# AUTOMATIC1111/stable-diffusion-webui

Hardware: AMD Instinct MI355X
Metric: images/sec SD1.5 512x512 20-step Euler-a, batch 8 per GPU (higher is better)
Workload: dtype f16

## Files before the change

### include/sdmi.h

```cpp
#ifndef SDMI_H
#define SDMI_H

#include <stdint.h>

#ifdef __cplusplus
extern "C" {
#endif

#define SDMI_VERSION 100

enum { SDMI_F16 = 0, SDMI_F32 = 1 };

typedef struct sdmi_engine sdmi_engine;

int sdmi_version(void);
const char* sdmi_last_error(void);
int sdmi_device_ok(void);


int64_t sdmi_attention_workspace_bytes(int B, int H, int M, int D);
int sdmi_attention(const void* q, const void* k, const void* v, void* out,
                   int B, int H, int N, int M, int D,
                   int ldq, int ldk, int ldv, int ldo, float scale,
                   void* workspace, int64_t workspace_bytes, void* stream);

int64_t sdmi_attention_wide_workspace_bytes(int B, int N, int M, int D);
int sdmi_attention_wide(const void* q, const void* k, const void* v, void* out,
                        int B, int N, int M, int D,
                        int ldq, int ldk, int ldv, int ldo, float scale,
                        void* workspace, int64_t workspace_bytes, void* stream);

int sdmi_attention_vt(const void* q, const void* k, const void* vt, void* out,
                      int B, int H, int N, int M, int D,
                      int ldq, int ldk, int vt_ld, int ldo, float scale, int force_generic, void* stream);

typedef struct sdmi_conv_desc {
    const void* a0;
    const void* a1;
    const void* w;
    const void* bias;
    const void* rowbias;
    const void* resid;
    void* out;
    int32_t c0, c1, lda0, lda1;
    int32_t B, Hi, Wi, Ho, Wo;
    int32_t taps;
    int32_t stride;
    int32_t pad;
    int32_t up;
    int32_t N;
    int32_t n_real;
    int32_t ldo, ldr;
    int32_t flags;
    float alpha;
    int32_t batch;
    int64_t a_bs, w_bs, o_bs, r_bs;
    int32_t force_generic;
    int32_t reserved;
    void* splitk_workspace;
    int64_t splitk_workspace_bytes;
} sdmi_conv_desc;

enum {
    SDMI_EP_OUT_F32  = 1,
    SDMI_EP_GEGLU    = 2,
    SDMI_EP_NCHW     = 4,
    SDMI_EP_BIAS_ROW = 8,
    SDMI_EP_WRAP = 128,
    SDMI_EP_TRANSPOSE = 64
};
int sdmi_conv_gemm(const sdmi_conv_desc* d, void* stream);
int64_t sdmi_conv_splitk_workspace_bytes(int M, int N, int K, int batch);

int sdmi_pack_conv_weight(const void* w_oihw, int dtype, void* out_f16, int O, int I, int kh, int kw,
                          int O_pad, int I_pad, int geglu, void* stream);

int sdmi_groupnorm(const void* x0, const void* x1, int c0, int c1, const void* gamma_f32, const void* beta_f32,
                   void* out_f16, int B, int HW, int groups, float eps, int silu,
                   void* workspace_f32, int64_t workspace_bytes, void* stream);
int64_t sdmi_groupnorm_workspace_bytes(int B, int HW, int groups);

int sdmi_layernorm(const void* x, const void* gamma_f32, const void* beta_f32, void* out_f16,
                   int64_t rows, int C, float eps, void* stream);

int64_t sdmi_rowchain_ff_pack_bytes(int C, int hidden);
int sdmi_rowchain_ff_pack(const void* w1_f16, const void* b1_f32_or_null, const void* w2_f16, void* packs, int C, int hidden,
                          void* stream);
int sdmi_rowchain_ff(const void* x_f16, void* out_f16, const void* ln_gamma_f32, const void* ln_beta_f32, const void* packs,
                     const void* b2_f32_or_null, int64_t rows, int C, int hidden, float eps, void* stream);

int sdmi_xattn_chain(const void* x_f16, void* out_f16, const void* ln_gamma_f32, const void* ln_beta_f32, const void* wq_f16,
                     const void* wo_f16, const void* bo_f32_or_null, const void* k_f16, const void* vt_f16, int64_t rows,
                     int rows_per_image, int C, int heads, int L, int Lpad, float eps, void* stream);


int sdmi_philox_randn(void* out_f32, int64_t n, uint64_t seed, uint32_t offset, void* stream);

int sdmi_slerp(void* out_f32, const void* low_f32, const void* high_f32, float val, int C, int H, int W, void* scratch_f32,
               void* stream);


int sdmi_cfg_prepare_input(const void* x_f32, const void* c_in_f32, void* x_in, int out_dtype,
                           int B, int reps, int64_t chw, void* stream);

int sdmi_cfg_prepare_concat(const void* x_f32, const void* c_in_f32, const void* c_concat_f32, void* x_in, int out_dtype,
                            int B, int reps, int C, int Cc, int64_t hw, uint32_t zero_reps, void* stream);

int sdmi_cfg_combine(const void* x_f32, const void* eps_f32, const void* c_out_f32, float cond_scale, int mode,
                     const void* mask_f32, const void* nmask_f32, const void* init_latent_f32,
                     void* denoised_f32, int B, int64_t chw, void* stream);

int sdmi_cfg_combine_affine(const void* x_f32, const void* out_f32, const void* c_out_f32, const void* c_skip_f32,
                            float cond_scale, const void* mask_f32, const void* nmask_f32, const void* init_latent_f32,
                            void* denoised_f32, int B, int64_t chw, void* stream);

int sdmi_euler_step(void* x_f32, const void* denoised_f32, const void* noise_f32_or_null,
                    float sigma, float sigma_down, float sigma_up, float s_noise, int64_t n, void* stream);

int sdmi_dpmpp2m_step(void* x_f32, const void* denoised_f32, const void* old_denoised_f32_or_null,
                      float ratio, float em1, float c1, float c2, int64_t n, void* stream);

int sdmi_ddim_step(void* x_f32, const void* e_t_f32, const void* noise_f32_or_null, void* pred_x0_f32_or_null,
                   float a_t, float a_prev, float sigma_t, float sqrt_one_minus_at, int64_t n, void* stream);

int sdmi_axpby(void* y_f32, const void* x_f32, float a, const void* z_f32_or_null, float b, int64_t n, void* stream);

int sdmi_lincomb(void* out_f32, const void* const* terms_f32, const float* coefs, int n_terms, int64_t n, void* stream);

int sdmi_dpm_error_partials(const void* x_low_f32, const void* x_high_f32, const void* x_prev_f32, float atol, float rtol,
                            void* partial256_f32, int64_t n, void* stream);

int sdmi_latent_resize(const void* in_f32, void* out_f32, int planes, int hi, int wi, int ho, int wo, int mode, void* stream);

int sdmi_mask_blend(void* x_f32, const void* init_f32, const void* mask_f32, const void* nmask_f32, int64_t n, void* stream);

int sdmi_image_to_u8(const void* img_f32_nchw, void* out_u8_nhwc, int B, int C, int H, int W, void* stream);

typedef struct sdmi_unet_config {
    int32_t in_channels, out_channels, model_channels;
    int32_t num_levels;
    int32_t channel_mult[8];
    int32_t num_res_blocks;
    int32_t attn_level[8];
    int32_t transformer_depth[8];
    int32_t num_heads;
    int32_t num_head_channels;
    int32_t context_dim;
    int32_t adm_in_channels;
    int32_t reserved[4];
} sdmi_unet_config;

typedef struct sdmi_vae_config {
    int32_t ch, num_levels;
    int32_t ch_mult[8];
    int32_t num_res_blocks, in_channels, out_ch, z_channels;
    float scale_factor;
    int32_t reserved[4];
} sdmi_vae_config;

sdmi_engine* sdmi_engine_create(int device);
void sdmi_engine_destroy(sdmi_engine* e);

int sdmi_unet_configure(sdmi_engine* e, const sdmi_unet_config* cfg);
int sdmi_unet_load_tensor(sdmi_engine* e, const char* key, const void* data, int dtype, int ndim,
                          const int64_t* shape, int on_device);
int sdmi_unet_finalize(sdmi_engine* e);

int sdmi_unet_update_weight(sdmi_engine* e, const char* key, const void* data, int dtype, int ndim,
                            const int64_t* shape, int on_device);

int sdmi_unet_hypernet_clear(sdmi_engine* e);
int sdmi_unet_hypernet_begin(sdmi_engine* e, float multiplier);
int sdmi_unet_hypernet_linear(sdmi_engine* e, int dim, int which, const void* w, const void* b, int dtype, int out_features,
                              int in_features, int on_device);
int sdmi_unet_hypernet_act(sdmi_engine* e, int dim, int which, int act);
int sdmi_unet_hypernet_layernorm(sdmi_engine* e, int dim, int which, const void* gamma, const void* beta, int dtype, int n, int on_device);

int sdmi_unet_update_vector(sdmi_engine* e, const char* key, const void* data, int dtype, int64_t n, int on_device);

int sdmi_lora_merge(void* out_f32, const void* w, int w_dtype, const void* up, int up_dtype, const void* down, int down_dtype,
                    int rows, int cols, int rank, float scale, void* stream);

int sdmi_weight_hadamard(void* out_f32, const void* w_f32, const void* a_f32, const void* b_f32, float scale, int64_t n, void* stream);
int sdmi_weight_kron(void* out_f32, const void* w_f32, const void* w1_f32, const void* w2_f32, int r1, int c1, int r2, int c2, int k,
                     float scale, void* stream);
int sdmi_weight_ia3(void* out_f32, const void* w_f32, const void* v_f32, int rows, int cols, int on_input, float scale, void* stream);
int sdmi_weight_dora(void* out_f32, const void* w_f32, const void* delta_f32, const void* dora_scale_f32, int rows, int cin, int k,
                     float mult, void* stream);

int sdmi_vae_configure(sdmi_engine* e, const sdmi_vae_config* cfg);
int sdmi_vae_load_tensor(sdmi_engine* e, const char* key, const void* data, int dtype, int ndim,
                         const int64_t* shape, int on_device);
int sdmi_vae_finalize(sdmi_engine* e);

int sdmi_unet_set_context(sdmi_engine* e, const void* context, int io_dtype, int Bn, int L, void* stream);
int sdmi_unet_set_context_cached(sdmi_engine* e, const void* context, int io_dtype, int Bn, int L, void* stream);
int sdmi_unet_forward(sdmi_engine* e, const void* x, const void* timesteps, const void* context, const void* y,
                      void* out, int io_dtype, int Bn, int h, int w, int L, void* stream);
enum { SDMI_CALL_UNIFORM_T = 1, SDMI_CALL_CFG_PAIRS = 2, SDMI_CALL_DERIVE = 4 };
int sdmi_unet_set_control(sdmi_engine* e, const void* const* tensors, const int64_t* numel, int n, int only_mid_control);
int sdmi_unet_forward_ex(sdmi_engine* e, const void* x, const void* timesteps, const void* context, const void* y,
                         void* out, int io_dtype, int Bn, int h, int w, int L, int call_flags, void* stream);

int sdmi_vae_decode(sdmi_engine* e, const void* z, int io_dtype, void* out_f32, int B, int h, int w, void* stream);

int sdmi_vae_encode(sdmi_engine* e, const void* x, int io_dtype, void* out_f32, int B, int H, int W, void* stream);

int64_t sdmi_engine_arena_bytes(sdmi_engine* e);
int sdmi_engine_set_option(sdmi_engine* e, const char* name, int value);

int sdmi_engine_tap_count(sdmi_engine* e);
int sdmi_engine_tap_info(sdmi_engine* e, int index, char* name_out, int capacity, int64_t* dims_bhwc);
int sdmi_engine_tap_read(sdmi_engine* e, int index, void* out_f16_nhwc, void* stream);

int sdmi_debug_set(const char* name, int value);
int sdmi_debug_set_str(const char* name, const char* value);

int sdmi_profile_begin(void);
int sdmi_profile_end(char* json_out, int capacity);

int sdmi_bench_conv_gemm(const sdmi_conv_desc* d, int iters, float* ms_out, void* stream);

typedef struct sdmi_clip_config {
    int vocab_size;
    int max_positions;
    int hidden;
    int layers;
    int heads;
    int intermediate;
    int act;
    float eps;
} sdmi_clip_config;

int sdmi_clip_configure(sdmi_engine* e, int slot, const sdmi_clip_config* cfg);
int sdmi_clip_load_tensor(sdmi_engine* e, int slot, const char* key, const void* data, int dtype, int ndim,
                          const int64_t* shape, int on_device);
int sdmi_clip_finalize(sdmi_engine* e, int slot);
int sdmi_clip_forward(sdmi_engine* e, int slot, const void* tokens_i32, const void* inputs_embeds_f32_or_null, int B, int L,
                      int skip, int apply_final_ln, void* out_f32, void* pooled_f32_or_null, void* stream);


enum {
    SDMI_RRDB_EP_NONE = 0,
    SDMI_RRDB_EP_LRELU = 1,
    SDMI_RRDB_EP_RES1 = 2,
    SDMI_RRDB_EP_RES2 = 3
// ... 98 lines not shown
```

### stable-diffusion-webui_amd/_lib.py

```python
from __future__ import annotations

import ctypes as C
import os
import re

_HERE = os.path.dirname(os.path.abspath(__file__))
LIB_PATH = os.environ.get("SDMI_LIB") or os.path.join(_HERE, "lib", "libsdmi.so")
HEADER_PATH = os.path.join(os.path.dirname(_HERE), "include", "sdmi.h")

F16, F32 = 0, 1
EP_OUT_F32, EP_GEGLU, EP_NCHW, EP_BIAS_ROW = 1, 2, 4, 8
EP_TRANSPOSE = 64
EP_WRAP = 128
RRDB_EP_NONE, RRDB_EP_LRELU, RRDB_EP_RES1, RRDB_EP_RES2 = 0, 1, 2, 3
RRDB_ST_F16, RRDB_ST_F32_NCHW, RRDB_ST_U8_HWC = 0, 1, 2
COMPACT_EP_NONE, COMPACT_EP_PRELU, COMPACT_EP_TAIL = 0, 1, 2


class SdmiError(RuntimeError):
    pass


class ConvDesc(C.Structure):
    _fields_ = [
        ("a0", C.c_void_p), ("a1", C.c_void_p), ("w", C.c_void_p), ("bias", C.c_void_p), ("rowbias", C.c_void_p),
        ("resid", C.c_void_p), ("out", C.c_void_p),
        ("c0", C.c_int32), ("c1", C.c_int32), ("lda0", C.c_int32), ("lda1", C.c_int32),
        ("B", C.c_int32), ("Hi", C.c_int32), ("Wi", C.c_int32), ("Ho", C.c_int32), ("Wo", C.c_int32),
        ("taps", C.c_int32), ("stride", C.c_int32), ("pad", C.c_int32), ("up", C.c_int32),
        ("N", C.c_int32), ("n_real", C.c_int32), ("ldo", C.c_int32), ("ldr", C.c_int32),
        ("flags", C.c_int32), ("alpha", C.c_float), ("batch", C.c_int32),
        ("a_bs", C.c_int64), ("w_bs", C.c_int64), ("o_bs", C.c_int64), ("r_bs", C.c_int64),
        ("force_generic", C.c_int32), ("reserved", C.c_int32),
        ("splitk_workspace", C.c_void_p), ("splitk_workspace_bytes", C.c_int64),
    ]


class RrdbDesc(C.Structure):
    _fields_ = [
        ("in_", C.c_void_p), ("w", C.c_void_p), ("bias", C.c_void_p), ("r1", C.c_void_p), ("r2", C.c_void_p), ("out", C.c_void_p),
        ("B", C.c_int32), ("H", C.c_int32), ("W", C.c_int32), ("cin", C.c_int32), ("lda", C.c_int32), ("up", C.c_int32),
        ("nout", C.c_int32), ("n_real", C.c_int32), ("ldo", C.c_int32), ("ldr1", C.c_int32), ("ldr2", C.c_int32),
        ("ep", C.c_int32), ("store", C.c_int32), ("alpha", C.c_float), ("beta", C.c_float),
    ]


class CompactDesc(C.Structure):
    _fields_ = [
        ("in_", C.c_void_p), ("w", C.c_void_p), ("bias", C.c_void_p), ("slope", C.c_void_p), ("base", C.c_void_p), ("out", C.c_void_p),
        ("B", C.c_int32), ("H", C.c_int32), ("W", C.c_int32), ("cin", C.c_int32), ("lda", C.c_int32), ("ldo", C.c_int32),
        ("n_real", C.c_int32), ("ep", C.c_int32), ("r", C.c_int32), ("base_u8", C.c_int32), ("out_u8", C.c_int32), ("grid_cap", C.c_int32),
    ]


class SwinAttnDesc(C.Structure):
    _fields_ = [
        ("qkv", C.c_void_p), ("bias", C.c_void_p), ("out", C.c_void_p),
        ("B", C.c_int32), ("H", C.c_int32), ("W", C.c_int32), ("heads", C.c_int32), ("D", C.c_int32),
        ("ldq", C.c_int32), ("ldo", C.c_int32), ("shift", C.c_int32), ("scale", C.c_float),
    ]


class SwinIRConfigC(C.Structure):
    _fields_ = [("embed_dim", C.c_int32), ("num_layers", C.c_int32), ("depths", C.c_int32 * 16), ("num_heads", C.c_int32),
                ("mlp_hidden", C.c_int32), ("resi_3conv", C.c_int32), ("scale", C.c_int32)]


class UNetConfigC(C.Structure):
    _fields_ = [
        ("in_channels", C.c_int32), ("out_channels", C.c_int32), ("model_channels", C.c_int32),
        ("num_levels", C.c_int32), ("channel_mult", C.c_int32 * 8), ("num_res_blocks", C.c_int32),
        ("attn_level", C.c_int32 * 8), ("transformer_depth", C.c_int32 * 8),
        ("num_heads", C.c_int32), ("num_head_channels", C.c_int32), ("context_dim", C.c_int32),
        ("adm_in_channels", C.c_int32), ("reserved", C.c_int32 * 4),
    ]


class VAEConfigC(C.Structure):
    _fields_ = [
        ("ch", C.c_int32), ("num_levels", C.c_int32), ("ch_mult", C.c_int32 * 8),
        ("num_res_blocks", C.c_int32), ("in_channels", C.c_int32), ("out_ch", C.c_int32), ("z_channels", C.c_int32),
        ("scale_factor", C.c_float), ("reserved", C.c_int32 * 4),
    ]


class ClipConfigC(C.Structure):
    _fields_ = [("vocab_size", C.c_int32), ("max_positions", C.c_int32), ("hidden", C.c_int32), ("layers", C.c_int32),
                ("heads", C.c_int32), ("intermediate", C.c_int32), ("act", C.c_int32), ("eps", C.c_float)]


def declared_symbols() -> list:
    src = open(HEADER_PATH).read()
    src = re.sub(r"/\*.*?\*/", "", src, flags=re.S)
    return sorted(set(re.findall(r"\b(sdmi_[a-z0-9_]+)\s*\(", src)))


if not os.path.exists(LIB_PATH):
    raise ImportError(
        f"{LIB_PATH} is missing: build it with `python -c 'import __graft_entry__ as g; g.build()'` "
        "(hipcc --offload-arch=gfx950). There is no CPU fallback for the MI355X engine.")

lib = C.CDLL(LIB_PATH)

_vp, _i, _i64, _f, _u32 = C.c_void_p, C.c_int, C.c_int64, C.c_float, C.c_uint32
_SIGS = {
    "sdmi_version": (C.c_int, []),
    "sdmi_last_error": (C.c_char_p, []),
    "sdmi_device_ok": (C.c_int, []),
    "sdmi_attention_workspace_bytes": (_i64, [_i, _i, _i, _i]),
    "sdmi_attention": (_i, [_vp, _vp, _vp, _vp, _i, _i, _i, _i, _i, _i, _i, _i, _i, _f, _vp, _i64, _vp]),
    "sdmi_attention_wide_workspace_bytes": (_i64, [_i, _i, _i, _i]),
    "sdmi_attention_wide": (_i, [_vp, _vp, _vp, _vp, _i, _i, _i, _i, _i, _i, _i, _i, _f, _vp, _i64, _vp]),
    "sdmi_attention_vt": (_i, [_vp, _vp, _vp, _vp, _i, _i, _i, _i, _i, _i, _i, _i, _i, _f, _i, _vp]),
    "sdmi_conv_gemm": (_i, [C.POINTER(ConvDesc), _vp]),
    "sdmi_conv_splitk_workspace_bytes": (_i64, [_i, _i, _i, _i]),
    "sdmi_bench_conv_gemm": (_i, [C.POINTER(ConvDesc), _i, C.POINTER(C.c_float), _vp]),
    "sdmi_pack_conv_weight": (_i, [_vp, _i, _vp, _i, _i, _i, _i, _i, _i, _i, _vp]),
    "sdmi_groupnorm": (_i, [_vp, _vp, _i, _i, _vp, _vp, _vp, _i, _i, _i, _f, _i, _vp, _i64, _vp]),
    "sdmi_groupnorm_workspace_bytes": (_i64, [_i, _i, _i]),
    "sdmi_layernorm": (_i, [_vp, _vp, _vp, _vp, _i64, _i, _f, _vp]),
    "sdmi_rowchain_ff_pack_bytes": (_i64, [_i, _i]),
    "sdmi_rowchain_ff_pack": (_i, [_vp, _vp, _vp, _vp, _i, _i, _vp]),
    "sdmi_rowchain_ff": (_i, [_vp, _vp, _vp, _vp, _vp, _vp, _i64, _i, _i, _f, _vp]),
    "sdmi_xattn_chain": (_i, [_vp, _vp, _vp, _vp, _vp, _vp, _vp, _vp, _vp, _i64, _i, _i, _i, _i, _i, _f, _vp]),
    "sdmi_philox_randn": (_i, [_vp, _i64, C.c_uint64, C.c_uint32, _vp]),
    "sdmi_slerp": (_i, [_vp, _vp, _vp, _f, _i, _i, _i, _vp, _vp]),
    "sdmi_cfg_prepare_input": (_i, [_vp, _vp, _vp, _i, _i, _i, _i64, _vp]),
    "sdmi_cfg_prepare_concat": (_i, [_vp, _vp, _vp, _vp, _i, _i, _i, _i, _i, _i64, _u32, _vp]),
    "sdmi_cfg_combine": (_i, [_vp, _vp, _vp, _f, _i, _vp, _vp, _vp, _vp, _i, _i64, _vp]),
    "sdmi_cfg_combine_affine": (_i, [_vp, _vp, _vp, _vp, _f, _vp, _vp, _vp, _vp, _i, _i64, _vp]),
    "sdmi_euler_step": (_i, [_vp, _vp, _vp, _f, _f, _f, _f, _i64, _vp]),
    "sdmi_dpmpp2m_step": (_i, [_vp, _vp, _vp, _f, _f, _f, _f, _i64, _vp]),
    "sdmi_ddim_step": (_i, [_vp, _vp, _vp, _vp, _f, _f, _f, _f, _i64, _vp]),
    "sdmi_axpby": (_i, [_vp, _vp, _f, _vp, _f, _i64, _vp]),
    "sdmi_dpm_error_partials": (_i, [_vp, _vp, _vp, _f, _f, _vp, _i64, _vp]),
    "sdmi_lincomb": (_i, [_vp, C.POINTER(_vp), C.POINTER(_f), _i, _i64, _vp]),
    "sdmi_mask_blend": (_i, [_vp, _vp, _vp, _vp, _i64, _vp]),
    "sdmi_latent_resize": (_i, [_vp, _vp, _i, _i, _i, _i, _i, _i, _vp]),
    "sdmi_image_to_u8": (_i, [_vp, _vp, _i, _i, _i, _i, _vp]),
    "sdmi_engine_create": (_vp, [_i]),
    "sdmi_engine_destroy": (None, [_vp]),
    "sdmi_unet_configure": (_i, [_vp, C.POINTER(UNetConfigC)]),
    "sdmi_unet_load_tensor": (_i, [_vp, C.c_char_p, _vp, _i, _i, C.POINTER(C.c_int64), _i]),
    "sdmi_unet_finalize": (_i, [_vp]),
    "sdmi_clip_configure": (_i, [_vp, _i, C.POINTER(ClipConfigC)]),
    "sdmi_clip_load_tensor": (_i, [_vp, _i, C.c_char_p, _vp, _i, _i, C.POINTER(C.c_int64), _i]),
    "sdmi_clip_finalize": (_i, [_vp, _i]),
    "sdmi_clip_forward": (_i, [_vp, _i, _vp, _vp, _i, _i, _i, _i, _vp, _vp, _vp]),
    "sdmi_unet_update_weight": (_i, [_vp, C.c_char_p, _vp, _i, _i, C.POINTER(C.c_int64), _i]),
    "sdmi_unet_hypernet_clear": (_i, [_vp]),
    "sdmi_unet_hypernet_begin": (_i, [_vp, _f]),
    "sdmi_unet_hypernet_linear": (_i, [_vp, _i, _i, _vp, _vp, _i, _i, _i, _i]),
    "sdmi_unet_hypernet_act": (_i, [_vp, _i, _i, _i]),
    "sdmi_unet_hypernet_layernorm": (_i, [_vp, _i, _i, _vp, _vp, _i, _i, _i]),
    "sdmi_unet_update_vector": (_i, [_vp, C.c_char_p, _vp, _i, _i64, _i]),
    "sdmi_lora_merge": (_i, [_vp, _vp, _i, _vp, _i, _vp, _i, _i, _i, _i, _f, _vp]),
    "sdmi_weight_hadamard": (_i, [_vp, _vp, _vp, _vp, _f, _i64, _vp]),
    "sdmi_weight_kron": (_i, [_vp, _vp, _vp, _vp, _i, _i, _i, _i, _i, _f, _vp]),
    "sdmi_weight_ia3": (_i, [_vp, _vp, _vp, _i, _i, _i, _f, _vp]),
    "sdmi_weight_dora": (_i, [_vp, _vp, _vp, _vp, _i, _i, _i, _f, _vp]),
    "sdmi_vae_configure": (_i, [_vp, C.POINTER(VAEConfigC)]),
    "sdmi_vae_load_tensor": (_i, [_vp, C.c_char_p, _vp, _i, _i, C.POINTER(C.c_int64), _i]),
    "sdmi_vae_finalize": (_i, [_vp]),
    "sdmi_unet_set_context": (_i, [_vp, _vp, _i, _i, _i, _vp]),
    "sdmi_unet_set_context_cached": (_i, [_vp, _vp, _i, _i, _i, _vp]),
    "sdmi_unet_forward": (_i, [_vp, _vp, _vp, _vp, _vp, _vp, _i, _i, _i, _i, _i, _vp]),
    "sdmi_unet_set_control": (_i, [_vp, _vp, _vp, _i, _i]),
    "sdmi_unet_forward_ex": (_i, [_vp, _vp, _vp, _vp, _vp, _vp, _i, _i, _i, _i, _i, _i, _vp]),
    "sdmi_vae_decode": (_i, [_vp, _vp, _i, _vp, _i, _i, _i, _vp]),
    "sdmi_vae_encode": (_i, [_vp, _vp, _i, _vp, _i, _i, _i, _vp]),
    "sdmi_debug_set": (_i, [C.c_char_p, _i]),
    "sdmi_debug_set_str": (_i, [C.c_char_p, C.c_char_p]),
    "sdmi_profile_begin": (_i, []),
    "sdmi_profile_end": (_i, [C.c_char_p, _i]),
    "sdmi_engine_arena_bytes": (_i64, [_vp]),
    "sdmi_engine_set_option": (_i, [_vp, C.c_char_p, _i]),
    "sdmi_engine_tap_count": (_i, [_vp]),
    "sdmi_engine_tap_info": (_i, [_vp, _i, C.c_char_p, _i, C.POINTER(C.c_int64)]),
    "sdmi_engine_tap_read": (_i, [_vp, _i, _vp, _vp]),
    "sdmi_rrdb_conv": (_i, [C.POINTER(RrdbDesc), _vp]),
    "sdmi_esrgan_blob_floats": (_i64, [_i, _i]),
    "sdmi_esrgan_create": (_vp, [_vp, _vp, _i64, _i, _i, _i]),
    "sdmi_esrgan_destroy": (None, [_vp]),
    "sdmi_esrgan_scratch_bytes": (_i64, [_vp, _i, _i, _i]),
    "sdmi_esrgan_run": (_i, [_vp, _vp, _i, _i, _i, _i, _vp, _i, _vp]),
    "sdmi_compact_conv": (_i, [C.POINTER(CompactDesc), _vp]),
    "sdmi_compact_blob_floats": (_i64, [_i, _i]),
    "sdmi_compact_create": (_vp, [_vp, _vp, _i64, _i, _i]),
    "sdmi_compact_destroy": (None, [_vp]),
    "sdmi_compact_scratch_bytes": (_i64, [_vp, _i, _i, _i]),
    "sdmi_compact_run": (_i, [_vp, _vp, _i, _i, _i, _i, _vp, _i, _vp]),
    "sdmi_swin_attention": (_i, [C.POINTER(SwinAttnDesc), _vp]),
    "sdmi_swin_layernorm": (_i, [_vp, _vp, _vp, _vp, _i64, _i, _i, _f, _vp]),
    "sdmi_swinir_blob_floats": (_i64, [C.POINTER(SwinIRConfigC)]),
    "sdmi_swinir_create": (_vp, [_vp, _vp, _i64, C.POINTER(SwinIRConfigC)]),
    "sdmi_swinir_destroy": (None, [_vp]),
    "sdmi_swinir_scratch_bytes": (_i64, [_vp, _i, _i, _i]),
    "sdmi_swinir_run": (_i, [_vp, _vp, _i, _i, _i, _i, _vp, _i, _vp]),
}
for _name, (_res, _args) in _SIGS.items():
    _fn = getattr(lib, _name)
    _fn.restype = _res
    _fn.argtypes = _args


def last_error() -> str:
    return (lib.sdmi_last_error() or b"").decode("utf-8", "replace")


def check(rc: int, what: str = "sdmi call"):
    if rc != 0:
        raise SdmiError(f"{what} failed: {last_error()}")


def device_ok() -> bool:
    return bool(lib.sdmi_device_ok())


def require_device():
    if not device_ok():
        raise SdmiError("no gfx950 (MI355X) device visible to HIP: the engine has no CPU path")


def ptr(t):
    return None if t is None else C.c_void_p(t.data_ptr())


def stream_ptr():
    import torch
    return C.c_void_p(torch.cuda.current_stream().cuda_stream)


def dtype_code(t) -> int:
    import torch
    if t.dtype == torch.float16:
        return F16
    if t.dtype == torch.float32:
        return F32
    raise SdmiError(f"unsupported dtype {t.dtype}: the engine takes fp16 or fp32 tensors")
```

### stable-diffusion-webui_amd/csrc/capi.cpp

```cpp
#include "engine.h"
#include "prof.h"
#include <cstring>

namespace sdmi {
extern int g_vae_attn_rows;
int unet_forward(sdmi_engine* e, const void* x, const void* t, const void* ctx, const void* y, void* out, int io_dtype,
                 int Bn, int h, int w, int L, hipStream_t s);
int vae_decode(sdmi_engine* e, const void* z, int io_dtype, float* out, int B, int h, int w, hipStream_t s);
int vae_encode(sdmi_engine* e, const void* x, int io_dtype, float* out, int B, int H, int W, hipStream_t s);
int engine_load_unet_tensor(sdmi_engine* e, const char* key, const void* data, int dtype, int ndim, const int64_t* shape, int on_device);
int engine_load_vae_tensor(sdmi_engine* e, const char* key, const void* data, int dtype, int ndim, const int64_t* shape, int on_device);
int engine_unet_finalize(sdmi_engine* e);
int engine_clip_configure(sdmi_engine* e, int slot, const sdmi_clip_config* cfg);
int engine_clip_load_tensor(sdmi_engine* e, int slot, const char* key, const void* data, int dtype, int ndim, const int64_t* shape, int on_device);
int engine_clip_finalize(sdmi_engine* e, int slot);
int engine_clip_forward(sdmi_engine* e, int slot, const int* tokens, const float* inputs_embeds, int B, int L, int skip,
                        int apply_final_ln, float* out, float* pooled, hipStream_t s);
int engine_unet_update_weight(sdmi_engine* e, const char* key, const void* data, int dtype, int ndim, const int64_t* shape, int on_device);
int engine_vae_finalize(sdmi_engine* e);
int engine_hypernet_clear(sdmi_engine* e);
int engine_hypernet_begin(sdmi_engine* e, float multiplier);
int engine_hypernet_linear(sdmi_engine* e, int dim, int which, const void* w, const void* b, int dtype, int out_f, int in_f, int on_device);
int engine_hypernet_act(sdmi_engine* e, int dim, int which, int act);
int engine_hypernet_layernorm(sdmi_engine* e, int dim, int which, const void* g, const void* b, int dtype, int n, int on_device);
// ... 82 lines not shown
    SDMI_REQUIRE(ldq % 8 == 0 && ldk % 8 == 0 && ldo % 8 == 0, "sdmi_attention_wide: row strides must be multiples of 8 elements");
    SDMI_REQUIRE(ldq >= D && ldk >= D && ldv >= D && ldo >= D, "sdmi_attention_wide: row strides must be at least D");
    SDMI_REQUIRE(workspace && workspace_bytes >= sdmi_attention_wide_workspace_bytes(B, N, M, D), "attention workspace too small");
    hipStream_t s = (hipStream_t)stream;
    const int mpad = (M + 63) / 64 * 64;
    const int rows_max = N < kWideRows ? N : kWideRows;
    half_t* vt = (half_t*)workspace;
    float* S = (float*)(vt + (size_t)B * D * mpad);
    half_t* P = (half_t*)(S + (size_t)rows_max * mpad);
    if (launch_transpose_v((const half_t*)v, vt, B, 1, M, D, ldv, mpad, s)) return 1;
    for (int b = 0; b < B; ++b)
        for (int r0 = 0; r0 < N; r0 += kWideRows) {
            const int rows = N - r0 < kWideRows ? N - r0 : kWideRows;
            GemmP p{};
            p.a0 = (const half_t*)q + ((size_t)b * N + r0) * ldq; p.c0 = D; p.cin = D; p.lda0 = ldq;
            p.w = (const half_t*)k + (size_t)b * M * ldk; p.ldw = ldk;
            p.out = S;
            p.Hi = rows; p.Wi = 1; p.Ho = rows; p.Wo = 1; p.taps = 1; p.stride = 1;
            p.M = rows; p.N = mpad; p.n_valid = M; p.K = D; p.ldo = mpad; p.rows_per_batch = rows; p.n_real = mpad;
            p.flags = EP_OUT_F32;
            p.alpha = scale;
            if (launch_gemm(p, 1, false, true, s)) return 1;
            if (launch_softmax_rows(S, P, rows, M, mpad, mpad, s)) return 1;
            GemmP g{};
            g.a0 = P; g.c0 = mpad; g.cin = mpad; g.lda0 = mpad;
            g.w = vt + (size_t)b * D * mpad; g.ldw = mpad;
            g.out = (half_t*)out + ((size_t)b * N + r0) * ldo;
            g.Hi = rows; g.Wi = 1; g.Ho = rows; g.Wo = 1; g.taps = 1; g.stride = 1;
            g.M = rows; g.N = D; g.K = mpad; g.ldo = ldo; g.rows_per_batch = rows; g.n_real = D;
            g.alpha = 1.f;
            if (launch_gemm(g, 1, false, true, s)) return 1;
        }
    return 0;
    API_GUARD_END
}

static int desc_to_p(const sdmi_conv_desc* d, GemmP* p) {
    SDMI_REQUIRE(d != nullptr, "null descriptor");
    SDMI_REQUIRE(d->a0 && d->w && d->out, "sdmi_conv_gemm: null a0 / w / out");
    SDMI_REQUIRE(d->B > 0 && d->Hi > 0 && d->Wi > 0 && d->Ho > 0 && d->Wo > 0 && d->N > 0 && d->c0 > 0 && (!d->a1 || d->c1 > 0),
                 "sdmi_conv_gemm: B, Hi, Wi, Ho, Wo, N, c0 (and c1 with a second source) must be positive");
    SDMI_REQUIRE(d->stride >= 0 && d->stride <= 2, "sdmi_conv_gemm: stride must be 1 or 2 (0 = 1)");
    *p = GemmP{};
    p->a0 = (const half_t*)d->a0; p->a1 = (const half_t*)d->a1; p->w = (const half_t*)d->w;
    p->bias = (const float*)d->bias; p->rowbias = (const float*)d->rowbias; p->resid = (const half_t*)d->resid;
    p->out = d->out;
    p->c0 = d->c0; p->c1 = d->a1 ? d->c1 : 0; p->cin = p->c0 + p->c1;
    p->lda0 = d->lda0 ? d->lda0 : d->c0; p->lda1 = d->lda1 ? d->lda1 : d->c1;
    p->Hi = d->Hi; p->Wi = d->Wi; p->Ho = d->Ho; p->Wo = d->Wo;
    p->taps = d->taps; p->stride = d->stride ? d->stride : 1; p->pad = d->pad; p->up = d->up;
    SDMI_REQUIRE(p->taps == 1 || p->taps == 9, "taps must be 1 or 9");
    SDMI_REQUIRE(p->c0 % 8 == 0 && p->c1 % 8 == 0, "sdmi_conv_gemm: c0 and c1 must each be a multiple of 8 (pad channels)");
    SDMI_REQUIRE(p->lda0 >= p->c0 && (!p->a1 || p->lda1 >= p->c1), "sdmi_conv_gemm: lda smaller than the channel count");
    p->M = d->B * d->Ho * d->Wo; p->N = d->N; p->K = p->taps * p->cin;
    p->ldw = p->K; p->ldrb = d->N;
    p->rows_per_batch = d->Ho * d->Wo;
    p->n_real = d->n_real ? d->n_real : d->N;
    p->flags = d->flags;
    SDMI_REQUIRE(!(p->flags & EP_NCHW) || (p->n_real > 0 && p->n_real <= p->N), "sdmi_conv_gemm: n_real must lie in 1 .. N");
    SDMI_REQUIRE(!(p->flags & EP_GEGLU) || p->N % 64 == 0, "sdmi_conv_gemm: SDMI_EP_GEGLU needs N % 64 == 0 (32 values | 32 gates)");
    const int batch = d->batch > 0 ? d->batch : 1;
    const bool tr = (p->flags & EP_TRANSPOSE) != 0, nchw = (p->flags & EP_NCHW) != 0;
    const long cols = tr ? p->rows_per_batch : (p->flags & EP_GEGLU) ? p->N / 2 : p->N;
    const long rows = tr ? (long)d->B * p->N : p->M;
    p->ldo = d->ldo ? d->ldo : (int)cols; p->ldr = d->ldr ? d->ldr : d->N;
    SDMI_REQUIRE(nchw || p->ldo >= cols, "sdmi_conv_gemm: ldo smaller than the stored columns");
    SDMI_REQUIRE(!p->resid || p->ldr >= p->N, "sdmi_conv_gemm: ldr smaller than N");
    p->alpha = d->alpha == 0.f ? 1.f : d->alpha;
    p->a_bs = d->a_bs; p->w_bs = d->w_bs; p->o_bs = d->o_bs; p->r_bs = d->r_bs;
    const long foot = nchw ? (long)d->B * p->n_real * p->rows_per_batch : (rows - 1) * p->ldo + cols;
    SDMI_REQUIRE(batch == 1 || p->o_bs >= foot, "sdmi_conv_gemm: batch > 1 needs o_bs >= the elements one batch element stores");
    SDMI_REQUIRE(batch == 1 || (p->a_bs >= 0 && p->w_bs >= 0 && p->r_bs >= 0), "sdmi_conv_gemm: negative batch stride");
    const size_t need = gemm_splitk_ws_bytes(p->M, p->N, p->K, batch);
    if (d->splitk_workspace && need && (size_t)d->splitk_workspace_bytes >= need) p->splitk_ws = (float*)d->splitk_workspace;
    return 0;
}

int64_t sdmi_conv_splitk_workspace_bytes(int M, int N, int K, int batch) { return (int64_t)gemm_splitk_ws_bytes(M, N, K, batch); }

int sdmi_conv_gemm(const sdmi_conv_desc* d, void* stream) {
    API_GUARD_BEGIN
    GemmP p;
    if (desc_to_p(d, &p)) return 1;
    const char* env = getenv("SDMI_NO_GLDS");
    return launch_gemm(p, d->batch > 0 ? d->batch : 1, d->force_generic == 1, !(env && env[0] == '1') && d->force_generic != 2,
                       (hipStream_t)stream);
    API_GUARD_END
}

int sdmi_bench_conv_gemm(const sdmi_conv_desc* d, int iters, float* ms_out, void* stream) {
    API_GUARD_BEGIN
    GemmP p;
    if (desc_to_p(d, &p)) return 1;
    hipStream_t s = (hipStream_t)stream;
    hipEvent_t e0, e1;
    SDMI_CHECK_HIP(hipEventCreate(&e0));
    SDMI_CHECK_HIP(hipEventCreate(&e1));
    const bool glds = d->force_generic != 2;
    for (int i = 0; i < 2; ++i)
        if (launch_gemm(p, d->batch > 0 ? d->batch : 1, d->force_generic == 1, glds, s)) return 1;
    SDMI_CHECK_HIP(hipEventRecord(e0, s));
    for (int i = 0; i < iters; ++i)
        if (launch_gemm(p, d->batch > 0 ? d->batch : 1, d->force_generic == 1, glds, s)) return 1;
    SDMI_CHECK_HIP(hipEventRecord(e1, s));
    SDMI_CHECK_HIP(hipEventSynchronize(e1));
    float ms = 0.f;
    SDMI_CHECK_HIP(hipEventElapsedTime(&ms, e0, e1));
    *ms_out = ms / (float)iters;
    (void)hipEventDestroy(e0);
    (void)hipEventDestroy(e1);
    return 0;
    API_GUARD_END
}

int sdmi_pack_conv_weight(const void* w, int dtype, void* out, int O, int I, int kh, int kw, int O_pad, int I_pad, int geglu,
                          void* stream) {
    API_GUARD_BEGIN
    return launch_pack_conv_weight(w, dtype, (half_t*)out, O, I, kh, kw, O_pad, I_pad, geglu, (hipStream_t)stream);
    API_GUARD_END
}

int64_t sdmi_groupnorm_workspace_bytes(int B, int HW, int groups) { return groupnorm_ws_bytes(B, HW, groups); }

int sdmi_groupnorm(const void* x0, const void* x1, int c0, int c1, const void* gamma, const void* beta, void* out, int B, int HW,
                   int groups, float eps, int silu, void* ws, int64_t ws_bytes, void* stream) {
    API_GUARD_BEGIN
    SDMI_REQUIRE(ws && ws_bytes >= groupnorm_ws_bytes(B, HW, groups), "groupnorm workspace too small");
    return launch_groupnorm((const half_t*)x0, (const half_t*)x1, c0, x1 ? c1 : 0, (const float*)gamma, (const float*)beta,
                            (half_t*)out, B, HW, groups, eps, silu != 0, (float*)ws, (hipStream_t)stream);
    API_GUARD_END
}

int sdmi_layernorm(const void* x, const void* gamma, const void* beta, void* out, int64_t rows, int C, float eps, void* stream) {
    API_GUARD_BEGIN
    return launch_layernorm((const half_t*)x, (const float*)gamma, (const float*)beta, (half_t*)out, rows, C, eps, (hipStream_t)stream);
    API_GUARD_END
}

int64_t sdmi_rowchain_ff_pack_bytes(int C, int hidden) { return (int64_t)rowchain_ff_pack_bytes(C, hidden); }
int sdmi_rowchain_ff_pack(const void* w1, const void* b1, const void* w2, void* packs, int C, int hidden, void* stream) {
    API_GUARD_BEGIN
    SDMI_REQUIRE(w1 && w2 && packs, "null argument");
    return launch_rowchain_ff_pack((const half_t*)w1, (const float*)b1, (const half_t*)w2, packs, C, hidden, false, (hipStream_t)stream);
    API_GUARD_END
}
int sdmi_rowchain_ff(const void* x, void* out, const void* g, const void* b, const void* packs, const void* b2, int64_t rows, int C,
                     int hidden, float eps, void* stream) {
    API_GUARD_BEGIN
    SDMI_REQUIRE(x && out && g && b && packs, "null argument");
    return launch_rowchain_ff((const half_t*)x, (half_t*)out, (const float*)g, (const float*)b, packs, (const float*)b2, (long)rows, C,
                              hidden, eps, (hipStream_t)stream);
    API_GUARD_END
}
int sdmi_xattn_chain(const void* x, void* out, const void* g, const void* b, const void* wq, const void* wo, const void* bo, const void* k,
                     const void* vt, int64_t rows, int rows_per_image, int C, int heads, int L, int Lpad, float eps, void* stream) {
    API_GUARD_BEGIN
    return launch_xattn_chain((const half_t*)x, (half_t*)out, (const float*)g, (const float*)b, (const half_t*)wq, (const half_t*)wo,
                              (const float*)bo, (const half_t*)k, (const half_t*)vt, (long)rows, rows_per_image, C, heads, L, Lpad, eps,
                              (hipStream_t)stream);
    API_GUARD_END
}


int sdmi_philox_randn(void* out, int64_t n, uint64_t seed, uint32_t offset, void* stream) {
    API_GUARD_BEGIN
    return launch_philox((float*)out, n, seed, offset, (hipStream_t)stream);
    API_GUARD_END
}

int sdmi_slerp(void* out, const void* low, const void* high, float val, int C, int H, int W, void* scratch, void* stream) {
    API_GUARD_BEGIN
    SDMI_REQUIRE(out && low && high && scratch && C > 0 && H > 0 && W > 0, "bad arguments");
    return launch_slerp((float*)out, (const float*)low, (const float*)high, val, C, H, W, (float*)scratch, (hipStream_t)stream);
    API_GUARD_END
}

int sdmi_cfg_prepare_input(const void* x, const void* c_in, void* x_in, int out_dtype, int B, int reps, int64_t chw, void* stream) {
    API_GUARD_BEGIN
    return launch_cfg_prepare((const float*)x, (const float*)c_in, x_in, out_dtype, B, reps, chw, (hipStream_t)stream);
    API_GUARD_END
}

int sdmi_cfg_prepare_concat(const void* x, const void* c_in, const void* c_concat, void* x_in, int out_dtype, int B, int reps,
                            int C, int Cc, int64_t hw, uint32_t zero_reps, void* stream) {
    API_GUARD_BEGIN
    SDMI_REQUIRE(x && c_concat && x_in, "null pointer");
    SDMI_REQUIRE(B > 0 && reps > 0 && reps <= 32 && C > 0 && Cc > 0 && hw > 0, "bad sizes");
    return launch_cfg_prepare_concat((const float*)x, (const float*)c_in, (const float*)c_concat, x_in, out_dtype, B, reps, C, Cc, hw,
                                     zero_reps, (hipStream_t)stream);
    API_GUARD_END
}

int sdmi_cfg_combine(const void* x, const void* eps, const void* c_out, float cond_scale, int mode, const void* mask,
                     const void* nmask, const void* init_latent, void* den, int B, int64_t chw, void* stream) {
    API_GUARD_BEGIN
    SDMI_REQUIRE(mode == 1 || (x && c_out), "sigma-space combine needs x and c_out");
    return launch_cfg_combine((const float*)x, (const float*)eps, (const float*)c_out, cond_scale, mode, (const float*)mask,
                              (const float*)nmask, (const float*)init_latent, (float*)den, B, chw, (hipStream_t)stream);
    API_GUARD_END
}

int sdmi_euler_step(void* x, const void* den, const void* noise, float sigma, float sigma_down, float sigma_up, float s_noise,
                    int64_t n, void* stream) {
    API_GUARD_BEGIN
    SDMI_REQUIRE(x && den && n >= 0, "sdmi_euler_step: null x / denoised or negative n");
    return launch_euler_step((float*)x, (const float*)den, (const float*)noise, sigma, sigma_down, sigma_up, s_noise, n,
                             (hipStream_t)stream);
    API_GUARD_END
}

int sdmi_dpmpp2m_step(void* x, const void* den, const void* old, float ratio, float em1, float c1, float c2, int64_t n,
                      void* stream) {
    API_GUARD_BEGIN
    SDMI_REQUIRE(x && den && n >= 0, "sdmi_dpmpp2m_step: null x / denoised or negative n");
    return launch_dpmpp2m_step((float*)x, (const float*)den, (const float*)old, ratio, em1, c1, c2, n, (hipStream_t)stream);
    API_GUARD_END
}

int sdmi_ddim_step(void* x, const void* e_t, const void* noise, void* pred_x0, float a_t, float a_prev, float sigma_t,
                   float sqrt_one_minus_at, int64_t n, void* stream) {
    API_GUARD_BEGIN
    SDMI_REQUIRE(x && e_t && n >= 0, "sdmi_ddim_step: null x / e_t or negative n");
    return launch_ddim_step((float*)x, (const float*)e_t, (const float*)noise, (float*)pred_x0, a_t, a_prev, sigma_t,
                            sqrt_one_minus_at, n, (hipStream_t)stream);
    API_GUARD_END
}

int sdmi_dpm_error_partials(const void* x_low, const void* x_high, const void* x_prev, float atol, float rtol, void* partial256_f32,
                            int64_t n, void* stream) {
    API_GUARD_BEGIN
    SDMI_REQUIRE(x_low && x_high && x_prev && partial256_f32 && n > 0, "null argument");
    return launch_dpm_error((const float*)x_low, (const float*)x_high, (const float*)x_prev, atol, rtol, (float*)partial256_f32, n,
                            (hipStream_t)stream);
    API_GUARD_END
}
int sdmi_lincomb(void* out, const void* const* terms, const float* coefs, int n_terms, int64_t n, void* stream) {
    API_GUARD_BEGIN
    SDMI_REQUIRE(out && terms && coefs, "null argument");
    return launch_lincomb((float*)out, (const float* const*)terms, coefs, n_terms, n, (hipStream_t)stream);
    API_GUARD_END
}

int sdmi_latent_resize(const void* in, void* out, int planes, int hi, int wi, int ho, int wo, int mode, void* stream) {
    API_GUARD_BEGIN
    SDMI_REQUIRE(in && out, "null argument");
    return launch_latent_resize((const float*)in, (float*)out, planes, hi, wi, ho, wo, mode, (hipStream_t)stream);
    API_GUARD_END
}

int sdmi_cfg_combine_affine(const void* x, const void* out, const void* c_out, const void* c_skip, float cond_scale,
                            const void* mask, const void* nmask, const void* init_latent, void* den, int B, int64_t chw, void* stream) {
    API_GUARD_BEGIN
    SDMI_REQUIRE(x && out && c_out && c_skip && den, "null argument");
    return launch_cfg_combine_affine((const float*)x, (const float*)out, (const float*)c_out, (const float*)c_skip, cond_scale,
                                     (const float*)mask, (const float*)nmask, (const float*)init_latent, (float*)den, B, chw,
                                     (hipStream_t)stream);
    API_GUARD_END
}

int sdmi_mask_blend(void* x, const void* init, const void* mask, const void* nmask, int64_t n, void* stream) {
    API_GUARD_BEGIN
    SDMI_REQUIRE(x && init && mask && nmask, "null argument");
    return launch_mask_blend((float*)x, (const float*)init, (const float*)mask, (const float*)nmask, n, (hipStream_t)stream);
    API_GUARD_END
}

int sdmi_axpby(void* y, const void* x, float a, const void* z, float b, int64_t n, void* stream) {
    API_GUARD_BEGIN
    SDMI_REQUIRE(y && x && n >= 0, "sdmi_axpby: null y / x or negative n");
    return launch_axpby((float*)y, (const float*)x, a, (const float*)z, b, n, (hipStream_t)stream);
    API_GUARD_END
}

int sdmi_image_to_u8(const void* img, void* out, int B, int C, int H, int W, void* stream) {
    API_GUARD_BEGIN
    return launch_image_to_u8((const float*)img, (uint8_t*)out, B, C, H, W, (hipStream_t)stream);
    API_GUARD_END
}

sdmi_engine* sdmi_engine_create(int device) {
    try {
        if (hipSetDevice(device) != hipSuccess) {
            set_error("hipSetDevice failed");
            return nullptr;
        }
        sdmi_engine* e = new sdmi_engine();
        e->device = device;
        const char* g = getenv("SDMI_NO_GLDS");
        if (g && g[0] == '1') e->use_glds = false;
        const char* f = getenv("SDMI_FORCE_GENERIC");
        if (f && f[0] == '1') e->force_generic = true;
        return e;
    } catch (...) {
        set_error("engine allocation failed");
        return nullptr;
    }
}
void sdmi_engine_destroy(sdmi_engine* e) { delete e; }

int sdmi_unet_configure(sdmi_engine* e, const sdmi_unet_config* cfg) {
    API_GUARD_BEGIN
    SDMI_REQUIRE(e && cfg, "null argument");
    SDMI_REQUIRE(cfg->num_levels >= 1 && cfg->num_levels <= 8, "num_levels out of range");
    SDMI_REQUIRE(cfg->model_channels % 64 == 0, "model_channels must be a multiple of 64");
    SDMI_REQUIRE(cfg->context_dim % 64 == 0, "context_dim must be a multiple of 64");
    SDMI_REQUIRE(cfg->in_channels <= 16 && cfg->out_channels <= 64, "in_channels <= 16, out_channels <= 64");
    e->unet.cfg = *cfg;
    e->unet.ready = false;
    return 0;
    API_GUARD_END
}
int sdmi_unet_load_tensor(sdmi_engine* e, const char* key, const void* data, int dtype, int ndim, const int64_t* shape,
// ... 414 lines not shown
```

### stable-diffusion-webui_amd/csrc/common.h

```cpp
#pragma once
#include <hip/hip_runtime.h>
#include <stdint.h>
#include <string>

typedef _Float16 half_t;
typedef _Float16 h8 __attribute__((ext_vector_type(8)));
typedef _Float16 h4 __attribute__((ext_vector_type(4)));
typedef _Float16 h2 __attribute__((ext_vector_type(2)));
typedef float f4 __attribute__((ext_vector_type(4)));
typedef float f16v __attribute__((ext_vector_type(16)));

namespace sdmi {

#ifndef SDMI_GELU_SIG
#define SDMI_GELU_SIG 1
#endif
__device__ __forceinline__ float geglu_gate(float val, float g) {
    const float gc = fminf(fmaxf(g, -10.0f), 10.0f);
    const float g2 = gc * gc;
    float p = fmaf(1.01426306e-3f, g2, -0.106775724f);
    p = fmaf(p, g2, -2.30112135f);
    const float e = __builtin_amdgcn_exp2f(p * gc);
    return (val * g) * __builtin_amdgcn_rcpf(1.0f + e);
}

void set_error(const std::string& msg);
const char* get_error();

#define SDMI_CHECK_HIP(expr)                                                                       \
    do {                                                                                           \
        hipError_t _e = (expr);                                                                    \
        if (_e != hipSuccess) {                                                                    \
            ::sdmi::set_error(std::string(#expr) + ": " + hipGetErrorString(_e));                  \
            return 1;                                                                              \
        }                                                                                          \
    } while (0)

#define SDMI_REQUIRE(cond, msg)                                                                    \
    do {                                                                                           \
        if (!(cond)) {                                                                             \
            ::sdmi::set_error(std::string("requirement failed: ") + #cond + " — " + (msg));        \
            return 1;                                                                              \
        }                                                                                          \
    } while (0)

static inline int cdiv(int64_t a, int64_t b) { return (int)((a + b - 1) / b); }

struct PerDeviceOnce {
    int level[64] = {};
    bool need(int want = 1) {
        int d = 0;
        if (hipGetDevice(&d) != hipSuccess) d = 0;
        d &= 63;
        if (level[d] >= want) return false;
        level[d] = want;
        return true;
    }
};

constexpr int kZeroPageHalfs = 16384;
const half_t* zero_page();

struct GemmP {
    const half_t* a0;
    const half_t* a1;
    const half_t* w;
    const float* bias;
    const float* rowbias;
    const half_t* resid;
    void* out;
    const half_t* zero;
    int c0, c1, cin;
    int lda0, lda1;
    int Hi, Wi, Ho, Wo;
    int taps, stride, pad, up;
    int M, N, K;
    int ldo, ldr;
    int ldw;
    int ldrb;
    int rows_per_batch;
    int n_real;
    int n_valid;
    int flags;
    float alpha;
    long a_bs, w_bs, o_bs, r_bs;
    float* splitk_ws;
    int splitk;
    int splitk_steps;
    long long* dbg;
    float* stats_out;
    int stats_cpg;
    int stats_nchunk;
    int korder;
    int tile_order;
    float bias_scale;
    const int* gate;
    const float* ln_stats;
    const float* ln_s;
    int ln_np;
    float ln_inv_c, ln_eps;
    float* lnp_out;
    int lnp_np;
};

enum { EP_OUT_F32 = 1, EP_GEGLU = 2, EP_NCHW = 4, EP_BIAS_ROW = 8,
       EP_QUICK_GELU = 16, EP_GELU = 32,
       EP_TRANSPOSE = 64,
       EP_WRAP = 128,
       EP_DBG_NO_BAR_A = 0x100, EP_DBG_NO_BAR_B = 0x200, EP_DBG_NO_GLDS = 0x400, EP_DBG_NO_VMWAIT = 0x800,
       EP_DBG_NO_DSREAD = 0x1000,
       EP_LNFOLD = 0x4000,
       EP_HILO = 0x8000,
       EP_NARROW = 0x2000
     };

__host__ __device__ inline half_t* gemm_out_lo(const GemmP& p) {
    return (p.flags & EP_HILO) ? reinterpret_cast<half_t*>(const_cast<float*>(p.ln_stats)) : nullptr;
}
__host__ __device__ inline const half_t* gemm_resid_lo(const GemmP& p) { return (p.flags & EP_HILO) ? reinterpret_cast<const half_t*>(p.ln_s) : nullptr; }

int launch_gemm(const GemmP& p, int batch, bool force_generic, bool use_glds, hipStream_t s, int* stats_nchunk_out = nullptr,
                int* lnp_np_out = nullptr);
extern int g_ep_wide;
extern int g_small_linear_lds;
extern int g_gn_small;
extern int g_gn_fuse;
size_t gemm_splitk_ws_bytes(int M, int N, int K, int batch);
int gemm_set_override(const char* spec);
extern int g_force_gemm_cfg;
extern int g_shortk_gemm_cfg;
extern int g_shortk_max_k;
extern int g_geglu_gemm_cfg;
extern int g_conv_korder;
extern int g_conv_korder_default;
extern int g_tile_order;
extern int g_vt_mode;
extern long g_gn_band_elems;
extern int g_gn_apply_blocks;
extern int g_gemm_lin;
extern int g_gemm_pipe;
extern int g_gemm_pipe_default;
extern int g_force_gemm_split;
extern int g_attn_kvt;
extern int g_attn_occ;
extern int g_attn_lds_pad;
extern int g_attn_fold_min_m;
extern int g_attn_tau;
extern unsigned long long g_attn_dbg;
extern int g_gemm_dbgflags;
extern unsigned long long g_gemm_dbg;

struct AttnP {
    const half_t* q;
    const half_t* k;
    const half_t* vt;
    half_t* out;
    int B, H, N, M, D;
    int ldq, ldk, vt_ld, ldo;
    float scale_log2;
    int causal;
    long long* dbg;
    float tau;
};
int launch_attention(const AttnP& p, bool force_generic, hipStream_t s);
int launch_transpose_v(const half_t* v, half_t* vt, int B, int H, int M, int D, int ldv, int Mpad, hipStream_t s);

bool rowchain_supports(int C);
size_t rowchain_ff_pack_bytes(int C, int hidden);
int launch_rowchain_ff_pack(const half_t* w1, const float* b1, const half_t* w2, void* packs, int C, int hidden, bool permuted,
                            hipStream_t s);
int launch_rowchain_ff(const half_t* x, half_t* out, const float* gamma, const float* beta, const void* packs, const float* bias_out,
                       long rows, int C, int hidden, float eps, hipStream_t s);

int launch_xattn_chain(const half_t* x, half_t* out, const float* gamma, const float* beta, const half_t* wq, const half_t* wo,
                       const float* bo, const half_t* k, const half_t* vt, long rows, int rows_per_image, int C, int heads, int L, int Lpad,
                       float eps, hipStream_t s);

enum { RRDB_EP_NONE = 0, RRDB_EP_LRELU = 1,
       RRDB_EP_RES1 = 2,
       RRDB_EP_RES2 = 3 };
enum { RRDB_ST_F16 = 0, RRDB_ST_F32_NCHW = 1, RRDB_ST_U8_HWC = 2 };
struct RrdbP {
    const half_t* in;
    const half_t* w;
    const float* bias;
    const half_t* r1;
    const half_t* r2;
    void* out;
    const half_t* zero;
    int B, H, W;
    int cin, lda, ldw, up;
    int ldo, n_real, ldr1, ldr2;
    int ep, store;
    float alpha, beta;
    long long M;
};
int launch_rrdb_conv(const RrdbP& p, int nout, hipStream_t s);
int launch_rrdb_input(const void* in, int u8, half_t* out, int B, int C, int H, int W, int f, int cpad, hipStream_t s);

enum { COMPACT_EP_NONE = 0, COMPACT_EP_PRELU = 1,
       COMPACT_EP_TAIL = 2 };
struct CompactP {
    const half_t* in;
    const half_t* w;
    const float* bias;
    const float* slope;
    const void* base;
    void* out;
    const half_t* zero;
    int B, H, W;
    int cin, lda, ldo, n_real;
    int ep, r, base_u8, out_u8;
    int grid_cap;
    int tiles_x, tiles_y;
    int tiles;
};
int launch_compact_conv(const CompactP& p, hipStream_t s);

struct SwinAttnP {
    const half_t* qkv;
    const float* bias;
    half_t* out;
    int B, H, W;
    int heads, D, ldq, ldo;
    int shift;
    float scale;
};
int launch_swin_attention(const SwinAttnP& p, hipStream_t s);
int launch_swin_layernorm(const half_t* x, const float* gamma, const float* beta, half_t* out, int64_t rows, int C, int ld, float eps,
                          hipStream_t s);
int launch_swin_input(const void* in, int u8, half_t* out, int B, int H, int W, int Hp, int Wp, int cpad, hipStream_t s);
int launch_swin_lrelu(half_t* x, int64_t n, float slope, hipStream_t s);
int launch_swin_output(const float* src, void* out, int out_u8, int B, int H, int W, int Hp, int Wp, hipStream_t s);

int launch_groupnorm(const half_t* x0, const half_t* x1, int c0, int c1, const float* gamma, const float* beta,
                     half_t* out, int B, int HW, int groups, float eps, bool silu, float* ws, hipStream_t s, int pre_nchunk = 0,
                     const half_t* x0_lo = nullptr, const half_t* x1_lo = nullptr);
int64_t groupnorm_ws_bytes(int B, int HW, int groups);
int launch_layernorm(const half_t* x, const float* gamma, const float* beta, half_t* out, int64_t rows, int C,
                     float eps, hipStream_t s, const half_t* x_lo = nullptr);
int launch_ln_rowstats(const half_t* x, float* stats, int64_t rows, int C, float eps, hipStream_t s);
int launch_ln_fold_weights(const half_t* w, const float* gamma, const float* beta, const float* bias, half_t* wf, float* s_out,
                           float* c_out, int n_rows, int K, int C, hipStream_t s);

int launch_philox(float* out, int64_t n, uint64_t seed, uint32_t offset, hipStream_t s);
int launch_cfg_prepare(const float* x, const float* c_in, void* xin, int out_dtype, int B, int reps, int64_t chw, hipStream_t s);
int launch_slerp(float* out, const float* low, const float* high, float val, int C, int H, int W, float* scratch, hipStream_t s);
int launch_weight_hadamard(float* out, const float* w, const float* a, const float* b, float scale, int64_t n, hipStream_t s);
int launch_weight_kron(float* out, const float* w, const float* w1, const float* w2, int r1, int c1, int r2, int c2, int k, float scale,
                       hipStream_t s);
int launch_weight_ia3(float* out, const float* w, const float* v, int rows, int cols, int on_input, float scale, hipStream_t s);
int launch_weight_dora(float* out, const float* w, const float* delta, const float* dora_scale, int rows, int cin, int k, float mult,
                       hipStream_t s);
int launch_cfg_prepare_concat(const float* x, const float* c_in, const float* cond, void* xin, int out_dtype, int B, int reps,
                              int C, int Cc, int64_t hw, unsigned zero_reps, hipStream_t s);
int launch_cfg_combine(const float* x, const float* eps, const float* c_out, float cond_scale, int mode,
                       const float* mask, const float* nmask, const float* init_latent, float* den, int B,
                       int64_t chw, hipStream_t s);
int launch_euler_step(float* x, const float* den, const float* noise, float sigma, float sigma_down, float sigma_up,
                      float s_noise, int64_t n, hipStream_t s);
int launch_dpmpp2m_step(float* x, const float* den, const float* old, float ratio, float em1, float c1, float c2,
                        int64_t n, hipStream_t s);
int launch_ddim_step(float* x, const float* e, const float* noise, float* pred_x0, float a_t, float a_prev,
                     float sigma_t, float somat, int64_t n, hipStream_t s);
int launch_axpby(float* y, const float* x, float a, const float* z, float b, int64_t n, hipStream_t s);
int launch_dpm_error(const float* lo, const float* hi, const float* prev, float atol, float rtol, float* partial256, int64_t n,
                     hipStream_t s);
int launch_lincomb(float* out, const float* const* terms, const float* coefs, int n_terms, int64_t n, hipStream_t s);
int launch_lora_merge(float* out, const void* w, int w_dtype, const void* up, int up_dtype, const void* down, int down_dtype,
                      int rows, int cols, int rank, float scale, hipStream_t s);
int launch_clip_embed(const int* tokens, const void* tok_emb, int tok_dtype, const float* pos_emb, const float* inputs_embeds,
                      half_t* out, int B, int L, int C, int vocab, hipStream_t s);
int launch_clip_pool(const int* tokens, const half_t* hidden, float* pooled, int B, int L, int C, hipStream_t s);
int launch_latent_resize(const float* in, float* out, int planes, int hi, int wi, int ho, int wo, int mode, hipStream_t s);
int launch_cfg_combine_affine(const float* x, const float* out, const float* c_out, const float* c_skip, float cond_scale,
                              const float* mask, const float* nmask, const float* init_latent, float* den, int B, int64_t chw,
                              hipStream_t s);
int launch_act_f16(half_t* x, int64_t n, int kind, hipStream_t s);
int launch_axpy_f16(half_t* y, const half_t* x, const half_t* h, float a, int64_t n, hipStream_t s);
int launch_silu_f32(const float* x, float* y, int64_t n, hipStream_t s);
int launch_mask_blend(float* x, const float* init, const float* mask, const float* nmask, int64_t n, hipStream_t s);
int launch_image_to_u8(const float* img, uint8_t* out, int B, int C, int H, int W, hipStream_t s);

int launch_nchw_to_nhwc(const void* x, int dtype, half_t* out, int B, int C, int HW, int cpad, float scale,
                        const float* mix_w, const float* mix_b, hipStream_t s, bool lo_ch = false);
int launch_add_nchw_residual(const half_t* src, const half_t* src_lo, const void* ctrl, int dtype, half_t* dst, half_t* dst_lo, int B, int C,
                             int HW, hipStream_t s);
int launch_copy_out(const float* src, void* dst, int dtype, int64_t n, hipStream_t s);
int launch_convert_to_f16(const void* src, int dtype, half_t* dst, int64_t n, hipStream_t s);
int launch_convert_to_f32(const void* src, int dtype, float* dst, int64_t n, hipStream_t s);
int launch_ctx_compare(const void* src, int dtype, const half_t* cached, int B, int L, int Lpad, int C, int* gate, hipStream_t s);
int launch_ctx_update_gated(const void* src, int dtype, half_t* cached, int B, int L, int Lpad, int C, const int* gate, hipStream_t s);
int launch_timestep_embedding(const void* t, int dtype, float* out, int B, int dim, hipStream_t s);
int launch_small_linear(const float* a, const half_t* w, const float* bias, const float* add, float* out, int B,
                        int N, int K, int lda, int ldo, bool silu_in, bool silu_out, hipStream_t s);
int launch_softmax_rows(const float* in, half_t* out, int64_t rows, int cols, int ldi, int ldo, hipStream_t s);
int launch_pack_conv_weight(const void* w, int dtype, half_t* out, int O, int I, int kh, int kw, int O_pad,
                            int I_pad, int geglu, hipStream_t s);
int launch_pack_bias(const void* b, int dtype, float* out, int O, int O_pad, int geglu, hipStream_t s);

}
```

### stable-diffusion-webui_amd/csrc/engine.cpp

```cpp
#include "engine.h"

#include <algorithm>
#include <cmath>
#include <cstring>
#include <functional>

namespace sdmi {

static thread_local std::string g_err;
void set_error(const std::string& m) { g_err = m; }
const char* get_error() { return g_err.c_str(); }

const half_t* zero_page() {
    static thread_local int cached_dev = -1;
    static thread_local half_t* cached = nullptr;
    static std::map<int, half_t*> pages;
    int dev = 0;
    if (hipGetDevice(&dev) != hipSuccess) return nullptr;
    if (dev == cached_dev) return cached;
    auto it = pages.find(dev);
    if (it == pages.end()) {
        void* p = nullptr;
        if (hipMalloc(&p, kZeroPageHalfs * sizeof(half_t)) != hipSuccess) return nullptr;
        if (hipMemset(p, 0, kZeroPageHalfs * sizeof(half_t)) != hipSuccess) return nullptr;
// ... 481 lines not shown
    {
        ConvArgs c;
        c.a0 = t1; c.c0 = w.cin; c.B = B; c.Hi = H; c.Wi = Wd; c.Ho = H; c.Wo = Wd; c.pad = 1;
        if (embs) { c.rowbias = embs + w.emb_off; c.ldrb = emb_ld; }
        c.out = h1; c.ldo = w.cout;
        c.out_lo = acc ? r.lo(h1, M * w.cout) : nullptr;
        c.stats_C = w.cout;
        TRY(run_conv(r, w.c1, c));
    }
    half_t* t2 = r.H(M * w.cout);
    TRY(run_gn(r, w.n2, h1, nullptr, w.cout, 0, B, HW, eps, true, t2, acc ? r.lo(h1, M * w.cout) : nullptr));
    const half_t* resid = x0;
    const half_t* resid_lo = x0_lo;
    if (w.has_skip) {
        half_t* sk = acc ? r.S(M * w.cout) : r.H(M * w.cout);
        ConvArgs c;
        c.a0 = x0; c.a1 = x1; c.c0 = c0; c.c1 = c1; c.B = B; c.Hi = H; c.Wi = Wd; c.Ho = H; c.Wo = Wd;
        c.out = sk; c.ldo = w.cout;
        c.resid_lo = nullptr;
        c.out_lo = acc ? r.lo(sk, M * w.cout) : nullptr;
        c.bias_scale = ss;
        TRY(run_conv(r, w.skip, c));
        resid = sk;
        resid_lo = c.out_lo;
    } else {
        SDMI_REQUIRE(x1 == nullptr, "identity skip with a concatenated input");
    }
    half_t* o = out_buf ? out_buf : (reuse ? o_pre : (acc ? r.S(M * w.cout) : r.H(M * w.cout)));
    {
        ConvArgs c;
        c.a0 = t2; c.c0 = w.cout; c.B = B; c.Hi = H; c.Wi = Wd; c.Ho = H; c.Wo = Wd; c.pad = 1;
        c.resid = resid; c.ldr = w.cout; c.out = o; c.ldo = w.cout;
        c.resid_lo = resid_lo; c.out_lo = acc ? r.lo(o, (out_buf ? LR : M) * w.cout) : nullptr;
        c.alpha = ss; c.bias_scale = ss;
        c.stats_C = ss == 1.f ? w.cout : 0;
        c.stats_ws_pre = st_pre;
        TRY(run_conv(r, w.c2, c));
    }
    if (reuse) r.ar->rewind(mk);
    *out = o;
    return 0;
}

static int run_attn(Run& r, const half_t* q, const half_t* k, const half_t* vt, half_t* out, int B, int H, int N, int M,
                    int D, int ldq, int ldk, int vt_ld, int ldo) {
    if (r.dry) return 0;
    AttnP p{};
    p.q = q; p.k = k; p.vt = vt; p.out = out;
    p.B = B; p.H = H; p.N = N; p.M = M; p.D = D;
    p.ldq = ldq; p.ldk = ldk; p.vt_ld = vt_ld; p.ldo = ldo;
    p.scale_log2 = (1.0f / sqrtf((float)D)) * 1.4426950408889634f;
    return launch_attention(p, r.e->force_generic, r.s);
}

static int run_vt(Run& r, const ConvW& Wv, const half_t* x, int ldx, int B, int tokens, int tokens_pad, half_t* vt,
                  bool bias_row, const int* gate = nullptr) {
    if (r.dry) return 0;
    GemmP p{};
    const int C = Wv.n_pad, K = Wv.cin_pad;
    if (g_vt_mode == 1 && tokens == tokens_pad && tokens % 4 == 0 && ldx == K && gate == nullptr) {
        p.a0 = x; p.c0 = K; p.cin = K; p.lda0 = ldx;
        p.w = Wv.w; p.ldw = K;
        p.bias = bias_row ? Wv.b : nullptr;
        p.out = vt;
        p.Hi = tokens; p.Wi = 1; p.Ho = tokens; p.Wo = 1;
        p.taps = 1; p.stride = 1; p.pad = 0; p.up = 0;
        p.M = B * tokens; p.N = C; p.K = K; p.n_valid = C;
        p.ldo = tokens_pad; p.rows_per_batch = tokens; p.n_real = C;
        p.flags = EP_TRANSPOSE;
        p.alpha = 1.f;
        return launch_gemm(p, 1, r.e->force_generic, r.e->use_glds, r.s);
    }
    p.a0 = Wv.w; p.c0 = K; p.cin = K; p.lda0 = K;
    p.w = x; p.ldw = ldx;
    p.bias = bias_row ? Wv.b : nullptr;
    p.out = vt;
    p.Hi = C; p.Wi = 1; p.Ho = C; p.Wo = 1;
    p.taps = 1; p.stride = 1; p.pad = 0; p.up = 0;
    p.M = C; p.N = tokens_pad; p.K = K; p.n_valid = tokens;
    p.ldo = tokens_pad; p.rows_per_batch = C; p.n_real = tokens_pad;
    p.flags = bias_row ? EP_BIAS_ROW : 0;
    p.alpha = 1.f;
    p.a_bs = 0; p.w_bs = (long)tokens * ldx;
    p.o_bs = (long)C * tokens_pad;
    p.gate = gate;
    return launch_gemm(p, B, r.e->force_generic, r.e->use_glds, r.s);
}

static bool hn_has_dim(const sdmi_engine* e, int dim) {
    for (const auto& n : e->hypernets)
        if (n.by_dim.count(dim)) return true;
    return false;
}

template <typename Alloc>
static int run_hn(Run& r, int dim, int which, const half_t* x, size_t rows, Alloc alloc, bool no_split, const half_t** out) {
    const half_t* cur = x;
    for (const HnNet& net : r.e->hypernets) {
        auto it = net.by_dim.find(dim);
        if (it == net.by_dim.end()) continue;
        const HnModule& mod = which ? it->second.second : it->second.first;
        const half_t* h = cur;
        int width = dim;
        half_t* y = nullptr;
        for (size_t i = 0; i < mod.ops.size(); ++i) {
            const HnOp& op = mod.ops[i];
            const bool last = i + 1 == mod.ops.size();
            if (op.kind == 0) {
                SDMI_REQUIRE(op.lin.cin_pad == width || r.dry, "hypernetwork layer widths do not chain");
                half_t* t = alloc(rows * (size_t)op.lin.n_pad);
                if (last) {
                    SDMI_REQUIRE(op.lin.n_pad == dim, "hypernetwork output width must equal its input width");
                    TRY(run_linear(r, op.lin, h, (int)rows, cur, t, op.lin.n_pad, net.multiplier, no_split));
                    y = t;
                } else {
                    TRY(run_linear(r, op.lin, h, (int)rows, nullptr, t, op.lin.n_pad, 1.f, no_split));
                }
                h = t;
                width = op.lin.n_pad;
            } else if (op.kind == 1) {
                if (!r.dry) TRY(launch_act_f16(const_cast<half_t*>(h), (int64_t)rows * width, op.act, r.s));
            } else {
                half_t* t = alloc(rows * (size_t)width);
                if (!r.dry) TRY(launch_layernorm(h, op.ln.g, op.ln.b, t, (int64_t)rows, width, 1e-5f, r.s));
                h = t;
            }
        }
        if (y == nullptr) {
            SDMI_REQUIRE(width == dim, "hypernetwork output width must equal its input width");
            y = alloc(rows * (size_t)dim);
            if (!r.dry) TRY(launch_axpy_f16(y, cur, h, net.multiplier, (int64_t)rows * dim, r.s));
        }
        cur = y;
    }
    *out = cur;
    return 0;
}

static int run_st(Run& r, const STW& st, const half_t* x, int B, int H, int Wd, int L, half_t** out,
                  const std::string& name = std::string(), int Bh = 0) {
    sdmi_engine* e = r.e;
    const int C = st.ch, HW = H * Wd;
    const size_t M = (size_t)B * HW;
    int B1 = Bh > 0 ? Bh : B;
    size_t M1 = (size_t)B1 * HW;
    const int Npad = rup(HW, 64);
    const bool reuse = r.reuse();
    half_t* o_pre = reuse ? r.H(M * C) : nullptr;
    half_t* cur_pre = reuse ? r.H(M * C) : nullptr;
    half_t* pp[2] = {reuse ? r.H(M * C) : nullptr, (reuse && st.blocks.size() > 1) ? r.H(M * C) : nullptr};
    const size_t mk = r.ar->mark();
    const bool acc = r.acc();
    const size_t MC = M * C;
    half_t* n0 = r.H(M * C);
    TRY(run_gn(r, st.norm, x, nullptr, C, 0, B1, HW, 1e-6f, false, n0, r.lo(x, MC)));
    half_t* cur = reuse ? cur_pre : r.S(M * C);
    const bool fold_any = e->ln_fold && !acc && !hn_has_dim(e, C) && !e->force_generic && e->use_glds && g_vt_mode == 1 && HW == Npad && HW % 4 == 0;
    r.lnp_want = fold_any && e->ln_fold >= 2;
    TRY(run_linear(r, st.proj_in, n0, (int)M1, nullptr, cur, C, 1.f, false, nullptr, r.lo(cur, MC)));
    if (reuse) r.ar->rewind(mk);
    int bi = 0, blk = 0;
    for (const TBlockW& b : st.blocks) {
        const std::string bname = name + ".transformer_blocks." + std::to_string(bi++);
        const bool fold = fold_any;
        half_t* a1 = nullptr;
        if (fold) {
            LnStats st1;
            TRY(run_ln_stats(r, b.ln1, cur, M, &st1));
            half_t* qk = r.H(M * 2 * C);
            TRY(run_linear_ln(r, b.qk1, b.ln1, cur, st1, (int)M, qk, 2 * C));
            half_t* vt = r.H((size_t)B * C * Npad);
            TRY(run_vt_ln(r, b.v1, b.ln1, cur, st1, B, HW, Npad, vt));
            a1 = r.H(M * C);
            TRY(run_attn(r, qk, qk + C, vt, a1, B, st.heads, HW, HW, st.dhead, 2 * C, 2 * C, Npad, C));
        }
        half_t* n1 = fold ? nullptr : r.H(M * C);
        if (!fold) TRY(run_ln(r, b.ln1, cur, M1, n1, r.lo(cur, MC)));
        if (fold) {
        } else if (!hn_has_dim(e, C)) {
            half_t* qk = r.H(M * 2 * C);
            TRY(run_linear(r, b.qk1, n1, (int)M1, nullptr, qk, 2 * C));
            half_t* vt = r.H((size_t)B * C * Npad);
            TRY(run_vt(r, b.v1, n1, C, B1, HW, Npad, vt, false));
            a1 = r.H(M * C);
            TRY(run_attn(r, qk, qk + C, vt, a1, B1, st.heads, HW, HW, st.dhead, 2 * C, 2 * C, Npad, C));
        } else {
            auto alloc = [&](size_t n) { return r.H(n); };
            const half_t *xk = nullptr, *xv = nullptr;
            TRY(run_hn(r, C, 0, n1, M, alloc, false, &xk));
            TRY(run_hn(r, C, 1, n1, M, alloc, false, &xv));
            ConvW wq = b.qk1, wk = b.qk1;
            wq.n_pad = wk.n_pad = C; wq.cout = wk.cout = C;
            wk.w = b.qk1.w + (size_t)C * b.qk1.cin_pad;
            if (b.qk1.b) wk.b = b.qk1.b + C;
            half_t* q = r.H(M * C);
            half_t* k = r.H(M * C);
            TRY(run_linear(r, wq, n1, (int)M, nullptr, q, C));
            TRY(run_linear(r, wk, xk, (int)M, nullptr, k, C));
            half_t* vt = r.H((size_t)B * C * Npad);
            TRY(run_vt(r, b.v1, xv, C, B, HW, Npad, vt, false));
            a1 = r.H(M * C);
            TRY(run_attn(r, q, k, vt, a1, B, st.heads, HW, HW, st.dhead, C, C, Npad, C));
        }
        half_t* x1 = r.S(M * C);
        r.lnp_want = fold && e->ln_fold >= 2;
        TRY(run_linear(r, b.o1, a1, (int)M1, cur, x1, C, 1.f, false, r.lo(cur, MC), r.lo(x1, MC)));
        if (B1 != B) {
            if (!r.dry) SDMI_CHECK_HIP(hipMemcpyAsync(x1 + M1 * C, x1, M1 * C * sizeof(half_t), hipMemcpyDeviceToDevice, r.s));
            if (!r.dry && acc) SDMI_CHECK_HIP(hipMemcpyAsync(x1 + MC + M1 * C, x1 + MC, M1 * C * sizeof(half_t), hipMemcpyDeviceToDevice, r.s));
            B1 = B; M1 = M;
        }
        r.tap(bname + ".attn1+x", x1, B, H, Wd, C);
        const bool chain_ok = !fold && !acc && !e->force_generic && e->use_glds && rowchain_supports(C) && HW % 128 == 0 && e->n_streams <= 1;
        const bool xchain = chain_ok && (e->fuse_rows & 1) && !hn_has_dim(e, C) && st.heads == 8 && st.dhead == 40 && !b.q2.b &&
                            b.q2.cin_pad == C && b.q2.n_pad == C && b.o2.cin_pad == C && b.o2.n_pad == C;
        half_t* x2 = nullptr;
        if (xchain) {
            x2 = r.S(M * C);
            if (!r.dry) {
                SDMI_REQUIRE(e->ctx_valid && e->ctx_B == (r.Btot ? r.Btot : B), "context not set for this batch size");
                TRY(launch_xattn_chain(x1, x2, b.ln2.g, b.ln2.b, b.q2.w, b.o2.w, b.o2.b, e->ctx_k[b.ctx_slot] + (size_t)r.b0 * e->ctx_L * C,
                                       e->ctx_vt[b.ctx_slot] + (size_t)r.b0 * C * e->ctx_Lpad, (long)M, HW, C, st.heads, e->ctx_L,
                                       e->ctx_Lpad, 1e-5f, r.s));
            }
        } else {
        half_t* q2 = nullptr;
        if (fold) {
            LnStats st2;
            TRY(run_ln_stats(r, b.ln2, x1, M, &st2));
            q2 = r.H(M * C);
            TRY(run_linear_ln(r, b.q2, b.ln2, x1, st2, (int)M, q2, C));
        } else {
            half_t* n2 = r.H(M * C);
            TRY(run_ln(r, b.ln2, x1, M, n2, r.lo(x1, MC)));
            q2 = r.H(M * C);
            TRY(run_linear(r, b.q2, n2, (int)M, nullptr, q2, C));
        }
        half_t* a2 = r.H(M * C);
        if (!r.dry) {
            SDMI_REQUIRE(e->ctx_valid && e->ctx_B == (r.Btot ? r.Btot : B), "context not set for this batch size");
            AttnP p{};
            p.q = q2; p.out = a2;
            p.k = e->ctx_k[b.ctx_slot] + (size_t)r.b0 * e->ctx_L * C;
            p.vt = e->ctx_vt[b.ctx_slot] + (size_t)r.b0 * C * e->ctx_Lpad;
            p.B = B; p.H = st.heads; p.N = HW; p.M = e->ctx_L; p.D = st.dhead;
            p.ldq = C; p.ldk = C; p.vt_ld = e->ctx_Lpad; p.ldo = C;
            p.scale_log2 = (1.0f / sqrtf((float)st.dhead)) * 1.4426950408889634f;
            TRY(launch_attention(p, e->force_generic, r.s));
        }
        x2 = r.S(M * C);
        r.lnp_want = fold && e->ln_fold >= 2;
        TRY(run_linear(r, b.o2, a2, (int)M, x1, x2, C, 1.f, false, r.lo(x1, MC), r.lo(x2, MC)));
        }
        r.tap(bname + ".attn2+x", x2, B, H, Wd, C);
        half_t* x3 = reuse ? pp[blk & 1] : r.S(M * C);
        if (chain_ok && (e->fuse_rows & 2) && b.ff1.geglu && b.ff1.n_pad % 64 == 0 && b.ff2.cin_pad * 2 == b.ff1.n_pad && b.ff1.cin_pad == C &&
            b.ff2.n_pad == C) {
            if (!r.dry) {
                const int hidden = b.ff2.cin_pad;
                if (!b.ff_packs) {
                    void* pk = nullptr;
                    SDMI_CHECK_HIP(hipMalloc(&pk, rowchain_ff_pack_bytes(C, hidden)));
                    e->owned.push_back(pk);
                    b.ff_packs = (char*)pk;
                }
                if (b.ff_epoch != e->weights_epoch) {
                    TRY(launch_rowchain_ff_pack(b.ff1.w, b.ff1.b, b.ff2.w, b.ff_packs, C, hidden, true, r.s));
                    b.ff_epoch = e->weights_epoch;
                }
                TRY(launch_rowchain_ff(x2, x3, b.ln3.g, b.ln3.b, b.ff_packs, b.ff2.b, (long)M, C, hidden, 1e-5f, r.s));
            }
        } else {
        half_t* g = nullptr;
        if (fold) {
            LnStats st3;
            TRY(run_ln_stats(r, b.ln3, x2, M, &st3));
            g = r.H(M * 4 * C);
            TRY(run_linear_ln(r, b.ff1, b.ln3, x2, st3, (int)M, g, 4 * C));
        } else {
            half_t* n3 = r.H(M * C);
            TRY(run_ln(r, b.ln3, x2, M, n3, r.lo(x2, MC)));
            g = r.H(M * 4 * C);
            TRY(run_linear(r, b.ff1, n3, (int)M, nullptr, g, 4 * C));
        }
        r.lnp_want = fold && e->ln_fold >= 2;
        TRY(run_linear(r, b.ff2, g, (int)M, x2, x3, C, 1.f, false, r.lo(x2, MC), r.lo(x3, MC)));
        }
        r.tap(bname, x3, B, H, Wd, C);
        cur = x3;
        ++blk;
        if (reuse) r.ar->rewind(mk);
    }
    half_t* o = reuse ? o_pre : r.S(M * C);
    TRY(run_linear(r, st.proj_out, cur, (int)M, x, o, C, 1.f, false, r.lo(x, MC), r.lo(o, MC)));
    *out = o;
    (void)L;
    return 0;
}

static void ctx_free(sdmi_engine* e) {
    for (void* p : e->ctx_owned) (void)hipFree(p);
    e->ctx_owned.clear(); e->ctx_k.clear(); e->ctx_vt.clear();
    e->ctx_f16 = nullptr; e->ctx_valid = false;
}

static void collect_st(const UNetW& u, std::vector<const STW*>* out) {
    for (auto& blk : u.input) for (auto& L : blk) if (L.kind == UNetLayer::ST) out->push_back(&L.st);
    for (auto& L : u.middle) if (L.kind == UNetLayer::ST) out->push_back(&L.st);
    for (auto& blk : u.output) for (auto& L : blk) if (L.kind == UNetLayer::ST) out->push_back(&L.st);
}

static int unet_set_context(sdmi_engine* e, const void* ctx, int dtype, int Bn, int L, hipStream_t s, bool conditional = false) {
    UNetW& u = e->unet;
    SDMI_REQUIRE(u.ready, "unet not finalized");
    const int cd = u.cfg.context_dim;
    const int Lpad = rup(L, 64);
    const int* gate = nullptr;
    if (conditional && e->ctx_valid && e->ctx_B == Bn && e->ctx_L == L && !e->ctx_k.empty() && !hn_has_dim(e, cd)) {
        if (!e->ctx_gate) {
            SDMI_CHECK_HIP(hipMalloc((void**)&e->ctx_gate, 256));
            e->owned.push_back(e->ctx_gate);
        }
        SDMI_CHECK_HIP(hipMemsetAsync(e->ctx_gate, 0, sizeof(int), s));
        TRY(launch_ctx_compare(ctx, dtype, e->ctx_f16, Bn, L, Lpad, cd, e->ctx_gate, s));
        gate = e->ctx_gate;
    }
    if (e->ctx_B != Bn || e->ctx_L != L || e->ctx_k.empty()) {
        SDMI_CHECK_HIP(hipStreamSynchronize(s));
        ctx_free(e);
        void* p = nullptr;
        SDMI_CHECK_HIP(hipMalloc(&p, (size_t)Bn * Lpad * cd * sizeof(half_t)));
// ... 1331 lines not shown
        c.a0 = a; c.c0 = w.cin_pad; c.B = B; c.Hi = c.Ho = Hp; c.Wi = c.Wo = Wp; c.pad = w.taps == 9 ? 1 : 0;
        c.resid = resid; c.ldr = w.n_pad; c.out = o; c.ldo = w.n_pad; c.flags = flags;
        const size_t mark = r.ar->mark();
        const int rc = run_conv(r, w, c);
        r.ar->rewind(mark);
        return rc;
    };
    auto lnorm = [&](const NormW& w, const half_t* a, half_t* o) -> int {
        return r.dry ? 0 : launch_swin_layernorm(a, w.g, w.b, o, (int64_t)M, n.C, Cp, 1e-5f, r.s);
    };
    auto lrelu = [&](half_t* a, size_t cnt, float slope) -> int { return r.dry ? 0 : launch_swin_lrelu(a, (int64_t)cnt, slope, r.s); };
    auto resi = [&](const ConvW* w, const half_t* a, const half_t* resid, half_t* o) -> int {
        if (!n.cfg.resi_3conv) return conv(w[0], a, resid, o);
        TRY(conv(w[0], a, nullptr, c1));
        TRY(lrelu(c1, M * 64, 0.2f));
        TRY(conv(w[1], c1, nullptr, c2));
        TRY(lrelu(c2, M * 64, 0.2f));
        return conv(w[2], c2, resid, o);
    };

    if (!r.dry) {
        TRY(launch_swin_input(in, in_u8, x0, B, H, W, Hp, Wp, 64, r.s));
        if (n.lda > 32 * n.cfg.num_heads)
            SDMI_CHECK_HIP(hipMemsetAsync(att, 0, M * n.lda * sizeof(half_t), r.s));
    }
    TRY(conv(n.first, x0, nullptr, feat));
    half_t* x = pool[0];
    std::vector<half_t*> free_ = {pool[1], pool[2], pool[3]};
    TRY(lnorm(n.pe_norm, feat, x));
    for (const sdmi_swinir::Layer& L : n.layers) {
        half_t* cur = x;
        for (size_t j = 0; j < L.blocks.size(); ++j) {
            const sdmi_swinir::Block& bk = L.blocks[j];
            half_t* mid = free_.back(); free_.pop_back();
            half_t* nxt = free_.back(); free_.pop_back();
            TRY(lnorm(bk.n1, cur, ln));
            TRY(conv(bk.qkv, ln, nullptr, qkv));
            if (!r.dry) {
                SwinAttnP a{};
                a.qkv = qkv; a.bias = bk.bias; a.out = att; a.B = B; a.H = Hp; a.W = Wp; a.heads = n.cfg.num_heads; a.D = n.D;
                a.ldq = n.ldq; a.ldo = n.lda; a.shift = (j & 1) ? 4 : 0; a.scale = 1.0f / sqrtf((float)n.D);
                TRY(launch_swin_attention(a, r.s));
            }
            TRY(conv(bk.proj, att, cur, mid));
            TRY(lnorm(bk.n2, mid, ln));
            TRY(conv(bk.fc1, ln, nullptr, hid, EP_GELU));
            TRY(conv(bk.fc2, hid, mid, nxt));
            free_.push_back(mid);
            if (cur != x) free_.push_back(cur);
            cur = nxt;
        }
        half_t* y = free_.back(); free_.pop_back();
        TRY(resi(L.conv, cur, x, y));
        free_.push_back(x);
        if (cur != x) free_.push_back(cur);
        x = y;
    }
    TRY(lnorm(n.norm, x, ln));
    half_t* trunk = free_.back();
    TRY(resi(n.after, ln, feat, trunk));
    TRY(conv(n.before, trunk, nullptr, c1));
    TRY(lrelu(c1, M * 64, 0.01f));
    if (r.dry) return 0;

    auto tail = [&](const ConvW& w, const half_t* src, int hh, int ww, int upf, void* dst, int store) -> int {
        RrdbP p{};
        p.in = src; p.w = w.w; p.bias = w.b; p.out = dst;
        p.B = B; p.H = hh; p.W = ww; p.cin = 64; p.lda = 64; p.up = upf;
        p.ldo = store == RRDB_ST_F16 ? 64 : 0; p.n_real = w.cout; p.ep = store == RRDB_ST_F16 ? RRDB_EP_LRELU : RRDB_EP_NONE; p.store = store;
        p.alpha = 1.f; p.beta = 1.f;
        return launch_rrdb_conv(p, w.n_pad, r.s);
    };
    TRY(tail(n.up1, c1, 2 * Hp, 2 * Wp, 1, up[0], RRDB_ST_F16));
    const half_t* t = up[0];
    if (sc == 4) { TRY(tail(n.up2, t, 4 * Hp, 4 * Wp, 1, up[1], RRDB_ST_F16)); t = up[1]; }
    TRY(tail(n.hr, t, sc * Hp, sc * Wp, 0, up[2], RRDB_ST_F16));
    TRY(tail(n.last, up[2], sc * Hp, sc * Wp, 0, full, RRDB_ST_F32_NCHW));
    return launch_swin_output(full, out, out_u8, B, H * sc, W * sc, Hp * sc, Wp * sc, r.s);
}

static bool swinir_size_ok(const sdmi_swinir& n, int B, int H, int W) {
    if (B <= 0 || H < 8 || W < 8) return false;
    const long long M = (long long)B * rup(H, 8) * rup(W, 8);
    const long long widest = std::max<long long>({(long long)n.ldq, (long long)n.hid_pad, (long long)n.Cp, 64ll * n.cfg.scale * n.cfg.scale});
    return M * widest < (1ll << 31) - 256;
}

int64_t swinir_scratch_bytes(const sdmi_swinir* n, int B, int H, int W) {
    if (!n || !swinir_size_ok(*n, B, H, W)) return 0;
    Arena ar;
    ar.dry = true;
    Run dry(n->e, nullptr, true, &ar);
    if (swinir_pass(dry, *n, nullptr, 0, B, H, W, nullptr, 0) != 0) return 0;
    return (int64_t)ar.high;
}

int swinir_run(sdmi_swinir* n, const void* in, int in_u8, int B, int H, int W, void* out, int out_u8, hipStream_t s) {
    SDMI_REQUIRE(n && in && out, "null argument");
    sdmi_engine* e = n->e;
    SDMI_REQUIRE(B > 0 && H >= 8 && W >= 8, "image sides must be at least 8 (a smaller side cannot be reflect-padded to a window)");
    SDMI_REQUIRE(swinir_size_ok(*n, B, H, W), "image too large: every intermediate tensor must stay below 2^31 elements");
    SDMI_CHECK_HIP(hipSetDevice(e->device));
    const bool tiling = e->tiling;
    e->tiling = false;
    struct Restore { sdmi_engine* e; bool v; ~Restore() { e->tiling = v; } } restore{e, tiling};
    Run dry{e, s, true};
    e->arena.dry = true; e->arena.high = 0;
    const int rc = swinir_pass(dry, *n, in, in_u8, B, H, W, out, out_u8);
    e->arena.dry = false;
    TRY(rc);
    TRY(ensure_arena(e, e->arena.high, s));
    Run run{e, s, false};
    return swinir_pass(run, *n, in, in_u8, B, H, W, out, out_u8);
}

}

sdmi_swinir::~sdmi_swinir() {
    for (void* p : owned) (void)hipFree(p);
}

sdmi_compact::~sdmi_compact() {
    for (void* p : owned) (void)hipFree(p);
}

sdmi_esrgan::~sdmi_esrgan() {
    for (void* p : owned) (void)hipFree(p);
}

sdmi_engine::~sdmi_engine() {
    (void)hipSetDevice(device);
    (void)hipDeviceSynchronize();
    sdmi::free_raw(raw_unet);
    sdmi::free_raw(raw_vae);
    sdmi::free_raw(raw_clip[0]);
    sdmi::free_raw(raw_clip[1]);
    sdmi::ctx_free(this);
    for (void* p : owned) (void)hipFree(p);
    for (void* p : owned_vae) (void)hipFree(p);
    for (void* p : owned_hn) (void)hipFree(p);
    if (hn_ctx_scratch) (void)hipFree(hn_ctx_scratch);
    if (arena.base) (void)hipFree(arena.base);
    for (auto& a : aux_arenas) if (a.base) (void)hipFree(a.base);
    for (hipStream_t st : aux_streams) (void)hipStreamDestroy(st);
    for (hipEvent_t ev : ev_join) (void)hipEventDestroy(ev);
    if (ev_fork) (void)hipEventDestroy(ev_fork);
}

#ifndef __HIP__
#include "rrdb.hip"
#include "compact.hip"
#include "swinir.hip"
#include "xattn_chain.hip"
#endif
```

### stable-diffusion-webui_amd/csrc/engine.h

```cpp
#pragma once
#include "common.h"
#include "../../include/sdmi.h"

#include <cstdlib>
#include <map>
#include <memory>
#include <string>
#include <vector>

namespace sdmi {

struct RawTensor {
    void* ptr = nullptr;
    int dtype = 0;
    std::vector<int64_t> shape;
    size_t bytes = 0;
};

struct ConvW {
    half_t* w = nullptr;
    float* b = nullptr;
    int cin = 0, cin_pad = 0, cout = 0, n_pad = 0, taps = 1;
    bool geglu = false;
    mutable half_t* w_ln = nullptr;
// ... 6 lines not shown
    float* b = nullptr;
    int c = 0;
};

struct ResW {
    NormW n1, n2;
    ConvW c1, c2, skip;
    bool has_skip = false;
    int cin = 0, cout = 0;
    int emb_off = -1;
};
struct TBlockW {
    NormW ln1, ln2, ln3;
    ConvW qk1;
    ConvW v1;
    ConvW o1, q2, k2, v2, o2, ff1, ff2;
    int ctx_slot = -1;
    mutable char* ff_packs = nullptr;
    mutable long ff_epoch = -1;
};
struct STW {
    NormW norm;
    ConvW proj_in, proj_out;
    std::vector<TBlockW> blocks;
    int ch = 0, heads = 0, dhead = 0;
};
struct UNetLayer {
    enum Kind { CONV_IN, RES, ST, DOWN, UP } kind;
    ResW res;
    STW st;
    ConvW conv;
    int c0 = 0, c1 = 0;
};
struct UNetW {
    sdmi_unet_config cfg{};
    ConvW te0, te2, le0, le2;
    ConvW emb_all;
    int emb_cols = 0;
    std::vector<std::vector<UNetLayer>> input, output;
    std::vector<UNetLayer> middle;
    NormW out_norm;
    ConvW out_conv;
    int n_ctx_slots = 0;
    bool ready = false;
};

struct VAEAttnW {
    NormW norm;
    ConvW qk, v, proj;
    int c = 0;
};
struct VAELevel {
    std::vector<ResW> blocks;
    ConvW resample;
    bool has_resample = false;
};
struct ClipLayerW {
    NormW ln1, ln2;
    ConvW qk, v, o, fc1, fc2;
};
struct ClipW {
    sdmi_clip_config cfg{};
    void* tok_emb = nullptr;
    int tok_dtype = 0;
    float* pos_emb = nullptr;
    std::vector<ClipLayerW> layers;
    NormW final_ln;
    half_t* text_proj = nullptr;
    int proj_dim = 0;
    bool configured = false, ready = false;
};

struct VAEW {
    sdmi_vae_config cfg{};
    float* pqc_w = nullptr;
    float* pqc_b = nullptr;
    ConvW d_conv_in, d_conv_out;
    ResW d_mid1, d_mid2;
    VAEAttnW d_attn;
    std::vector<VAELevel> d_up;
    NormW d_norm_out;
    ConvW e_conv_in, e_conv_out;
    ResW e_mid1, e_mid2;
    VAEAttnW e_attn;
    std::vector<VAELevel> e_down;
    NormW e_norm_out;
    bool has_encoder = false;
    bool ready = false;
};

struct HnOp {
    int kind = 0;
    ConvW lin;
    int act = 0;
    NormW ln;
};
struct HnModule {
    std::vector<HnOp> ops;
};
struct HnNet {
    float multiplier = 1.f;
    std::map<int, std::pair<HnModule, HnModule>> by_dim;
};

class Arena {
public:
    char* base = nullptr;
    size_t cap = 0, off = 0, high = 0;
    bool dry = false;
    void reset() { off = 0; }
    size_t mark() const { return off; }
    void rewind(size_t m) { off = m; }
    void* take(size_t bytes) {
        const size_t a = (off + 255) & ~size_t(255);
        off = a + bytes;
        if (off > high) high = off;
        if (dry) return (void*)(uintptr_t)(0x1000 + a);
        return base + a;
    }
};

}

struct sdmi_engine {
    int device = 0;
    std::map<std::string, sdmi::RawTensor> raw_unet, raw_vae;
    struct PackSite { half_t* dst; int O, cin, kh, Opad, cin_pad, geglu; };
    std::map<std::string, std::vector<PackSite>> unet_sites;
    struct VecSite { float* dst; int n, n_pad, geglu; };
    std::map<std::string, std::vector<VecSite>> unet_vec_sites;
    bool recording_unet_sites = false;
    std::vector<void*> owned;
    std::vector<void*> owned_vae;
    std::vector<void*>* alloc_sink = nullptr;
    std::vector<sdmi::HnNet> hypernets;
    std::vector<void*> owned_hn;
    char* hn_ctx_scratch = nullptr;
    size_t hn_ctx_scratch_bytes = 0;
    sdmi::UNetW unet;
    sdmi::VAEW vae;
    sdmi::ClipW clip[2];
    std::map<std::string, sdmi::RawTensor> raw_clip[2];
    sdmi::Arena arena;
    int n_streams = 1;
    int arena_reuse = 0;
    std::vector<hipStream_t> aux_streams;
    std::vector<sdmi::Arena> aux_arenas;
    std::vector<hipEvent_t> ev_join;
    hipEvent_t ev_fork = nullptr;
    bool force_generic = false;
    bool use_glds = true;
    float vae_stream_scale = 1.f;
    int ln_fold = 0;
    int fuse_rows = [] { const char* e = getenv("SDMI_FUSE_ROWS"); return e ? atoi(e) : 3; }();
    bool residual_fp32 = false;
    long weights_epoch = 0;
    bool cfg_pairs = false;
    bool uniform_t = false;
    bool auto_promises = false;
    bool tiling = false;
    bool trace = false;
    struct Tap { std::string name; const half_t* ptr; int B, H, W, C; };
    std::vector<Tap> taps;
    std::vector<const void*> control;
    std::vector<int64_t> control_numel;
    bool only_mid_control = false;
    half_t* ctx_f16 = nullptr;
    std::vector<half_t*> ctx_k;
    std::vector<half_t*> ctx_vt;
    std::vector<void*> ctx_owned;
    int ctx_B = 0, ctx_L = 0, ctx_Lpad = 0;
    bool ctx_valid = false;
    int* ctx_gate = nullptr;

    ~sdmi_engine();
};

struct sdmi_esrgan {
    struct Conv { half_t* w = nullptr; float* b = nullptr; int cin = 0, nout = 0, n_real = 0; };
    sdmi_engine* e = nullptr;
    int num_block = 0, in_ch = 0, scale = 0;
    int unshuffle = 1;
    int cin0 = 0;
    Conv first, body, up1, up2, hr, last;
    std::vector<Conv> rdb;
    std::vector<void*> owned;
    ~sdmi_esrgan();
};

struct sdmi_compact {
    struct Conv { half_t* w = nullptr; float* b = nullptr; float* slope = nullptr; };
    sdmi_engine* e = nullptr;
    int num_conv = 0, scale = 0;
    std::vector<Conv> convs;
    std::vector<void*> owned;
    ~sdmi_compact();
};

struct sdmi_swinir {
    struct Block {
        sdmi::NormW n1, n2;
        sdmi::ConvW qkv, proj, fc1, fc2;
        float* bias = nullptr;
    };
    struct Layer {
        std::vector<Block> blocks;
        sdmi::ConvW conv[3];
    };
    sdmi_engine* e = nullptr;
    sdmi_swinir_config cfg{};
    int C = 0, Cp = 0, D = 0, ldq = 0, lda = 0, hid_pad = 0;
    sdmi::ConvW first, after[3], before, up1, up2, hr, last;
    sdmi::NormW pe_norm, norm;
    std::vector<Layer> layers;
    std::vector<void*> owned;
    ~sdmi_swinir();
};
```

### stable-diffusion-webui_amd/csrc/norm.hip

```cpp
#include "common.h"
#include "prof.h"
#include <algorithm>
#include <cstdio>
#include <cstdlib>

namespace sdmi {

static constexpr int GN_MAX_C = 4096;

template <bool HILO = false>
__global__ __launch_bounds__(256) void gn_stats_kernel(const half_t* x0, const half_t* x1, int c0, int c1, int HW,
                                                       int groups, int rows_per_chunk, float* partial, const half_t* l0 = nullptr,
                                                       const half_t* l1 = nullptr) {
    __shared__ float s_sum[GN_MAX_C];
    __shared__ float s_sq[GN_MAX_C];
    const int C = c0 + c1, VP = C / 8;
    const int chunk = blockIdx.x, b = blockIdx.y, nchunk = gridDim.x;
    const int tid = threadIdx.x;
    const int TP = VP < 256 ? VP : 256;
    const int R = 256 / TP;
    const int p_begin = chunk * rows_per_chunk;
    const int p_end = min(HW, p_begin + rows_per_chunk);
    if (tid < TP * R) {
        const int tr = tid / TP, tc = tid - tr * TP;
        for (int cv = tc; cv < VP; cv += TP) {
            const int c = cv * 8;
            const half_t* src;
            int cc, ld;
            if (c < c0) { src = x0; cc = c; ld = c0; } else { src = x1; cc = c - c0; ld = c1; }
            const half_t* base = src + (long)b * HW * ld + cc;
            [[maybe_unused]] const half_t* lbase = HILO ? (c < c0 ? l0 : l1) + (long)b * HW * ld + cc : nullptr;
            float a[8], q[8], k[8];
#pragma unroll
            for (int e = 0; e < 8; ++e) { a[e] = 0.f; q[e] = 0.f; k[e] = 0.f; }
            int pix = p_begin + tr;
            const int n_t = pix < p_end ? (p_end - pix + R - 1) / R : 0;
            if (pix < p_end) {
                const h8 v = *reinterpret_cast<const h8*>(base + (long)pix * ld);
                h8 lv = {0, 0, 0, 0, 0, 0, 0, 0};
                if constexpr (HILO) lv = *reinterpret_cast<const h8*>(lbase + (long)pix * ld);
#pragma unroll
                for (int e = 0; e < 8; ++e) k[e] = HILO ? (float)v[e] + (float)lv[e] : (float)v[e];
                pix += R;
            }
            for (; pix + 3 * R < p_end; pix += 4 * R) {
                h8 v[4];
#pragma unroll
                for (int u = 0; u < 4; ++u) v[u] = *reinterpret_cast<const h8*>(base + (long)(pix + u * R) * ld);
#pragma unroll
                for (int u = 0; u < 4; ++u) {
                    h8 lv = {0, 0, 0, 0, 0, 0, 0, 0};
                    if constexpr (HILO) lv = *reinterpret_cast<const h8*>(lbase + (long)(pix + u * R) * ld);
#pragma unroll
                    for (int e = 0; e < 8; ++e) { const float f = (HILO ? (float)v[u][e] + (float)lv[e] : (float)v[u][e]) - k[e]; a[e] += f; q[e] = fmaf(f, f, q[e]); }
                }
            }
            for (; pix < p_end; pix += R) {
                const h8 v = *reinterpret_cast<const h8*>(base + (long)pix * ld);
                h8 lv = {0, 0, 0, 0, 0, 0, 0, 0};
                if constexpr (HILO) lv = *reinterpret_cast<const h8*>(lbase + (long)pix * ld);
#pragma unroll
                for (int e = 0; e < 8; ++e) { const float f = (HILO ? (float)v[e] + (float)lv[e] : (float)v[e]) - k[e]; a[e] += f; q[e] = fmaf(f, f, q[e]); }
            }
            const float inv = n_t > 0 ? 1.0f / (float)n_t : 0.f;
#pragma unroll
            for (int e = 0; e < 8; ++e) { s_sum[tr * C + c + e] = fmaf(a[e], inv, k[e]); s_sq[tr * C + c + e] = fmaxf(q[e] - a[e] * a[e] * inv, 0.f); }
        }
    }
    __syncthreads();
    {
        const int g = tid >> 3, l8 = tid & 7;
        const int cpg = C / groups, n = R * cpg;
        const int np = max(p_end - p_begin, 0);
        const float pv = g < groups ? s_sum[g * cpg] : 0.f;
        float a = 0.f;
        if (g < groups)
            for (int i = l8; i < n; i += 8) {
                const int r = i / cpg, c = g * cpg + (i - r * cpg);
                a = fmaf((float)max((np - r + R - 1) / R, 0), s_sum[r * C + c] - pv, a);
            }
        for (int off = 4; off > 0; off >>= 1) a += __shfl_xor(a, off);
        const float mean = np > 0 ? pv + a / ((float)np * (float)cpg) : 0.f;
        float q = 0.f;
        if (g < groups)
            for (int i = l8; i < n; i += 8) {
                const int r = i / cpg, c = g * cpg + (i - r * cpg);
                const float d = s_sum[r * C + c] - mean;
                q += fmaf((float)max((np - r + R - 1) / R, 0) * d, d, s_sq[r * C + c]);
            }
        for (int off = 4; off > 0; off >>= 1) q += __shfl_xor(q, off);
        if (g < groups && l8 == 0) {
            float* dst = partial + (((long)b * nchunk + chunk) * groups + g) * 2;
            dst[0] = mean; dst[1] = np > 0 ? q : 0.f;
        }
    }
}

__device__ __forceinline__ void gn_merge(float& n, float& mean, float& m2, float nb, float mb, float qb) {
    if (nb > 0.f) {
        const float r = nb / (n + nb), d = mb - mean;
        mean = fmaf(d, r, mean);
        m2 = (m2 + qb) + d * d * n * r;
        n += nb;
    }
}

template <bool HILO = false, int U = 8>
__global__ __launch_bounds__(256) void gn_apply_kernel(const half_t* x0, const half_t* x1, int c0, int c1, int HW,
                                                       int groups, int nchunk, int chunk_rows, int chunk_period, const float* partial,
                                                       const float* gamma, const float* beta, half_t* out, float eps,
                                                       int silu, const half_t* l0 = nullptr, const half_t* l1 = nullptr) {
    extern __shared__ __attribute__((aligned(16))) char smem[];
    __shared__ float s_mean[64], s_rstd[64];
    const int C = c0 + c1, VP = C / 8, cpg = C / groups;
    float* s_scale = reinterpret_cast<float*>(smem);
    float* s_shift = s_scale + C;
    const int b = blockIdx.y, tid = threadIdx.x;
    const int stride = (int)gridDim.x * 256;
    const int sp = stride / VP, sr = stride - sp * VP;
    const int spU = (U * stride) / VP, srU = U * stride - spU * VP;
    const int i_init = (int)blockIdx.x * 256 + tid;
    int pix_u[U], cv_u[U];
    unsigned iv[U];
    pix_u[0] = i_init / VP; cv_u[0] = i_init - pix_u[0] * VP; iv[0] = (unsigned)i_init;
#pragma unroll
    for (int u = 1; u < U; ++u) {
        iv[u] = iv[u - 1] + (unsigned)stride;
        pix_u[u] = pix_u[u - 1] + sp; cv_u[u] = cv_u[u - 1] + sr;
        if (cv_u[u] >= VP) { cv_u[u] -= VP; ++pix_u[u]; }
    }
    const half_t* x0b = x0 + (long)b * HW * c0;
    const half_t* x1b = x1 ? x1 + (long)b * HW * c1 : nullptr;
    [[maybe_unused]] const half_t* l0b = HILO ? l0 + (long)b * HW * c0 : nullptr;
    [[maybe_unused]] const half_t* l1b = (HILO && l1) ? l1 + (long)b * HW * c1 : nullptr;
    half_t* outb = out + (long)b * HW * C;
    h8 v[U];
    [[maybe_unused]] h8 lv[HILO ? U : 1];
    int cs[U];
    bool ok[U];
    auto request = [&]() {
#pragma unroll
        for (int u = 0; u < U; ++u) {
            ok[u] = pix_u[u] < HW;
            const unsigned pix = ok[u] ? (unsigned)pix_u[u] : 0u;
            const int c = (ok[u] ? cv_u[u] : 0) * 8;
            cs[u] = c;
            const half_t* src;
            unsigned cc, ld;
            if (c < c0) { src = x0b; cc = (unsigned)c; ld = (unsigned)c0; } else { src = x1b; cc = (unsigned)(c - c0); ld = (unsigned)c1; }
            v[u] = *reinterpret_cast<const h8*>(src + (__umul24(pix, ld) + cc));
            if constexpr (HILO) lv[u] = *reinterpret_cast<const h8*>((c < c0 ? l0b : l1b) + (__umul24(pix, ld) + cc));
        }
    };
    request();
    {
        const int g = tid >> 3, l8 = tid & 7;
        float n = 0.f, mean = 0.f, m2 = 0.f;
        if (g < groups)
            for (int ch = l8; ch < nchunk; ch += 8) {
                const float* src = partial + (((long)b * nchunk + ch) * groups + g) * 2;
                const int j = ch % chunk_period;
                gn_merge(n, mean, m2, (float)(max(min(chunk_rows, HW - j * chunk_rows), 0) * cpg), src[0], src[1]);
            }
        for (int off = 4; off > 0; off >>= 1) {
            const float nb = __shfl_xor(n, off), mb = __shfl_xor(mean, off), qb = __shfl_xor(m2, off);
            gn_merge(n, mean, m2, nb, mb, qb);
        }
        if (g < groups && l8 == 0) {
            s_mean[g] = mean;
            s_rstd[g] = rsqrtf(m2 / n + eps);
        }
    }
    __syncthreads();
    for (int c = tid; c < C; c += 256) {
        const int g = c / cpg;
        const float sc = s_rstd[g] * gamma[c];
        s_scale[c] = sc;
        s_shift[c] = beta[c] - s_mean[g] * sc;
    }
    __syncthreads();
    while (true) {
#pragma unroll
        for (int u = 0; u < U; ++u) {
            if (!ok[u]) continue;
            const f4 sa = *reinterpret_cast<const f4*>(&s_scale[cs[u]]), sb = *reinterpret_cast<const f4*>(&s_scale[cs[u] + 4]);
            const f4 ha = *reinterpret_cast<const f4*>(&s_shift[cs[u]]), hb = *reinterpret_cast<const f4*>(&s_shift[cs[u] + 4]);
            h8 o;
#pragma unroll
            for (int e = 0; e < 8; ++e) {
                const float sc = e < 4 ? sa[e] : sb[e - 4], sh = e < 4 ? ha[e] : hb[e - 4];
                float y = fmaf(HILO ? (float)v[u][e] + (float)lv[HILO ? u : 0][e] : (float)v[u][e], sc, sh);
                if (silu) y = y * __builtin_amdgcn_rcpf(1.0f + __expf(-y));
                o[e] = (half_t)y;
            }
            *reinterpret_cast<h8*>(outb + iv[u] * 8u) = o;
        }
#pragma unroll
        for (int u = 0; u < U; ++u) {
            iv[u] += (unsigned)(U * stride);
            pix_u[u] += spU; cv_u[u] += srU;
            if (cv_u[u] >= VP) { cv_u[u] -= VP; ++pix_u[u]; }
        }
        if (pix_u[0] >= HW) break;
        request();
    }
}

template <int NVT, bool HILO = false>
__global__ __launch_bounds__(256) void gn_fused_small_kernel(const half_t* x0, const half_t* x1, int c0, int c1, int HW, int groups,
                                                             const float* gamma, const float* beta, half_t* out, float eps, int silu,
                                                             const half_t* l0 = nullptr, const half_t* l1 = nullptr) {
    __shared__ float red[2][4];
    const int C = c0 + c1, cpg = C / groups, VW = cpg / 8;
    const int g = blockIdx.x, b = blockIdx.y, tid = threadIdx.x;
    const int cbase = g * cpg;
    const half_t* x0b = x0 + (long)b * HW * c0;
    const half_t* x1b = x1 ? x1 + (long)b * HW * c1 : nullptr;
    h8 v[NVT];
    [[maybe_unused]] h8 vl[HILO ? NVT : 1];
    [[maybe_unused]] const half_t* l0b = HILO ? l0 + (long)b * HW * c0 : nullptr;
    [[maybe_unused]] const half_t* l1b = (HILO && l1) ? l1 + (long)b * HW * c1 : nullptr;
    int off[NVT], cch[NVT];
    float s = 0.f;
    const int sp = 256 / VW, sr = 256 - sp * VW;
    int pix = tid / VW, vc = tid - pix * VW;
#pragma unroll
    for (int k = 0; k < NVT; ++k) {
        const bool ok = pix < HW;
        const int pp = ok ? pix : 0;
        const int c = cbase + vc * 8;
        off[k] = ok ? pp * C + c : -1;
        cch[k] = c;
        const half_t* src = c < c0 ? x0b + (long)pp * c0 + c : x1b + (long)pp * c1 + (c - c0);
        h8 z = {0, 0, 0, 0, 0, 0, 0, 0};
        v[k] = ok ? *reinterpret_cast<const h8*>(src) : z;
        if constexpr (HILO) {
            const half_t* srcl = c < c0 ? l0b + (long)pp * c0 + c : l1b + (long)pp * c1 + (c - c0);
            vl[k] = ok ? *reinterpret_cast<const h8*>(srcl) : z;
        }
        pix += sp; vc += sr;
        if (vc >= VW) { vc -= VW; ++pix; }
    }
#pragma unroll
    for (int k = 0; k < NVT; ++k)
#pragma unroll
        for (int e = 0; e < 8; ++e) s += HILO ? (float)v[k][e] + (float)vl[HILO ? k : 0][e] : (float)v[k][e];
    for (int o = 32; o > 0; o >>= 1) s += __shfl_xor(s, o);
    if ((tid & 63) == 0) red[0][tid >> 6] = s;
    __syncthreads();
    const float n = (float)cpg * (float)HW;
    const float mean = ((red[0][0] + red[0][1]) + (red[0][2] + red[0][3])) / n;
    float q = 0.f;
#pragma unroll
    for (int k = 0; k < NVT; ++k)
        if (off[k] >= 0) {
#pragma unroll
            for (int e = 0; e < 8; ++e) { const float d = (HILO ? (float)v[k][e] + (float)vl[HILO ? k : 0][e] : (float)v[k][e]) - mean; q = fmaf(d, d, q); }
        }
    for (int o = 32; o > 0; o >>= 1) q += __shfl_xor(q, o);
    if ((tid & 63) == 0) red[1][tid >> 6] = q;
    __syncthreads();
    const float rstd = rsqrtf(((red[1][0] + red[1][1]) + (red[1][2] + red[1][3])) / n + eps);
    half_t* outb = out + (long)b * HW * C;
#pragma unroll
    for (int k = 0; k < NVT; ++k) {
        if (off[k] < 0) continue;
        const int c = cch[k];
        const f4 g0 = *reinterpret_cast<const f4*>(gamma + c), g1 = *reinterpret_cast<const f4*>(gamma + c + 4);
        const f4 b0 = *reinterpret_cast<const f4*>(beta + c), b1 = *reinterpret_cast<const f4*>(beta + c + 4);
        h8 o;
#pragma unroll
        for (int e = 0; e < 8; ++e) {
            const float gm = e < 4 ? g0[e] : g1[e - 4], bt = e < 4 ? b0[e] : b1[e - 4];
            float y = fmaf(((HILO ? (float)v[k][e] + (float)vl[HILO ? k : 0][e] : (float)v[k][e]) - mean) * rstd, gm, bt);
            if (silu) y = y * __builtin_amdgcn_rcpf(1.0f + __expf(-y));
            o[e] = (half_t)y;
        }
        *reinterpret_cast<h8*>(outb + off[k]) = o;
    }
}

int g_gn_apply_blocks = 0;
int g_gn_small = [] { const char* e = getenv("SDMI_GN_SMALL"); return e ? atoi(e) : 1; }();

static inline int gn_chunks(int B, int HW) {
    int n = (1024 + B - 1) / B;
    if (n > HW / 32) n = HW / 32;
    if (n > 64) n = 64;
    if (n < 1) n = 1;
    return n;
}

long g_gn_band_elems = 0;
static inline long gn_band_limit() { return g_gn_band_elems > 0 ? g_gn_band_elems : (1L << 31); }
static inline int gn_row_limit() { return g_gn_band_elems > 0 ? (1 << 30) : (1 << 24); }
static int gn_bands(int HW, int C) {
    if ((long)HW * C < gn_band_limit() && HW < gn_row_limit()) return 1;
    for (int nb = 2; nb <= 8192; nb *= 2)
        if (HW % nb == 0 && (long)(HW / nb) * C < gn_band_limit() && HW / nb < gn_row_limit()) return nb;
    return 0;
}

int64_t groupnorm_ws_bytes(int B, int HW, int groups) {
    int64_t chunks = gn_chunks(B, HW);
    if ((long)HW * GN_MAX_C >= gn_band_limit() || HW >= gn_row_limit()) {
        int nb = 2;
        while (nb < 8192 && !((long)(HW / nb) * GN_MAX_C < gn_band_limit() && HW / nb < gn_row_limit())) nb *= 2;
        chunks = std::max<int64_t>(chunks, (int64_t)nb * 64);
    }
    return (int64_t)B * chunks * groups * 2 * sizeof(float);
}

static int groupnorm_banded(const half_t* x0, const half_t* x1, int c0, int c1, const float* gamma, const float* beta, half_t* out, int B,
                            int HW, int groups, float eps, bool silu, float* ws, hipStream_t s, int nb) {
    const int C = c0 + c1, HWb = HW / nb;
    const int nchunk_b = gn_chunks(1, HWb), rows = cdiv(HWb, nchunk_b), nchunk = nb * nchunk_b;
    SDMI_REQUIRE((int64_t)B * nchunk * groups * 2 * (int64_t)sizeof(float) <= groupnorm_ws_bytes(B, HW, groups),
                 "banded GroupNorm: partial sums exceed the workspace groupnorm_ws_bytes provisions");
    char pname[64];
    snprintf(pname, sizeof pname, "groupnorm_silu_banded B%d HW%d C%d x%d", B, HW, C, nb);
    ProfScope ps(pname, 0.0, 3.0 * B * (double)HW * C * 2.0, s);
    const long per_image = (long)nchunk * groups * 2;
    for (int b = 0; b < B; ++b)
        for (int k = 0; k < nb; ++k) {
            const long row0 = (long)b * HW + (long)k * HWb;
            hipLaunchKernelGGL(gn_stats_kernel<false>, dim3(nchunk_b, 1), dim3(256), 0, s, x0 + row0 * c0, x1 ? x1 + row0 * c1 : nullptr, c0, c1, HWb,
                               groups, rows, ws + b * per_image + (long)k * nchunk_b * groups * 2, nullptr, nullptr);
            SDMI_CHECK_HIP(hipGetLastError());
        }
    const long nvec = (long)HWb * (C / 8);
    const long trips = std::max<long>(1, cdiv(nvec, 2048L * 2048));
    int blocks = (int)std::max<long>(1, cdiv(nvec, 2048 * trips));
    if (g_gn_apply_blocks > 0) blocks = g_gn_apply_blocks;
    const size_t smem = (size_t)2 * C * sizeof(float);
    for (int b = 0; b < B; ++b)
        for (int k = 0; k < nb; ++k) {
            const long row0 = (long)b * HW + (long)k * HWb;
            hipLaunchKernelGGL((gn_apply_kernel<false, 8>), dim3(blocks, 1), dim3(256), smem, s, x0 + row0 * c0, x1 ? x1 + row0 * c1 : nullptr, c0, c1,
                               HWb, groups, nchunk, rows, nchunk_b, ws + b * per_image, gamma, beta, out + row0 * C, eps, silu ? 1 : 0, nullptr, nullptr);
            SDMI_CHECK_HIP(hipGetLastError());
        }
    return 0;
}


int launch_groupnorm(const half_t* x0, const half_t* x1, int c0, int c1, const float* gamma, const float* beta,
                     half_t* out, int B, int HW, int groups, float eps, bool silu, float* ws, hipStream_t s, int pre_nchunk,
                     const half_t* x0_lo, const half_t* x1_lo) {
    const int C = c0 + c1;
    const bool hilo = x0_lo != nullptr;
    SDMI_REQUIRE(!hilo || (x1 == nullptr) == (x1_lo == nullptr), "GroupNorm (hi, lo) input: both sources as pairs");
    SDMI_REQUIRE(C % 8 == 0 && c0 % 8 == 0, "GroupNorm channels must be multiples of 8");
    SDMI_REQUIRE(C <= GN_MAX_C && groups <= 32 && C % groups == 0, "GroupNorm: C <= 4096, groups <= 32, C % groups == 0");
    if (const int nb = gn_bands(HW, C); nb != 1) {
        SDMI_REQUIRE(nb > 1, "GroupNorm: an image of 2^31 elements or more must split into equal power-of-two bands of rows below that limit");
        SDMI_REQUIRE(!hilo && pre_nchunk <= 0, "GroupNorm beyond 2^31 elements per image: fp16 input with its own statistics pass only");
        return groupnorm_banded(x0, x1, c0, c1, gamma, beta, out, B, HW, groups, eps, silu, ws, s, nb);
    }
    char pname[64];
    {
        const int cpg = C / groups;
        const long nv = (long)HW * (cpg / 8);
        if (pre_nchunk <= 0 && g_gn_small && cpg % 8 == 0 && nv <= (hilo ? 6 : 12) * 256) {
            snprintf(pname, sizeof pname, "groupnorm_silu_fused B%d HW%d C%d", B, HW, C);
            ProfScope ps(pname, 0.0, (hilo ? 3.0 : 2.0) * B * (double)HW * C * 2.0, s);
            const dim3 grid(groups, B);
#define SDMI_GNS(NVT, HL) hipLaunchKernelGGL((gn_fused_small_kernel<NVT, HL>), grid, dim3(256), 0, s, x0, x1, c0, c1, HW, groups, gamma, beta, out, eps, silu ? 1 : 0, x0_lo, x1_lo)
            if (hilo) { if (nv <= 2 * 256) SDMI_GNS(2, true); else SDMI_GNS(6, true); }
            else if (nv <= 4 * 256) SDMI_GNS(4, false);
            else SDMI_GNS(12, false);
#undef SDMI_GNS
            SDMI_CHECK_HIP(hipGetLastError());
            return 0;
        }
    }
    const int nchunk = pre_nchunk > 0 ? pre_nchunk : gn_chunks(B, HW);
    const int rows = cdiv(HW, nchunk);
    snprintf(pname, sizeof pname, pre_nchunk > 0 ? "groupnorm_silu_apply B%d HW%d C%d" : "groupnorm_silu B%d HW%d C%d", B, HW, C);
    ProfScope ps(pname, 0.0, (pre_nchunk > 0 ? 2.0 : 3.0) * B * (double)HW * C * 2.0, s);
    if (pre_nchunk <= 0) {
        if (hilo) hipLaunchKernelGGL(gn_stats_kernel<true>, dim3(nchunk, B), dim3(256), 0, s, x0, x1, c0, c1, HW, groups, rows, ws, x0_lo, x1_lo);
        else hipLaunchKernelGGL(gn_stats_kernel<false>, dim3(nchunk, B), dim3(256), 0, s, x0, x1, c0, c1, HW, groups, rows, ws, nullptr, nullptr);
        SDMI_CHECK_HIP(hipGetLastError());
    }
    const long nvec = (long)HW * (C / 8);
    const long cap = std::max(1, 2048 / B);
    const long trips = std::max<long>(1, cdiv(nvec, 2048 * cap));
    int blocks = (int)std::max<long>(1, cdiv(nvec, 2048 * trips));
    if (g_gn_apply_blocks > 0) blocks = g_gn_apply_blocks;
    const size_t smem = (size_t)2 * C * sizeof(float);
    if (hilo)
        hipLaunchKernelGGL((gn_apply_kernel<true, 4>), dim3(blocks, B), dim3(256), smem, s, x0, x1, c0, c1, HW, groups, nchunk, rows, nchunk, ws, gamma,
                           beta, out, eps, silu ? 1 : 0, x0_lo, x1_lo);
    else
        hipLaunchKernelGGL((gn_apply_kernel<false, 8>), dim3(blocks, B), dim3(256), smem, s, x0, x1, c0, c1, HW, groups, nchunk, rows, nchunk, ws, gamma,
                           beta, out, eps, silu ? 1 : 0, nullptr, nullptr);
    SDMI_CHECK_HIP(hipGetLastError());
    return 0;
}

#define LN_VAL(r, k, e) (HILO ? (float)v[r][k][e] + (float)vl[HILO ? (r) : 0][HILO ? (k) : 0][e] : (float)v[r][k][e])
template <int K, int RPW, bool HILO = false>
__global__ __launch_bounds__(256) void layernorm_kernel(const half_t* x, const float* gamma, const float* beta,
                                                        half_t* out, long rows, int C, float eps, const half_t* xlo = nullptr) {
    const int lane = threadIdx.x & 63, wave = threadIdx.x >> 6;
    const long row0 = ((long)blockIdx.x * 4 + wave) * RPW;
    if (row0 >= rows) return;
    const int VP = C / 8;
    const float inv_c = 1.0f / (float)C;
    h8 v[RPW][K];
    [[maybe_unused]] h8 vl[HILO ? RPW : 1][HILO ? K : 1];
    float sum[RPW];
#pragma unroll
    for (int r = 0; r < RPW; ++r) {
        const long row = min(row0 + r, rows - 1);
        const half_t* src = x + row * C;
#pragma unroll
        for (int k = 0; k < K; ++k) {
            const int cv = lane + k * 64;
            h8 z = {0, 0, 0, 0, 0, 0, 0, 0};
            v[r][k] = cv < VP ? *reinterpret_cast<const h8*>(src + cv * 8) : z;
            if constexpr (HILO) vl[r][k] = cv < VP ? *reinterpret_cast<const h8*>(xlo + row * C + cv * 8) : z;
        }
    }
#pragma unroll
    for (int r = 0; r < RPW; ++r) {
        float a = 0.f;
#pragma unroll
        for (int k = 0; k < K; ++k)
#pragma unroll
            for (int e = 0; e < 8; ++e) a += LN_VAL(r, k, e);
        sum[r] = a;
    }
    for (int off = 32; off > 0; off >>= 1)
#pragma unroll
        for (int r = 0; r < RPW; ++r) sum[r] += __shfl_xor(sum[r], off);
    float mean[RPW], sq[RPW];
#pragma unroll
    for (int r = 0; r < RPW; ++r) {
        mean[r] = sum[r] * inv_c;
        float q = 0.f;
#pragma unroll
        for (int k = 0; k < K; ++k) {
            const int cv = lane + k * 64;
            if (cv < VP) {
#pragma unroll
                for (int e = 0; e < 8; ++e) { const float d = LN_VAL(r, k, e) - mean[r]; q = fmaf(d, d, q); }
            }
        }
        sq[r] = q;
    }
    for (int off = 32; off > 0; off >>= 1)
#pragma unroll
        for (int r = 0; r < RPW; ++r) sq[r] += __shfl_xor(sq[r], off);
#pragma unroll
    for (int k = 0; k < K; ++k) {
        const int cv = lane + k * 64;
        if (cv < VP) {
            const f4 g0 = *reinterpret_cast<const f4*>(gamma + cv * 8), g1 = *reinterpret_cast<const f4*>(gamma + cv * 8 + 4);
            const f4 b0 = *reinterpret_cast<const f4*>(beta + cv * 8), b1 = *reinterpret_cast<const f4*>(beta + cv * 8 + 4);
#pragma unroll
            for (int r = 0; r < RPW; ++r) {
                if (row0 + r >= rows) continue;
                const float rstd = rsqrtf(fmaf(sq[r], inv_c, eps));
                h8 o;
#pragma unroll
                for (int e = 0; e < 8; ++e) {
                    const float g = e < 4 ? g0[e] : g1[e - 4], bb = e < 4 ? b0[e] : b1[e - 4];
                    o[e] = (half_t)((LN_VAL(r, k, e) - mean[r]) * rstd * g + bb);
                }
                *reinterpret_cast<h8*>(out + (row0 + r) * C + cv * 8) = o;
            }
        }
    }
}

#undef LN_VAL

template <int K, int RPW>
__global__ __launch_bounds__(256) void ln_rowstats_kernel(const half_t* x, float* stats, long rows, int C, float eps) {
    const int lane = threadIdx.x & 63, wave = threadIdx.x >> 6;
    const long row0 = ((long)blockIdx.x * 4 + wave) * RPW;
    if (row0 >= rows) return;
    const int VP = C / 8;
    const float inv_c = 1.0f / (float)C;
    h8 v[RPW][K];
    float sum[RPW];
#pragma unroll
    for (int r = 0; r < RPW; ++r) {
        const long row = min(row0 + r, rows - 1);
        const half_t* src = x + row * C;
#pragma unroll
        for (int k = 0; k < K; ++k) {
            const int cv = lane + k * 64;
            h8 z = {0, 0, 0, 0, 0, 0, 0, 0};
            v[r][k] = cv < VP ? *reinterpret_cast<const h8*>(src + cv * 8) : z;
        }
    }
#pragma unroll
    for (int r = 0; r < RPW; ++r) {
        float a = 0.f;
#pragma unroll
        for (int k = 0; k < K; ++k)
#pragma unroll
            for (int e = 0; e < 8; ++e) a += (float)v[r][k][e];
        sum[r] = a;
    }
    for (int off = 32; off > 0; off >>= 1)
#pragma unroll
        for (int r = 0; r < RPW; ++r) sum[r] += __shfl_xor(sum[r], off);
    float mean[RPW], sq[RPW];
#pragma unroll
    for (int r = 0; r < RPW; ++r) {
        mean[r] = sum[r] * inv_c;
        float q = 0.f;
#pragma unroll
        for (int k = 0; k < K; ++k) {
            const int cv = lane + k * 64;
            if (cv < VP) {
#pragma unroll
                for (int e = 0; e < 8; ++e) { const float d = (float)v[r][k][e] - mean[r]; q = fmaf(d, d, q); }
            }
        }
        sq[r] = q;
    }
    for (int off = 32; off > 0; off >>= 1)
#pragma unroll
        for (int r = 0; r < RPW; ++r) sq[r] += __shfl_xor(sq[r], off);
    if (lane == 0) {
#pragma unroll
        for (int r = 0; r < RPW; ++r)
            if (row0 + r < rows) {
                stats[(row0 + r) * 2 + 0] = mean[r];
                stats[(row0 + r) * 2 + 1] = rsqrtf(fmaf(sq[r], inv_c, eps));
            }
    }
}
// ... 78 lines not shown
```

### stable-diffusion-webui_amd/csrc/xattn_chain.hip

```cpp
#include "common.h"
#include "prof.h"

#include <algorithm>
#include <cmath>

namespace sdmi {

#ifdef __HIP__
typedef const __attribute__((address_space(1))) void* xgptr_t;
typedef __attribute__((address_space(3))) void* xlptr_t;
#define XC_WAIT_VM3() asm volatile("s_waitcnt vmcnt(3) lgkmcnt(0)" ::: "memory")
#define XC_WAIT_VM0() asm volatile("s_waitcnt vmcnt(0) lgkmcnt(0)" ::: "memory")
#define XC_FENCE() asm volatile("" ::: "memory")
#define XC_REAL_BRANCH() asm volatile("")
#define XC_OPAQUE(x) asm volatile("" : "+v"(x))
#else
typedef const void* xgptr_t;
typedef void* xlptr_t;
#define XC_WAIT_VM3() ((void)0)
#define XC_WAIT_VM0() ((void)0)
#define XC_FENCE() ((void)0)
#define XC_REAL_BRANCH() ((void)0)
#define XC_OPAQUE(x) ((void)0)
#endif

constexpr int kXcC = 320, kXcD = 40, kXcRows = 128;
constexpr int kXcRowBytes = kXcC * 2;
constexpr int kXcImage = kXcRows * kXcRowBytes;
constexpr int kXcStage = 24 * 1024;
constexpr int kXcLds = kXcImage + 3 * kXcStage;

struct XattnP {
    const half_t* x;
    half_t* out;
    const float* gamma;
    const float* beta;
    const half_t* wq;
    const half_t* wo;
    const float* bo;
    const half_t* k;
    const half_t* vt;
    int rows_per_image;
    int L, Lpad;
    float eps, scale_log2, tau;
};

__device__ __forceinline__ int xc_img(int row, int col) { return row * kXcRowBytes + ((((col >> 3) ^ ((row >> 1) & 7))) << 4) + (col & 7) * 2; }

__global__ __launch_bounds__(512) void rowchain_xattn_kernel(const XattnP p) {
#ifdef __HIP__
    extern __shared__ __attribute__((aligned(16))) char smem[];
#else
    __shared__ __attribute__((aligned(16))) char smem[kXcLds];
#endif
    char* const img = smem;
    char* const ring = smem + kXcImage;
    const int tid = threadIdx.x, lane = tid & 63;
    const int wave = __builtin_amdgcn_readfirstlane(tid >> 6);
    const int wr = wave >> 2, wc = wave & 3;
    const int l16 = lane & 15, q4 = lane >> 4;
    const int lq = lane & 31, half = lane >> 5;
    const long row0 = (long)blockIdx.x * kXcRows;
    const int image = (int)(row0 / p.rows_per_image);
    const half_t* const kimg = p.k + (long)image * p.L * kXcC;
    const half_t* const vimg = p.vt + (long)image * kXcC * p.Lpad;
    const int nblk = (p.L + 31) >> 5;
    const int nsteps = 20 + 2 * nblk;

    auto stage_cols = [&](const half_t* w, int ld, int k0, char* buf) {
        int ln = lane;
        XC_OPAQUE(ln);
#pragma unroll
        for (int u = 0; u < 3; ++u) {
            const int pb = u * 8 + wave;
            const int n = pb * 16 + (ln >> 2);
            const int seg = (ln & 3) ^ (3 * ((n >> 3) & 1));
            const half_t* src = w + (long)min(n, kXcC - 1) * ld + k0 + seg * 8;
            __builtin_amdgcn_global_load_lds((xgptr_t)src, (xlptr_t)(buf + pb * 1024), 16, 0, 0);
        }
    };
    auto stage_keys = [&](int key0, char* buf) {
        int ln = lane;
        XC_OPAQUE(ln);
#pragma unroll
        for (int u = 0; u < 3; ++u) {
            const int pb = u * 8 + wave;
            const int pc = pb * 64 + ln;
            const int r = pc / 40, ps = pc - r * 40;
            const int rr = min(r, 31);
            const int key = min(key0 + rr, p.L - 1);
            const half_t* src = kimg + (long)key * kXcC + ((ps ^ ((rr >> 1) & 7)) << 3);
            __builtin_amdgcn_global_load_lds((xgptr_t)src, (xlptr_t)(buf + pb * 1024), 16, 0, 0);
        }
    };
    auto issue = [&](int seq) {
        if (seq >= nsteps) return;
        char* buf = ring + (seq % 3) * kXcStage;
        if (seq < 10) stage_cols(p.wq, kXcC, seq * 32, buf);
        else if (seq < 10 + 2 * nblk) {
            const int blk = (seq - 10) >> 1;
            if ((seq - 10) & 1) stage_cols(vimg, p.Lpad, blk * 32, buf);
            else stage_keys(blk * 32, buf);
        } else stage_cols(p.wo, kXcC, (seq - 10 - 2 * nblk) * 32, buf);
    };
    auto open_step = [&](int s) -> const char* {
        if (s + 1 < nsteps) XC_WAIT_VM3(); else XC_WAIT_VM0();
        __builtin_amdgcn_s_barrier();
        XC_FENCE();
        issue(s + 2);
        return ring + (s % 3) * kXcStage;
    };

    issue(0);
    issue(1);

    {
        const int sub = tid & 7;
        const float inv_c = 1.0f / (float)kXcC;
        h8 v[2][5];
#pragma unroll
        for (int ps = 0; ps < 2; ++ps) {
            const half_t* src = p.x + (row0 + ps * 64 + (tid >> 3)) * kXcC + sub * 8;
#pragma unroll
            for (int i = 0; i < 5; ++i) v[ps][i] = *reinterpret_cast<const h8*>(src + i * 64);
        }
#pragma unroll
        for (int ps = 0; ps < 2; ++ps) {
            const int row = ps * 64 + (tid >> 3);
            float a = 0.f;
#pragma unroll
            for (int i = 0; i < 5; ++i)
#pragma unroll
                for (int e = 0; e < 8; ++e) a += (float)v[ps][i][e];
            for (int off = 4; off > 0; off >>= 1) a += __shfl_xor(a, off);
            const float mean = a * inv_c;
            float sq = 0.f;
#pragma unroll
            for (int i = 0; i < 5; ++i)
#pragma unroll
                for (int e = 0; e < 8; ++e) { const float d = (float)v[ps][i][e] - mean; sq = fmaf(d, d, sq); }
            for (int off = 4; off > 0; off >>= 1) sq += __shfl_xor(sq, off);
            const float rstd = rsqrtf(fmaf(sq, inv_c, p.eps));
#pragma unroll
            for (int i = 0; i < 5; ++i) {
                const int c0 = (i * 8 + sub) * 8;
                const f4 g0 = *reinterpret_cast<const f4*>(p.gamma + c0), g1 = *reinterpret_cast<const f4*>(p.gamma + c0 + 4);
                const f4 b0 = *reinterpret_cast<const f4*>(p.beta + c0), b1 = *reinterpret_cast<const f4*>(p.beta + c0 + 4);
                h8 o;
#pragma unroll
                for (int e = 0; e < 8; ++e) {
                    const float g = e < 4 ? g0[e] : g1[e - 4], bb = e < 4 ? b0[e] : b1[e - 4];
                    o[e] = (half_t)(((float)v[ps][i][e] - mean) * rstd * g + bb);
                }
                *reinterpret_cast<h8*>(img + xc_img(row, c0)) = o;
            }
        }
    }

    const int a_off = (64 * wr + l16) * kXcRowBytes, a_sw = (l16 >> 1) & 7;
    const int w_off = (80 * wc + l16) * 64 + ((q4 ^ (3 * (l16 >> 3))) << 4);
    f4 acc[4][5];
    auto zero_acc = [&]() {
#pragma unroll
        for (int mi = 0; mi < 4; ++mi)
#pragma unroll
            for (int j = 0; j < 5; ++j) acc[mi][j] = f4{0.f, 0.f, 0.f, 0.f};
    };
    auto gemm_step = [&](const char* buf, int kc) {
        h8 af[4], wf[5];
#pragma unroll
        for (int j = 0; j < 5; ++j) wf[j] = *reinterpret_cast<const h8*>(buf + w_off + j * 1024);
#pragma unroll
        for (int mi = 0; mi < 4; ++mi) af[mi] = *reinterpret_cast<const h8*>(img + a_off + mi * 16 * kXcRowBytes + (((kc * 4 + q4) ^ a_sw) << 4));
#pragma unroll
        for (int mi = 0; mi < 4; ++mi)
#pragma unroll
            for (int j = 0; j < 5; ++j) acc[mi][j] = __builtin_amdgcn_mfma_f32_16x16x32_f16(wf[j], af[mi], acc[mi][j], 0, 0, 0);
    };

    zero_acc();
    int s = 0;
#pragma unroll 1
    for (; s < 10; ++s) {
        const char* buf = open_step(s);
        gemm_step(buf, s);
    }

    const char* kb = open_step(s++);
#pragma unroll
    for (int mi = 0; mi < 4; ++mi)
#pragma unroll
        for (int j = 0; j < 5; ++j) {
            const h4 hv = {(half_t)acc[mi][j][0], (half_t)acc[mi][j][1], (half_t)acc[mi][j][2], (half_t)acc[mi][j][3]};
            *reinterpret_cast<h4*>(img + xc_img(64 * wr + 16 * mi + l16, 80 * wc + 16 * j + 4 * q4)) = hv;
        }
    XC_FENCE();
    __builtin_amdgcn_wave_barrier();
    f16v o[4][2];
    float m_run[4];
    h8 pb[4][2];
// ... 183 lines not shown
```

### stable-diffusion-webui_amd/ops.py

```python
from __future__ import annotations

import ctypes as C
from typing import Optional

import torch

from . import _lib
from ._lib import lib, check, ptr, stream_ptr, ConvDesc, F16, F32, EP_OUT_F32, EP_GEGLU, EP_NCHW, EP_BIAS_ROW


def _rup(x, m):
    return (x + m - 1) // m * m


def attention(q: torch.Tensor, k: torch.Tensor, v: torch.Tensor, heads: int, scale: Optional[float] = None) -> torch.Tensor:
    _lib.require_device()
    assert q.dtype == torch.float16 and k.dtype == torch.float16 and v.dtype == torch.float16
    b, n, c = q.shape
    m = k.shape[1]
    d = c // heads
    q, k, v = [t if t.stride(-1) == 1 and t.stride(0) == t.shape[1] * t.stride(1) else t.contiguous() for t in (q, k, v)]
    out = torch.empty((b, n, c), dtype=torch.float16, device=q.device)
    scale = d ** -0.5 if scale is None else scale
    if heads == 1 and d > 160 and d % 64 == 0:
# ... 19 lines not shown
    return out


def pack_conv_weight(w: torch.Tensor, geglu: bool = False, pad: int = 64) -> torch.Tensor:
    _lib.require_device()
    w = w.contiguous()
    if w.dim() == 2:
        w = w[:, :, None, None]
    o, i, kh, kw = w.shape
    o_pad, i_pad = _rup(o, pad), _rup(i, pad)
    out = torch.empty((o_pad, kh * kw, i_pad), dtype=torch.float16, device=w.device)
    check(lib.sdmi_pack_conv_weight(ptr(w), _lib.dtype_code(w), ptr(out), o, i, kh, kw, o_pad, i_pad, 1 if geglu else 0,
                                    stream_ptr()), "pack_conv_weight")
    return out


def pack_bias(b: Optional[torch.Tensor], n_pad: int, geglu: bool = False) -> Optional[torch.Tensor]:
    if b is None:
        return None
    bf = b.float()
    if geglu:
        o = bf.shape[0]
        half = o // 2
        idx = torch.arange(o, device=bf.device)
        g, r = idx // 64, idx % 64
        src = torch.where(r < 32, g * 32 + r, half + g * 32 + (r - 32))
        bf = bf[src]
    out = torch.zeros(n_pad, dtype=torch.float32, device=b.device)
    out[: bf.shape[0]] = bf
    return out


def conv_gemm(a0: torch.Tensor, w_packed: torch.Tensor, *, a1: Optional[torch.Tensor] = None, bias=None, rowbias=None,
              resid=None, taps: int = 9, stride: int = 1, pad: int = 1, up: bool = False, Ho=None, Wo=None,
              geglu: bool = False, out_f32: bool = False, nchw_real: int = 0, bias_row: bool = False, alpha: float = 1.0,
              impl: str = "mfma", transpose: bool = False, wrap: bool = False) -> torch.Tensor:
    _lib.require_device()
    assert a0.dtype == torch.float16 and a0.is_contiguous()
    b, hi, wi, c0 = a0.shape
    c1 = a1.shape[3] if a1 is not None else 0
    n = w_packed.shape[0]
    if Ho is None:
        if up:
            Ho, Wo = 2 * hi, 2 * wi
        elif taps == 9:
            p2 = 2 if pad else 1
            Ho, Wo = (hi + p2 - 3) // stride + 1, (wi + p2 - 3) // stride + 1
        else:
            Ho, Wo = hi, wi
    d = ConvDesc()
    d.a0, d.a1, d.w = a0.data_ptr(), (a1.data_ptr() if a1 is not None else None), w_packed.data_ptr()
    d.bias = bias.data_ptr() if bias is not None else None
    d.rowbias = rowbias.data_ptr() if rowbias is not None else None
    d.resid = resid.data_ptr() if resid is not None else None
    d.c0, d.c1, d.lda0, d.lda1 = c0, c1, c0, c1
    d.B, d.Hi, d.Wi, d.Ho, d.Wo = b, hi, wi, Ho, Wo
    d.taps, d.stride, d.pad, d.up = taps, stride, pad if taps == 9 else 0, 1 if up else 0
    d.N = n
    flags = 0
    n_out = n
    if geglu:
        flags |= EP_GEGLU
        n_out = n // 2
    if bias_row:
        flags |= EP_BIAS_ROW
    if wrap:
        flags |= _lib.EP_WRAP
    if nchw_real:
        flags |= EP_NCHW
        out = torch.empty((b, nchw_real, Ho, Wo), dtype=torch.float32, device=a0.device)
        d.n_real = nchw_real
    elif out_f32:
        flags |= EP_OUT_F32
        out = torch.empty((b, Ho, Wo, n_out), dtype=torch.float32, device=a0.device)
    elif transpose:
        flags |= _lib.EP_TRANSPOSE
        out = torch.empty((b, n_out, Ho * Wo), dtype=torch.float16, device=a0.device)
    else:
        out = torch.empty((b, Ho, Wo, n_out), dtype=torch.float16, device=a0.device)
    d.out = out.data_ptr()
    d.ldo = Ho * Wo if transpose else n_out
    d.ldr = resid.shape[-1] if resid is not None else 0
    d.flags = flags
    d.alpha = alpha
    d.batch = 1
    d.force_generic = {"mfma": 0, "generic": 1, "mfma_reg": 2}[impl]
    wsb = lib.sdmi_conv_splitk_workspace_bytes(b * Ho * Wo, n, taps * (c0 + c1), 1)
    if wsb and not geglu and not nchw_real:
        ws = torch.empty(wsb, dtype=torch.uint8, device=a0.device)
        d.splitk_workspace, d.splitk_workspace_bytes = ws.data_ptr(), wsb
    check(lib.sdmi_conv_gemm(C.byref(d), stream_ptr()), "sdmi_conv_gemm")
    return out


def groupnorm(x0: torch.Tensor, gamma: torch.Tensor, beta: torch.Tensor, *, x1: Optional[torch.Tensor] = None,
              groups: int = 32, eps: float = 1e-5, silu: bool = True) -> torch.Tensor:
    _lib.require_device()
    b, h, w, c0 = x0.shape
    c1 = x1.shape[3] if x1 is not None else 0
    out = torch.empty((b, h, w, c0 + c1), dtype=torch.float16, device=x0.device)
    wsb = lib.sdmi_groupnorm_workspace_bytes(b, h * w, groups)
    ws = torch.empty(max(wsb, 16), dtype=torch.uint8, device=x0.device)
    check(lib.sdmi_groupnorm(ptr(x0), ptr(x1), c0, c1, ptr(gamma.float().contiguous()), ptr(beta.float().contiguous()),
                             ptr(out), b, h * w, groups, float(eps), 1 if silu else 0, ptr(ws), wsb, stream_ptr()), "sdmi_groupnorm")
    return out


def layernorm(x: torch.Tensor, gamma: torch.Tensor, beta: torch.Tensor, eps: float = 1e-5) -> torch.Tensor:
    _lib.require_device()
    c = x.shape[-1]
    x = x.contiguous()
    out = torch.empty_like(x)
    check(lib.sdmi_layernorm(ptr(x), ptr(gamma.float().contiguous()), ptr(beta.float().contiguous()), ptr(out),
                             x.numel() // c, c, float(eps), stream_ptr()), "sdmi_layernorm")
    return out


def rowchain_ff_pack(w1: torch.Tensor, b1, w2: torch.Tensor) -> torch.Tensor:
    _lib.require_device()
    hidden, c = w2.shape[1], w2.shape[0]
    w1, w2 = w1.half().contiguous(), w2.half().contiguous()
    b1 = b1.float().contiguous() if b1 is not None else None
    packs = torch.empty(int(lib.sdmi_rowchain_ff_pack_bytes(c, hidden)), dtype=torch.uint8, device=w1.device)
    check(lib.sdmi_rowchain_ff_pack(ptr(w1), ptr(b1) if b1 is not None else None, ptr(w2), ptr(packs), c, hidden, stream_ptr()),
          "sdmi_rowchain_ff_pack")
    return packs


def rowchain_ff(x: torch.Tensor, gamma, beta, packs: torch.Tensor, b2, hidden: int, eps: float = 1e-5) -> torch.Tensor:
    _lib.require_device()
    c = x.shape[-1]
    x = x.contiguous()
    out = torch.empty_like(x)
    b2 = b2.float().contiguous() if b2 is not None else None
    check(lib.sdmi_rowchain_ff(ptr(x), ptr(out), ptr(gamma.float().contiguous()), ptr(beta.float().contiguous()), ptr(packs),
                               ptr(b2) if b2 is not None else None, x.numel() // c, c, hidden, float(eps), stream_ptr()), "sdmi_rowchain_ff")
    return out


def xattn_chain(x: torch.Tensor, gamma, beta, wq: torch.Tensor, wo: torch.Tensor, bo, k: torch.Tensor, vt: torch.Tensor, L: int,
                heads: int = 8, eps: float = 1e-5) -> torch.Tensor:
    _lib.require_device()
    images, rpi, c = x.shape
    x = x.contiguous()
    out = torch.empty_like(x)
    wq, wo, k, vt = wq.half().contiguous(), wo.half().contiguous(), k.half().contiguous(), vt.half().contiguous()
    bo = bo.float().contiguous() if bo is not None else None
    check(lib.sdmi_xattn_chain(ptr(x), ptr(out), ptr(gamma.float().contiguous()), ptr(beta.float().contiguous()), ptr(wq), ptr(wo),
                               ptr(bo) if bo is not None else None, ptr(k), ptr(vt), images * rpi, rpi, c, heads, int(L), vt.shape[-1],
                               float(eps), stream_ptr()), "sdmi_xattn_chain")
    return out


def philox_randn(shape, seed: int, offset: int, device) -> torch.Tensor:
    _lib.require_device()
    out = torch.empty(tuple(shape), dtype=torch.float32, device=device)
    check(lib.sdmi_philox_randn(ptr(out), out.numel(), C.c_uint64(seed & 0xFFFFFFFFFFFFFFFF), C.c_uint32(offset), stream_ptr()),
          "sdmi_philox_randn")
    return out


def lincomb(out: torch.Tensor, terms, coefs) -> torch.Tensor:
    _lib.require_device()
    n = len(terms)
    assert 1 <= n <= 6 and len(coefs) == n
    for t in terms:
        assert t.dtype == torch.float32 and t.is_contiguous() and t.numel() == out.numel()
    assert out.dtype == torch.float32 and out.is_contiguous()
    tarr = (C.c_void_p * n)(*[t.data_ptr() for t in terms])
    carr = (C.c_float * n)(*[float(c) for c in coefs])
    check(lib.sdmi_lincomb(ptr(out), tarr, carr, n, out.numel(), stream_ptr()), "sdmi_lincomb")
    return out


def mask_blend(x: torch.Tensor, init: torch.Tensor, mask: torch.Tensor, nmask: torch.Tensor) -> torch.Tensor:
    _lib.require_device()
    m = mask.to(x.device, torch.float32).expand_as(x).contiguous()
    nm = nmask.to(x.device, torch.float32).expand_as(x).contiguous()
    init = init.to(x.device, torch.float32).expand_as(x).contiguous()
    check(lib.sdmi_mask_blend(ptr(x), ptr(init), ptr(m), ptr(nm), x.numel(), stream_ptr()), "sdmi_mask_blend")
    return x


def latent_resize(x: torch.Tensor, size, mode: str = "bilinear", antialias: bool = False) -> torch.Tensor:
    _lib.require_device()
    x = x.float().contiguous()
    b, c, hi, wi = x.shape
    ho, wo = int(size[0]), int(size[1])
    out = torch.empty((b, c, ho, wo), dtype=torch.float32, device=x.device)
    code = {"nearest": 0, "nearest-exact": 1, "bilinear": 2, "bicubic": 3}[mode]
    if antialias:
        if mode not in ("bilinear", "bicubic"):
            raise ValueError("antialias is defined for the bilinear and bicubic modes")
        code += 2
    check(lib.sdmi_latent_resize(ptr(x), ptr(out), b * c, hi, wi, ho, wo, code, stream_ptr()), "sdmi_latent_resize")
    return out


def image_to_u8(img: torch.Tensor) -> torch.Tensor:
    _lib.require_device()
    img = img.float().contiguous()
    b, c, h, w = img.shape
    out = torch.empty((b, h, w, c), dtype=torch.uint8, device=img.device)
    check(lib.sdmi_image_to_u8(ptr(img), ptr(out), b, c, h, w, stream_ptr()), "sdmi_image_to_u8")
    return out


def pack_rrdb_weight(w: torch.Tensor, nout: Optional[int] = None) -> torch.Tensor:
    _lib.require_device()
    w = w.contiguous()
    o, i, kh, kw = w.shape
    assert (kh, kw) == (3, 3)
    nout = nout or (32 if o <= 32 else 64)
    cin = _rup(i, 32)
    out = torch.empty((nout, 9, cin), dtype=torch.float16, device=w.device)
    check(lib.sdmi_pack_conv_weight(ptr(w), _lib.dtype_code(w), ptr(out), o, i, 3, 3, nout, cin, 0, stream_ptr()), "pack_rrdb_weight")
    return out


def rrdb_conv(x: torch.Tensor, w_packed: torch.Tensor, bias: Optional[torch.Tensor] = None, *, cin: Optional[int] = None,
              out: Optional[torch.Tensor] = None, out_offset: int = 0, n_real: Optional[int] = None, ep: str = "lrelu",
              alpha: float = 1.0, r1: Optional[torch.Tensor] = None, beta: float = 1.0, r2: Optional[torch.Tensor] = None,
              up: bool = False, store: str = "f16") -> torch.Tensor:
    _lib.require_device()
    assert x.dtype == torch.float16 and x.is_contiguous() and w_packed.dtype == torch.float16 and w_packed.is_contiguous()
    b, hi, wi, lda = x.shape
    nout, cin_w = w_packed.shape[0], w_packed.shape[2]
    cin = cin_w if cin is None else cin
    assert cin == cin_w, "the packed weights fix the number of input channels"
    ho, wo = (2 * hi, 2 * wi) if up else (hi, wi)
    n_real = nout if n_real is None else n_real
    d = _lib.RrdbDesc()
    d.in_, d.w = x.data_ptr(), w_packed.data_ptr()
    d.bias = bias.data_ptr() if bias is not None else None
    if bias is not None:
        assert bias.dtype == torch.float32 and bias.numel() == nout
    for name, r in (("r1", r1), ("r2", r2)):
        if r is not None:
            assert r.dtype == torch.float16 and r.is_contiguous() and tuple(r.shape[:3]) == (b, ho, wo)
            setattr(d, name, r.data_ptr())
            setattr(d, "ld" + name, r.shape[3])
    d.B, d.H, d.W, d.cin, d.lda, d.up = b, ho, wo, cin, lda, 1 if up else 0
    d.nout, d.n_real = nout, n_real
    d.ep = {"none": _lib.RRDB_EP_NONE, "lrelu": _lib.RRDB_EP_LRELU, "res1": _lib.RRDB_EP_RES1, "res2": _lib.RRDB_EP_RES2}[ep]
    d.store = {"f16": _lib.RRDB_ST_F16, "f32_nchw": _lib.RRDB_ST_F32_NCHW, "u8_hwc": _lib.RRDB_ST_U8_HWC}[store]
    d.alpha, d.beta = alpha, beta
    if store == "f16":
        if out is None:
            out = torch.empty((b, ho, wo, out_offset + n_real), dtype=torch.float16, device=x.device)
        assert out.dtype == torch.float16 and out.is_contiguous() and tuple(out.shape[:3]) == (b, ho, wo)
        assert out_offset + n_real <= out.shape[3]
        d.out, d.ldo = out.data_ptr() + 2 * out_offset, out.shape[3]
    elif store == "f32_nchw":
        out = torch.empty((b, n_real, ho, wo), dtype=torch.float32, device=x.device)
        d.out = out.data_ptr()
    else:
        out = torch.empty((b, ho, wo, n_real), dtype=torch.uint8, device=x.device)
        d.out = out.data_ptr()
    check(lib.sdmi_rrdb_conv(C.byref(d), stream_ptr()), "sdmi_rrdb_conv")
    return out


def pack_compact_weight(w: torch.Tensor) -> torch.Tensor:
    _lib.require_device()
    w = w.contiguous()
    o, i, kh, kw = w.shape
    assert (kh, kw) == (3, 3) and o <= 64 and i <= 64
    cin = _rup(i, 32)
    out = torch.empty((64, 9, cin), dtype=torch.float16, device=w.device)
    check(lib.sdmi_pack_conv_weight(ptr(w), _lib.dtype_code(w), ptr(out), o, i, 3, 3, 64, cin, 0, stream_ptr()), "pack_compact_weight")
    return out


def compact_conv(x: torch.Tensor, w_packed: torch.Tensor, bias: Optional[torch.Tensor] = None, *, slope: Optional[torch.Tensor] = None,
                 out: Optional[torch.Tensor] = None, n_real: Optional[int] = None, ep: str = "prelu", r: int = 0,
                 base: Optional[torch.Tensor] = None, store: str = "f32_nchw", grid_cap: int = 0) -> torch.Tensor:
    _lib.require_device()
    assert x.dtype == torch.float16 and x.is_contiguous() and w_packed.dtype == torch.float16 and w_packed.is_contiguous()
    b, h, w, lda = x.shape
    d = _lib.CompactDesc()
    d.in_, d.w = x.data_ptr(), w_packed.data_ptr()
    if bias is not None:
        assert bias.dtype == torch.float32 and bias.numel() == 64
        d.bias = bias.data_ptr()
    if slope is not None:
        assert slope.dtype == torch.float32 and slope.numel() == 64
        d.slope = slope.data_ptr()
    d.B, d.H, d.W, d.cin, d.lda = b, h, w, w_packed.shape[2], lda
    d.ep = {"none": _lib.COMPACT_EP_NONE, "prelu": _lib.COMPACT_EP_PRELU, "tail": _lib.COMPACT_EP_TAIL}[ep]
    d.grid_cap = grid_cap
    if ep == "tail":
        d.r, d.n_real = r, (3 * r * r if n_real is None else n_real)
        if base is not None:
            assert base.is_contiguous() and base.dtype in (torch.uint8, torch.float32)
            assert tuple(base.shape) == ((b, h, w, 3) if base.dtype == torch.uint8 else (b, 3, h, w))
            d.base, d.base_u8 = base.data_ptr(), 1 if base.dtype == torch.uint8 else 0
        rs = max(r, 0)
        out = (torch.empty((b, h * rs, w * rs, 3), dtype=torch.uint8, device=x.device) if store == "u8_hwc"
               else torch.empty((b, 3, h * rs, w * rs), dtype=torch.float32, device=x.device))
        d.out, d.out_u8 = out.data_ptr(), 1 if store == "u8_hwc" else 0
    else:
        d.n_real = 64 if n_real is None else n_real
        if out is None:
            out = torch.empty((b, h, w, d.n_real), dtype=torch.float16, device=x.device)
        assert out.dtype == torch.float16 and out.is_contiguous() and tuple(out.shape[:3]) == (b, h, w)
        d.out, d.ldo = out.data_ptr(), out.shape[3]
# ... 34 lines not shown
```

Baseline: 20.92.

## Fuse GroupNorm apply, proj_in, LayerNorm and QK/V projections into one kernel

Adds a row-chain kernel for C=320 transformer blocks that applies GroupNorm from precomputed chunk statistics, runs proj_in, LayerNorm1 and the QK and V projections. It writes x0, QK and transposed V directly, and reuses GroupNorm stats from a prior kernel when available. The default fuse_rows mask now includes bit 4, so the path runs by default for the first transformer block at the highest-resolution level. This removes several intermediate HBM round trips and kernel launches. In exchange it adds complex hand-scheduled LDS code and can only be used under narrow shape conditions.

```diff
diff --git a/include/sdmi.h b/include/sdmi.h
--- a/include/sdmi.h
+++ b/include/sdmi.h
@@ -79,6 +79,8 @@
                    void* out_f16, int B, int HW, int groups, float eps, int silu,
                    void* workspace_f32, int64_t workspace_bytes, void* stream);
 int64_t sdmi_groupnorm_workspace_bytes(int B, int HW, int groups);
+int sdmi_groupnorm_stats(const void* x_f16, int C, int B, int HW, int groups, void* workspace_f32, int64_t workspace_bytes,
+                         int* nchunk_out, void* stream);
 
 int sdmi_layernorm(const void* x, const void* gamma_f32, const void* beta_f32, void* out_f16,
                    int64_t rows, int C, float eps, void* stream);
@@ -92,6 +94,11 @@
 int sdmi_xattn_chain(const void* x_f16, void* out_f16, const void* ln_gamma_f32, const void* ln_beta_f32, const void* wq_f16,
                      const void* wo_f16, const void* bo_f32_or_null, const void* k_f16, const void* vt_f16, int64_t rows,
                      int rows_per_image, int C, int heads, int L, int Lpad, float eps, void* stream);
+
+int sdmi_qkv_chain(const void* h_f16, const void* gn_partial_f32, int nchunk, const void* gn_gamma_f32, const void* gn_beta_f32, float gn_eps,
+                   const void* w_in_f16, const void* b_in_f32_or_null, const void* ln_gamma_f32, const void* ln_beta_f32, float ln_eps,
+                   const void* wqk_f16, const void* bqk_f32_or_null, const void* wv_f16, void* x0_f16, void* qk_f16, void* vt_f16,
+                   int64_t rows, int rows_per_image, int C, int vt_ld, void* stream);
 
 
 int sdmi_philox_randn(void* out_f32, int64_t n, uint64_t seed, uint32_t offset, void* stream);
diff --git a/stable-diffusion-webui_amd/_lib.py b/stable-diffusion-webui_amd/_lib.py
--- a/stable-diffusion-webui_amd/_lib.py
+++ b/stable-diffusion-webui_amd/_lib.py
@@ -118,11 +118,13 @@
     "sdmi_pack_conv_weight": (_i, [_vp, _i, _vp, _i, _i, _i, _i, _i, _i, _i, _vp]),
     "sdmi_groupnorm": (_i, [_vp, _vp, _i, _i, _vp, _vp, _vp, _i, _i, _i, _f, _i, _vp, _i64, _vp]),
     "sdmi_groupnorm_workspace_bytes": (_i64, [_i, _i, _i]),
+    "sdmi_groupnorm_stats": (_i, [_vp, _i, _i, _i, _i, _vp, _i64, _vp, _vp]),
     "sdmi_layernorm": (_i, [_vp, _vp, _vp, _vp, _i64, _i, _f, _vp]),
     "sdmi_rowchain_ff_pack_bytes": (_i64, [_i, _i]),
     "sdmi_rowchain_ff_pack": (_i, [_vp, _vp, _vp, _vp, _i, _i, _vp]),
     "sdmi_rowchain_ff": (_i, [_vp, _vp, _vp, _vp, _vp, _vp, _i64, _i, _i, _f, _vp]),
     "sdmi_xattn_chain": (_i, [_vp, _vp, _vp, _vp, _vp, _vp, _vp, _vp, _vp, _i64, _i, _i, _i, _i, _i, _f, _vp]),
+    "sdmi_qkv_chain": (_i, [_vp, _vp, _i, _vp, _vp, _f, _vp, _vp, _vp, _vp, _f, _vp, _vp, _vp, _vp, _vp, _vp, _i64, _i, _i, _i, _vp]),
     "sdmi_philox_randn": (_i, [_vp, _i64, C.c_uint64, C.c_uint32, _vp]),
     "sdmi_slerp": (_i, [_vp, _vp, _vp, _f, _i, _i, _i, _vp, _vp]),
     "sdmi_cfg_prepare_input": (_i, [_vp, _vp, _vp, _i, _i, _i, _i64, _vp]),
diff --git a/stable-diffusion-webui_amd/csrc/capi.cpp b/stable-diffusion-webui_amd/csrc/capi.cpp
--- a/stable-diffusion-webui_amd/csrc/capi.cpp
+++ b/stable-diffusion-webui_amd/csrc/capi.cpp
@@ -258,12 +258,29 @@
                               hidden, eps, (hipStream_t)stream);
     API_GUARD_END
 }
+int sdmi_groupnorm_stats(const void* x, int C, int B, int HW, int groups, void* ws, int64_t ws_bytes, int* nchunk_out, void* stream) {
+    API_GUARD_BEGIN
+    SDMI_REQUIRE(x && nchunk_out, "null argument");
+    SDMI_REQUIRE(ws && ws_bytes >= groupnorm_ws_bytes(B, HW, groups), "groupnorm workspace too small");
+    return launch_groupnorm_stats((const half_t*)x, C, B, HW, groups, (float*)ws, (hipStream_t)stream, nchunk_out);
+    API_GUARD_END
+}
 int sdmi_xattn_chain(const void* x, void* out, const void* g, const void* b, const void* wq, const void* wo, const void* bo, const void* k,
                      const void* vt, int64_t rows, int rows_per_image, int C, int heads, int L, int Lpad, float eps, void* stream) {
     API_GUARD_BEGIN
     return launch_xattn_chain((const half_t*)x, (half_t*)out, (const float*)g, (const float*)b, (const half_t*)wq, (const half_t*)wo,
                               (const float*)bo, (const half_t*)k, (const half_t*)vt, (long)rows, rows_per_image, C, heads, L, Lpad, eps,
                               (hipStream_t)stream);
+    API_GUARD_END
+}
+int sdmi_qkv_chain(const void* h, const void* gn_partial, int nchunk, const void* gn_g, const void* gn_b, float gn_eps, const void* w_in,
+                   const void* b_in, const void* ln_g, const void* ln_b, float ln_eps, const void* wqk, const void* bqk, const void* wv, void* x0,
+                   void* qk, void* vt, int64_t rows, int rows_per_image, int C, int vt_ld, void* stream) {
+    API_GUARD_BEGIN
+    return launch_qkv_chain((const half_t*)h, (const float*)gn_partial, nchunk, (const float*)gn_g, (const float*)gn_b, gn_eps,
+                            (const half_t*)w_in, (const float*)b_in, (const float*)ln_g, (const float*)ln_b, ln_eps, (const half_t*)wqk,
+                            (const float*)bqk, (const half_t*)wv, (half_t*)x0, (half_t*)qk, (half_t*)vt, (long)rows, rows_per_image, C, vt_ld,
+                            (hipStream_t)stream);
     API_GUARD_END
 }
 
diff --git a/stable-diffusion-webui_amd/csrc/chain_tile.h b/stable-diffusion-webui_amd/csrc/chain_tile.h
--- /dev/null
+++ b/stable-diffusion-webui_amd/csrc/chain_tile.h
@@ -0,0 +1,58 @@
+#pragma once
+#include "common.h"
+
+namespace sdmi {
+
+#ifdef __HIP__
+typedef const __attribute__((address_space(1))) void* xgptr_t;
+typedef __attribute__((address_space(3))) void* xlptr_t;
+#define XC_WAIT_VM3() asm volatile("s_waitcnt vmcnt(3) lgkmcnt(0)" ::: "memory")
+#define XC_WAIT_VM0() asm volatile("s_waitcnt vmcnt(0) lgkmcnt(0)" ::: "memory")
+#define XC_WAIT_LGKM() asm volatile("s_waitcnt lgkmcnt(0)" ::: "memory")
+#define XC_FENCE() asm volatile("" ::: "memory")
+#define XC_REAL_BRANCH() asm volatile("")
+#define XC_OPAQUE(x) asm volatile("" : "+v"(x))
+#else
+typedef const void* xgptr_t;
+typedef void* xlptr_t;
+#define XC_WAIT_VM3() ((void)0)
+#define XC_WAIT_VM0() ((void)0)
+#define XC_WAIT_LGKM() ((void)0)
+#define XC_FENCE() ((void)0)
+#define XC_REAL_BRANCH() ((void)0)
+#define XC_OPAQUE(x) ((void)0)
+#endif
+
+constexpr int kXcC = 320, kXcD = 40, kXcRows = 128;
+constexpr int kXcRowBytes = kXcC * 2;
+constexpr int kXcImage = kXcRows * kXcRowBytes;
+constexpr int kXcStage = 24 * 1024;
+constexpr int kXcLds = kXcImage + 3 * kXcStage;
+
+__device__ __forceinline__ int xc_img(int row, int col) { return row * kXcRowBytes + ((((col >> 3) ^ ((row >> 1) & 7))) << 4) + (col & 7) * 2; }
+
+__device__ __forceinline__ void gn_merge(float& n, float& mean, float& m2, float nb, float mb, float qb) {
+    if (nb > 0.f) {
+        const float r = nb / (n + nb), d = mb - mean;
+        mean = fmaf(d, r, mean);
+        m2 = (m2 + qb) + d * d * n * r;
+        n += nb;
+    }
+}
+
+__device__ __forceinline__ void gn_merge_chunks(const float* partial_b, int nchunk, int chunk_period, int chunk_rows, int HW, int cpg, int groups,
+                                                int g, int l8, float& n, float& mean, float& m2) {
+    n = 0.f; mean = 0.f; m2 = 0.f;
+    if (g < groups)
+        for (int ch = l8; ch < nchunk; ch += 8) {
+            const float* src = partial_b + ((long)ch * groups + g) * 2;
+            const int j = ch % chunk_period;
+            gn_merge(n, mean, m2, (float)(max(min(chunk_rows, HW - j * chunk_rows), 0) * cpg), src[0], src[1]);
+        }
+    for (int off = 4; off > 0; off >>= 1) {
+        const float nb = __shfl_xor(n, off), mb = __shfl_xor(mean, off), qb = __shfl_xor(m2, off);
+        gn_merge(n, mean, m2, nb, mb, qb);
+    }
+}
+
+}
diff --git a/stable-diffusion-webui_amd/csrc/common.h b/stable-diffusion-webui_amd/csrc/common.h
--- a/stable-diffusion-webui_amd/csrc/common.h
+++ b/stable-diffusion-webui_amd/csrc/common.h
@@ -176,6 +176,11 @@
                        const float* bo, const half_t* k, const half_t* vt, long rows, int rows_per_image, int C, int heads, int L, int Lpad,
                        float eps, hipStream_t s);
 
+int launch_qkv_chain(const half_t* h, const float* gn_partial, int nchunk, const float* gn_gamma, const float* gn_beta, float gn_eps,
+                     const half_t* w_in, const float* b_in, const float* ln_gamma, const float* ln_beta, float ln_eps, const half_t* wqk,
+                     const float* bqk, const half_t* wv, half_t* x0, half_t* qk, half_t* vt, long rows, int rows_per_image, int C, int vt_ld,
+                     hipStream_t s);
+
 enum { RRDB_EP_NONE = 0, RRDB_EP_LRELU = 1,
        RRDB_EP_RES1 = 2,
        RRDB_EP_RES2 = 3 };
@@ -237,6 +242,7 @@
                      half_t* out, int B, int HW, int groups, float eps, bool silu, float* ws, hipStream_t s, int pre_nchunk = 0,
                      const half_t* x0_lo = nullptr, const half_t* x1_lo = nullptr);
 int64_t groupnorm_ws_bytes(int B, int HW, int groups);
+int launch_groupnorm_stats(const half_t* x, int C, int B, int HW, int groups, float* ws, hipStream_t s, int* nchunk_out);
 int launch_layernorm(const half_t* x, const float* gamma, const float* beta, half_t* out, int64_t rows, int C,
                      float eps, hipStream_t s, const half_t* x_lo = nullptr);
 int launch_ln_rowstats(const half_t* x, float* stats, int64_t rows, int C, float eps, hipStream_t s);
diff --git a/stable-diffusion-webui_amd/csrc/engine.cpp b/stable-diffusion-webui_amd/csrc/engine.cpp
--- a/stable-diffusion-webui_amd/csrc/engine.cpp
+++ b/stable-diffusion-webui_amd/csrc/engine.cpp
@@ -657,13 +657,39 @@
     const size_t mk = r.ar->mark();
     const bool acc = r.acc();
     const size_t MC = M * C;
+    const bool fold_any = e->ln_fold && !acc && !hn_has_dim(e, C) && !e->force_generic && e->use_glds && g_vt_mode == 1 && HW == Npad && HW % 4 == 0;
+    const bool qchain = (e->fuse_rows & 4) && !e->ln_fold && !acc && !e->force_generic && e->use_glds && rowchain_supports(C) && HW % 128 == 0 &&
+                        e->n_streams <= 1 && !hn_has_dim(e, C) && st.heads == 8 && st.dhead == 40 && HW == Npad && !st.blocks.empty() &&
+                        st.proj_in.taps == 1 && st.proj_in.cin_pad == C && st.proj_in.n_pad == C && st.blocks[0].qk1.cin_pad == C &&
+                        st.blocks[0].qk1.n_pad == 2 * C && st.blocks[0].v1.cin_pad == C && st.blocks[0].v1.n_pad == C;
+    half_t* cur = nullptr;
+    half_t *qk_front = nullptr, *vt_front = nullptr;
+    if (qchain) {
+        const TBlockW& b0 = st.blocks[0];
+        float* ws = r.F(groupnorm_ws_bytes(B1, HW, 32) / sizeof(float));
+        cur = reuse ? cur_pre : r.S(M * C);
+        qk_front = r.H(M * 2 * C);
+        vt_front = r.H((size_t)B * C * Npad);
+        if (!r.dry) {
+            SDMI_REQUIRE(st.norm.c == C, "GroupNorm channel mismatch");
+            const float* partial = r.st_ws;
+            int nchunk = r.st_nchunk;
+            if (!(nchunk > 0 && r.st_tensor == x)) {
+                TRY(launch_groupnorm_stats(x, C, B1, HW, 32, ws, r.s, &nchunk));
+                partial = ws;
+            }
+            TRY(launch_qkv_chain(x, partial, nchunk, st.norm.g, st.norm.b, 1e-6f, st.proj_in.w, st.proj_in.b, b0.ln1.g, b0.ln1.b, 1e-5f, b0.qk1.w,
+                                 b0.qk1.b, b0.v1.w, cur, qk_front, vt_front, (long)M1, HW, C, Npad, r.s));
+        }
+        r.st_tensor = nullptr; r.st_nchunk = 0;
+    } else {
     half_t* n0 = r.H(M * C);
     TRY(run_gn(r, st.norm, x, nullptr, C, 0, B1, HW, 1e-6f, false, n0, r.lo(x, MC)));
-    half_t* cur = reuse ? cur_pre : r.S(M * C);
-    const bool fold_any = e->ln_fold && !acc && !hn_has_dim(e, C) && !e->force_generic && e->use_glds && g_vt_mode == 1 && HW == Npad && HW % 4 == 0;
+    cur = reuse ? cur_pre : r.S(M * C);
     r.lnp_want = fold_any && e->ln_fold >= 2;
     TRY(run_linear(r, st.proj_in, n0, (int)M1, nullptr, cur, C, 1.f, false, nullptr, r.lo(cur, MC)));
     if (reuse) r.ar->rewind(mk);
+    }
     int bi = 0, blk = 0;
     for (const TBlockW& b : st.blocks) {
         const std::string bname = name + ".transformer_blocks." + std::to_string(bi++);
@@ -679,9 +705,13 @@
             a1 = r.H(M * C);
             TRY(run_attn(r, qk, qk + C, vt, a1, B, st.heads, HW, HW, st.dhead, 2 * C, 2 * C, Npad, C));
         }
-        half_t* n1 = fold ? nullptr : r.H(M * C);
-        if (!fold) TRY(run_ln(r, b.ln1, cur, M1, n1, r.lo(cur, MC)));
+        const bool front = qchain && blk == 0;
+        half_t* n1 = (fold || front) ? nullptr : r.H(M * C);
+        if (!fold && !front) TRY(run_ln(r, b.ln1, cur, M1, n1, r.lo(cur, MC)));
         if (fold) {
+        } else if (front) {
+            a1 = r.H(M * C);
+            TRY(run_attn(r, qk_front, qk_front + C, vt_front, a1, B1, st.heads, HW, HW, st.dhead, 2 * C, 2 * C, Npad, C));
         } else if (!hn_has_dim(e, C)) {
             half_t* qk = r.H(M * 2 * C);
             TRY(run_linear(r, b.qk1, n1, (int)M1, nullptr, qk, 2 * C));
@@ -2319,4 +2349,5 @@
 #include "compact.hip"
 #include "swinir.hip"
 #include "xattn_chain.hip"
+#include "qkv_chain.hip"
 #endif
diff --git a/stable-diffusion-webui_amd/csrc/engine.h b/stable-diffusion-webui_amd/csrc/engine.h
--- a/stable-diffusion-webui_amd/csrc/engine.h
+++ b/stable-diffusion-webui_amd/csrc/engine.h
@@ -182,7 +182,7 @@
     bool use_glds = true;
     float vae_stream_scale = 1.f;
     int ln_fold = 0;
-    int fuse_rows = [] { const char* e = getenv("SDMI_FUSE_ROWS"); return e ? atoi(e) : 3; }();
+    int fuse_rows = [] { const char* e = getenv("SDMI_FUSE_ROWS"); return e ? atoi(e) : 7; }();
     bool residual_fp32 = false;
     long weights_epoch = 0;
     bool cfg_pairs = false;
diff --git a/stable-diffusion-webui_amd/csrc/norm.hip b/stable-diffusion-webui_amd/csrc/norm.hip
--- a/stable-diffusion-webui_amd/csrc/norm.hip
+++ b/stable-diffusion-webui_amd/csrc/norm.hip
@@ -1,4 +1,4 @@
-#include "common.h"
+#include "chain_tile.h"
 #include "prof.h"
 #include <algorithm>
 #include <cstdio>
@@ -96,15 +96,6 @@
     }
 }
 
-__device__ __forceinline__ void gn_merge(float& n, float& mean, float& m2, float nb, float mb, float qb) {
-    if (nb > 0.f) {
-        const float r = nb / (n + nb), d = mb - mean;
-        mean = fmaf(d, r, mean);
-        m2 = (m2 + qb) + d * d * n * r;
-        n += nb;
-    }
-}
-
 template <bool HILO = false, int U = 8>
 __global__ __launch_bounds__(256) void gn_apply_kernel(const half_t* x0, const half_t* x1, int c0, int c1, int HW,
                                                        int groups, int nchunk, int chunk_rows, int chunk_period, const float* partial,
@@ -155,17 +146,8 @@
     request();
     {
         const int g = tid >> 3, l8 = tid & 7;
-        float n = 0.f, mean = 0.f, m2 = 0.f;
-        if (g < groups)
-            for (int ch = l8; ch < nchunk; ch += 8) {
-                const float* src = partial + (((long)b * nchunk + ch) * groups + g) * 2;
-                const int j = ch % chunk_period;
-                gn_merge(n, mean, m2, (float)(max(min(chunk_rows, HW - j * chunk_rows), 0) * cpg), src[0], src[1]);
-            }
-        for (int off = 4; off > 0; off >>= 1) {
-            const float nb = __shfl_xor(n, off), mb = __shfl_xor(mean, off), qb = __shfl_xor(m2, off);
-            gn_merge(n, mean, m2, nb, mb, qb);
-        }
+        float n, mean, m2;
+        gn_merge_chunks(partial + (long)b * nchunk * groups * 2, nchunk, chunk_period, chunk_rows, HW, cpg, groups, g, l8, n, mean, m2);
         if (g < groups && l8 == 0) {
             s_mean[g] = mean;
             s_rstd[g] = rsqrtf(m2 / n + eps);
@@ -344,6 +326,27 @@
 }
 
 
+static int gn_stats_pass(const half_t* x0, const half_t* x1, int c0, int c1, int B, int HW, int groups, int nchunk, float* ws, hipStream_t s,
+                         const half_t* x0_lo, const half_t* x1_lo) {
+    const int rows = cdiv(HW, nchunk);
+    if (x0_lo) hipLaunchKernelGGL(gn_stats_kernel<true>, dim3(nchunk, B), dim3(256), 0, s, x0, x1, c0, c1, HW, groups, rows, ws, x0_lo, x1_lo);
+    else hipLaunchKernelGGL(gn_stats_kernel<false>, dim3(nchunk, B), dim3(256), 0, s, x0, x1, c0, c1, HW, groups, rows, ws, nullptr, nullptr);
+    SDMI_CHECK_HIP(hipGetLastError());
+    return 0;
+}
+
+int launch_groupnorm_stats(const half_t* x, int C, int B, int HW, int groups, float* ws, hipStream_t s, int* nchunk_out) {
+    SDMI_REQUIRE(C % 8 == 0 && C <= GN_MAX_C && groups <= 32 && C % groups == 0, "GroupNorm: C % 8 == 0, C <= 4096, groups <= 32, C % groups == 0");
+    SDMI_REQUIRE(gn_bands(HW, C) == 1, "GroupNorm statistics pass: images below 2^31 elements only");
+    const int nchunk = gn_chunks(B, HW);
+    char pname[64];
+    snprintf(pname, sizeof pname, "groupnorm_stats B%d HW%d C%d", B, HW, C);
+    ProfScope ps(pname, 0.0, B * (double)HW * C * 2.0, s);
+    if (int rc = gn_stats_pass(x, nullptr, C, 0, B, HW, groups, nchunk, ws, s, nullptr, nullptr)) return rc;
+    *nchunk_out = nchunk;
+    return 0;
+}
+
 int launch_groupnorm(const half_t* x0, const half_t* x1, int c0, int c1, const float* gamma, const float* beta,
                      half_t* out, int B, int HW, int groups, float eps, bool silu, float* ws, hipStream_t s, int pre_nchunk,
                      const half_t* x0_lo, const half_t* x1_lo) {
@@ -378,11 +381,8 @@
     const int rows = cdiv(HW, nchunk);
     snprintf(pname, sizeof pname, pre_nchunk > 0 ? "groupnorm_silu_apply B%d HW%d C%d" : "groupnorm_silu B%d HW%d C%d", B, HW, C);
     ProfScope ps(pname, 0.0, (pre_nchunk > 0 ? 2.0 : 3.0) * B * (double)HW * C * 2.0, s);
-    if (pre_nchunk <= 0) {
-        if (hilo) hipLaunchKernelGGL(gn_stats_kernel<true>, dim3(nchunk, B), dim3(256), 0, s, x0, x1, c0, c1, HW, groups, rows, ws, x0_lo, x1_lo);
-        else hipLaunchKernelGGL(gn_stats_kernel<false>, dim3(nchunk, B), dim3(256), 0, s, x0, x1, c0, c1, HW, groups, rows, ws, nullptr, nullptr);
-        SDMI_CHECK_HIP(hipGetLastError());
-    }
+    if (pre_nchunk <= 0)
+        if (int rc = gn_stats_pass(x0, x1, c0, c1, B, HW, groups, nchunk, ws, s, x0_lo, x1_lo)) return rc;
     const long nvec = (long)HW * (C / 8);
     const long cap = std::max(1, 2048 / B);
     const long trips = std::max<long>(1, cdiv(nvec, 2048 * cap));
diff --git a/stable-diffusion-webui_amd/csrc/qkv_chain.hip b/stable-diffusion-webui_amd/csrc/qkv_chain.hip
--- /dev/null
+++ b/stable-diffusion-webui_amd/csrc/qkv_chain.hip
@@ -0,0 +1,344 @@
+#include "chain_tile.h"
+#include "prof.h"
+
+#include <algorithm>
+#include <type_traits>
+
+namespace sdmi {
+
+constexpr int kQcTables = kXcLds;
+constexpr int kQcLds = kXcLds + (2 * kXcC + 64) * 4;
+constexpr int kQcSteps = 40;
+
+#ifndef SDMI_QKV_SKIP
+#define SDMI_QKV_SKIP 0
+#endif
+
+struct QkvP {
+    const half_t* h;
+    const float* partial;
+    const float* gn_gamma;
+    const float* gn_beta;
+    const half_t* w_in;
+    const float* b_in;
+    const float* ln_gamma;
+    const float* ln_beta;
+    const half_t* wqk;
+    const float* bqk;
+    const half_t* wv;
+    half_t* x0;
+    half_t* qk;
+    half_t* vt;
+    int rows_per_image, nchunk, chunk_rows, vt_ld;
+    float gn_eps, ln_eps;
+};
+
+__global__ __launch_bounds__(512) void rowchain_qkv_kernel(const QkvP p) {
+#ifdef __HIP__
+    extern __shared__ __attribute__((aligned(16))) char smem[];
+#else
+    __shared__ __attribute__((aligned(16))) char smem[kQcLds];
+#endif
+    char* const img = smem;
+    char* const ring = smem + kXcImage;
+    float* const s_scale = reinterpret_cast<float*>(smem + kQcTables);
+    float* const s_shift = s_scale + kXcC;
+    float* const s_mean = s_shift + kXcC;
+    float* const s_rstd = s_mean + 32;
+    const int tid = threadIdx.x, lane = tid & 63;
+    const int wave = __builtin_amdgcn_readfirstlane(tid >> 6);
+    const int wr = wave >> 2, wc = wave & 3;
+    const int l16 = lane & 15, q4 = lane >> 4;
+    const long row0 = (long)blockIdx.x * kXcRows;
+    const int image = (int)(row0 / p.rows_per_image);
+    const int tok0 = (int)(row0 - (long)image * p.rows_per_image);
+
+    auto issue = [&](int seq) {
+        if (seq >= kQcSteps || (SDMI_QKV_SKIP & 4)) return;
+        char* buf = ring + (seq % 3) * kXcStage;
+        const int m = seq / 10;
+        const half_t* w = m == 0 ? p.w_in : m == 1 ? p.wqk : m == 2 ? p.wqk + kXcC * kXcC : p.wv;
+        const int k0 = (seq - m * 10) * 32;
+        int ln = lane;
+        XC_OPAQUE(ln);
+#pragma unroll
+        for (int u = 0; u < 3; ++u) {
+            const int pb = u * 8 + wave;
+            const int n = pb * 16 + (ln >> 2);
+            const int seg = (ln & 3) ^ (3 * ((n >> 3) & 1));
+            const half_t* src = w + (long)min(n, kXcC - 1) * kXcC + k0 + seg * 8;
+            __builtin_amdgcn_global_load_lds((xgptr_t)src, (xlptr_t)(buf + pb * 1024), 16, 0, 0);
+        }
+    };
+    auto open_step = [&](int s) -> const char* {
+        if (s + 1 < kQcSteps) XC_WAIT_VM3(); else XC_WAIT_VM0();
+        __builtin_amdgcn_s_barrier();
+        XC_FENCE();
+        issue(s + 2);
+        return ring + (s % 3) * kXcStage;
+    };
+    auto tile_barrier = [&]() {
+        XC_WAIT_LGKM();
+        __builtin_amdgcn_s_barrier();
+        XC_FENCE();
+    };
+
+    issue(0);
+    issue(1);
+
+    const int sub = tid & 7;
+    {
+        h8 v[2][5];
+#pragma unroll
+        for (int ps = 0; ps < 2; ++ps) {
+            const half_t* src = p.h + (row0 + ps * 64 + (tid >> 3)) * kXcC + sub * 8;
+#pragma unroll
+            for (int i = 0; i < 5; ++i) v[ps][i] = *reinterpret_cast<const h8*>(src + i * 64);
+        }
+        {
+            const int g = tid >> 3;
+            const int HW = p.rows_per_image;
+            float n, mean, m2;
+            gn_merge_chunks(p.partial + (long)image * p.nchunk * 64, p.nchunk, p.nchunk, p.chunk_rows, HW, kXcC / 32, 32, g, sub, n, mean, m2);
+            if (g < 32 && sub == 0) {
+                s_mean[g] = mean;
+                s_rstd[g] = rsqrtf(m2 / n + p.gn_eps);
+            }
+        }
+        __syncthreads();
+        if (tid < kXcC) {
+            const int g = tid / (kXcC / 32);
+            const float sc = s_rstd[g] * p.gn_gamma[tid];
+            s_scale[tid] = sc;
+            s_shift[tid] = p.gn_beta[tid] - s_mean[g] * sc;
+        }
+        __syncthreads();
+#pragma unroll
+        for (int ps = 0; ps < 2; ++ps) {
+            const int row = ps * 64 + (tid >> 3);
+#pragma unroll
+            for (int i = 0; i < 5; ++i) {
+                const int c0 = (i * 8 + sub) * 8;
+                const f4 sa = *reinterpret_cast<const f4*>(&s_scale[c0]), sb = *reinterpret_cast<const f4*>(&s_scale[c0 + 4]);
+                const f4 ha = *reinterpret_cast<const f4*>(&s_shift[c0]), hb = *reinterpret_cast<const f4*>(&s_shift[c0 + 4]);
+                h8 o;
+#pragma unroll
+                for (int e = 0; e < 8; ++e) o[e] = (half_t)fmaf((float)v[ps][i][e], e < 4 ? sa[e] : sb[e - 4], e < 4 ? ha[e] : hb[e - 4]);
+                *reinterpret_cast<h8*>(img + xc_img(row, c0)) = o;
+            }
+        }
+    }
+
+    const int a_off = (64 * wr + l16) * kXcRowBytes, a_sw = (l16 >> 1) & 7;
+    const int w_off = (80 * wc + l16) * 64 + ((q4 ^ (3 * (l16 >> 3))) << 4);
+    f4 acc[4][5];
+    auto zero_acc = [&]() {
+#pragma unroll
+        for (int mi = 0; mi < 4; ++mi)
+#pragma unroll
+            for (int j = 0; j < 5; ++j) acc[mi][j] = f4{0.f, 0.f, 0.f, 0.f};
+    };
+    auto gemm_step = [&](const char* buf, int kc, auto tokens_a) {
+        if (SDMI_QKV_SKIP & 1) return;
+        h8 af[4], wf[5];
+#pragma unroll
+        for (int j = 0; j < 5; ++j) wf[j] = *reinterpret_cast<const h8*>(buf + w_off + j * 1024);
+#pragma unroll
+        for (int mi = 0; mi < 4; ++mi) af[mi] = *reinterpret_cast<const h8*>(img + a_off + mi * 16 * kXcRowBytes + (((kc * 4 + q4) ^ a_sw) << 4));
+#pragma unroll
+        for (int mi = 0; mi < 4; ++mi)
+#pragma unroll
+            for (int j = 0; j < 5; ++j) {
+                if constexpr (decltype(tokens_a)::value) acc[mi][j] = __builtin_amdgcn_mfma_f32_16x16x32_f16(af[mi], wf[j], acc[mi][j], 0, 0, 0);
+                else acc[mi][j] = __builtin_amdgcn_mfma_f32_16x16x32_f16(wf[j], af[mi], acc[mi][j], 0, 0, 0);
+            }
+    };
+    auto pack = [&](h4 (&dst)[4][5], const float* bias) {
+        int ln = lane;
+        XC_OPAQUE(ln);
+#pragma unroll
+        for (int j = 0; j < 5; ++j) {
+            const f4 bb = *reinterpret_cast<const f4*>(bias + 80 * wc + 16 * j + 4 * (ln >> 4));
+#pragma unroll
+            for (int mi = 0; mi < 4; ++mi) {
+                dst[mi][j] = h4{(half_t)(acc[mi][j][0] + bb[0]), (half_t)(acc[mi][j][1] + bb[1]), (half_t)(acc[mi][j][2] + bb[2]),
+                                (half_t)(acc[mi][j][3] + bb[3])};
+                XC_OPAQUE(dst[mi][j]);
+            }
+        }
+    };
+    auto to_image = [&](const h4 (&src)[4][5]) {
+        int ln = lane;
+        XC_OPAQUE(ln);
+#pragma unroll
+        for (int mi = 0; mi < 4; ++mi)
+#pragma unroll
+            for (int j = 0; j < 5; ++j)
+                *reinterpret_cast<h4*>(img + xc_img(64 * wr + 16 * mi + (ln & 15), 80 * wc + 16 * j + 4 * (ln >> 4))) = src[mi][j];
+    };
+    auto image_out = [&](half_t* dst, int ld, int col0) {
+        int t = tid;
+        XC_OPAQUE(t);
+#pragma unroll
+        for (int u = 0; u < 10; ++u) {
+            const int pc = u * 512 + t;
+            const int r = pc / 40, ps = pc - r * 40;
+            const h8 hv = *reinterpret_cast<const h8*>(img + pc * 16);
+            if (!(SDMI_QKV_SKIP & 16)) *reinterpret_cast<h8*>(dst + (row0 + r) * ld + col0 + ((ps ^ ((r >> 1) & 7)) << 3)) = hv;
+        }
+    };
+
+    zero_acc();
+    int s = 0;
+#pragma unroll 1
+    for (; s < 10; ++s) {
+        const char* buf = open_step(s);
+        gemm_step(buf, s, std::false_type{});
+    }
+    h4 qh[4][5], kh[4][5];
+    const char* buf10 = open_step(s++);
+    pack(qh, p.b_in);
+    to_image(qh);
+    tile_barrier();
+    {
+        const float inv_c = 1.0f / (float)kXcC;
+        int t = tid;
+        XC_OPAQUE(t);
+        const int sub = t & 7;
+#pragma unroll
+        for (int ps = 0; ps < 2; ++ps) {
+            const int row = ps * 64 + (t >> 3);
+            h8 v[5];
+#pragma unroll
+            for (int i = 0; i < 5; ++i) v[i] = *reinterpret_cast<const h8*>(img + xc_img(row, (i * 8 + sub) * 8));
+            half_t* dst = p.x0 + (row0 + row) * kXcC + sub * 8;
+#pragma unroll
+            for (int i = 0; i < 5; ++i)
+                if (!(SDMI_QKV_SKIP & 8)) *reinterpret_cast<h8*>(dst + i * 64) = v[i];
+            if (SDMI_QKV_SKIP & 2) continue;
+            float a = 0.f;
+#pragma unroll
+            for (int i = 0; i < 5; ++i)
+#pragma unroll
+                for (int e = 0; e < 8; ++e) a += (float)v[i][e];
+            for (int off = 4; off > 0; off >>= 1) a += __shfl_xor(a, off);
+            const float mean = a * inv_c;
+            float sq = 0.f;
+#pragma unroll
+            for (int i = 0; i < 5; ++i)
+#pragma unroll
+                for (int e = 0; e < 8; ++e) { const float d = (float)v[i][e] - mean; sq = fmaf(d, d, sq); }
+            for (int off = 4; off > 0; off >>= 1) sq += __shfl_xor(sq, off);
+            const float rstd = rsqrtf(fmaf(sq, inv_c, p.ln_eps));
+#pragma unroll
+            for (int i = 0; i < 5; ++i) {
+                const int c0 = (i * 8 + sub) * 8;
+                const f4 g0 = *reinterpret_cast<const f4*>(p.ln_gamma + c0), g1 = *reinterpret_cast<const f4*>(p.ln_gamma + c0 + 4);
+                const f4 b0 = *reinterpret_cast<const f4*>(p.ln_beta + c0), b1 = *reinterpret_cast<const f4*>(p.ln_beta + c0 + 4);
+                h8 o;
+#pragma unroll
+                for (int e = 0; e < 8; ++e) {
+                    const float g = e < 4 ? g0[e] : g1[e - 4], bb = e < 4 ? b0[e] : b1[e - 4];
+                    o[e] = (half_t)(((float)v[i][e] - mean) * rstd * g + bb);
+                }
+                *reinterpret_cast<h8*>(img + xc_img(row, c0)) = o;
+            }
+        }
+    }
+    tile_barrier();
+
+    zero_acc();
+    gemm_step(buf10, 0, std::false_type{});
+#pragma unroll 1
+    for (int kc = 1; kc < 10; ++kc) {
+        const char* buf = open_step(s++);
+        gemm_step(buf, kc, std::false_type{});
+    }
+    pack(qh, p.bqk);
+    __builtin_amdgcn_sched_barrier(0);
+    zero_acc();
+#pragma unroll 1
+    for (int kc = 0; kc < 10; ++kc) {
+        const char* buf = open_step(s++);
+        gemm_step(buf, kc, std::false_type{});
+    }
+    pack(kh, p.bqk + kXcC);
+    __builtin_amdgcn_sched_barrier(0);
+    zero_acc();
+#pragma unroll 1
+    for (int kc = 0; kc < 10; ++kc) {
+        const char* buf = open_step(s++);
+        gemm_step(buf, kc, std::true_type{});
+    }
+    XC_WAIT_VM0();
+    __builtin_amdgcn_s_barrier();
+    XC_FENCE();
+    int lv = lane, tv = tid;
+    XC_OPAQUE(lv);
+    XC_OPAQUE(tv);
+#pragma unroll
+    for (int mi = 0; mi < 4; ++mi)
+#pragma unroll
+        for (int j = 0; j < 5; ++j) {
+            const int l16 = lv & 15, q4 = lv >> 4;
+            const int c = 80 * wc + 16 * j + l16, t = 64 * wr + 16 * mi + 4 * q4;
+            const h4 hv = {(half_t)acc[mi][j][0], (half_t)acc[mi][j][1], (half_t)acc[mi][j][2], (half_t)acc[mi][j][3]};
+            *reinterpret_cast<h4*>(img + c * 256 + (((t >> 3) ^ l16) << 4) + (t & 7) * 2) = hv;
+        }
+    tile_barrier();
+    {
+        half_t* vimg = p.vt + (long)image * kXcC * p.vt_ld + tok0;
+#pragma unroll
+        for (int u = 0; u < 10; ++u) {
+            const int pc = u * 512 + tv;
+            const int c = pc >> 4, sl = pc & 15;
+            const h8 hv = *reinterpret_cast<const h8*>(img + pc * 16);
+            if (!(SDMI_QKV_SKIP & 32)) *reinterpret_cast<h8*>(vimg + (long)c * p.vt_ld + ((sl ^ (c & 15)) << 3)) = hv;
+        }
+    }
+    tile_barrier();
+    to_image(qh);
+    tile_barrier();
+    image_out(p.qk, 2 * kXcC, 0);
+    tile_barrier();
+    to_image(kh);
+    tile_barrier();
+    image_out(p.qk, 2 * kXcC, kXcC);
+}
+
+int launch_qkv_chain(const half_t* h, const float* gn_partial, int nchunk, const float* gn_gamma, const float* gn_beta, float gn_eps,
+                     const half_t* w_in, const float* b_in, const float* ln_gamma, const float* ln_beta, float ln_eps, const half_t* wqk,
+                     const float* bqk, const half_t* wv, half_t* x0, half_t* qk, half_t* vt, long rows, int rows_per_image, int C, int vt_ld,
+                     hipStream_t s) {
+    SDMI_REQUIRE(C == kXcC, "q/k/v chain: built for row width C = 320");
+    SDMI_REQUIRE(rows > 0 && rows % kXcRows == 0, "q/k/v chain: rows % 128 == 0");
+    SDMI_REQUIRE(rows_per_image > 0 && rows_per_image % kXcRows == 0, "q/k/v chain: rows_per_image % 128 == 0 (a tile lies in one image)");
+    SDMI_REQUIRE(rows % rows_per_image == 0, "q/k/v chain: rows must be whole images");
+    SDMI_REQUIRE(vt_ld >= rows_per_image, "q/k/v chain: vt_ld >= rows_per_image");
+    SDMI_REQUIRE(vt_ld % 8 == 0, "q/k/v chain: vt_ld % 8 == 0 (16-byte pieces of V^T)");
+    SDMI_REQUIRE(nchunk >= 1, "q/k/v chain: nchunk >= 1 (GroupNorm chunk statistics per image)");
+    SDMI_REQUIRE(h && gn_partial && gn_gamma && gn_beta && w_in && ln_gamma && ln_beta && wqk && wv && x0 && qk && vt, "q/k/v chain: null pointer");
+    SDMI_REQUIRE(rows / kXcRows < (1l << 31), "q/k/v chain: too many tiles");
+    SDMI_REQUIRE((((uintptr_t)h | (uintptr_t)gn_partial | (uintptr_t)gn_gamma | (uintptr_t)gn_beta | (uintptr_t)w_in | (uintptr_t)b_in |
+                   (uintptr_t)ln_gamma | (uintptr_t)ln_beta | (uintptr_t)wqk | (uintptr_t)bqk | (uintptr_t)wv | (uintptr_t)x0 | (uintptr_t)qk |
+                   (uintptr_t)vt) & 15) == 0, "q/k/v chain: 16-byte aligned operands");
+    QkvP p{};
+    const float* zeros = reinterpret_cast<const float*>(zero_page());
+    p.h = h; p.partial = gn_partial; p.gn_gamma = gn_gamma; p.gn_beta = gn_beta; p.w_in = w_in; p.b_in = b_in ? b_in : zeros;
+    p.ln_gamma = ln_gamma; p.ln_beta = ln_beta; p.wqk = wqk; p.bqk = bqk ? bqk : zeros; p.wv = wv;
+    p.x0 = x0; p.qk = qk; p.vt = vt; p.rows_per_image = rows_per_image; p.nchunk = nchunk; p.chunk_rows = cdiv(rows_per_image, nchunk); p.vt_ld = vt_ld;
+    p.gn_eps = gn_eps; p.ln_eps = ln_eps;
+    ProfScope ps("rowchain_qkv groupnorm_apply+proj_in+norm1+qk+vt", 8.0 * (double)rows * C * C, 10.0 * (double)rows * C + 8.0 * C * C, s);
+    auto kern = rowchain_qkv_kernel;
+#ifdef __HIP__
+    static PerDeviceOnce attr;
+    if (attr.need()) SDMI_CHECK_HIP(hipFuncSetAttribute((const void*)kern, hipFuncAttributeMaxDynamicSharedMemorySize, kQcLds));
+    hipLaunchKernelGGL(kern, dim3((unsigned)(rows / kXcRows)), dim3(512), kQcLds, s, p);
+#else
+    hipLaunchKernelGGL(kern, dim3((unsigned)(rows / kXcRows)), dim3(512), 0, s, p);
+#endif
+    SDMI_CHECK_HIP(hipGetLastError());
+    return 0;
+}
+
+}
diff --git a/stable-diffusion-webui_amd/csrc/xattn_chain.hip b/stable-diffusion-webui_amd/csrc/xattn_chain.hip
--- a/stable-diffusion-webui_amd/csrc/xattn_chain.hip
+++ b/stable-diffusion-webui_amd/csrc/xattn_chain.hip
@@ -1,34 +1,10 @@
-#include "common.h"
+#include "chain_tile.h"
 #include "prof.h"
 
 #include <algorithm>
 #include <cmath>
 
 namespace sdmi {
-
-#ifdef __HIP__
-typedef const __attribute__((address_space(1))) void* xgptr_t;
-typedef __attribute__((address_space(3))) void* xlptr_t;
-#define XC_WAIT_VM3() asm volatile("s_waitcnt vmcnt(3) lgkmcnt(0)" ::: "memory")
-#define XC_WAIT_VM0() asm volatile("s_waitcnt vmcnt(0) lgkmcnt(0)" ::: "memory")
-#define XC_FENCE() asm volatile("" ::: "memory")
-#define XC_REAL_BRANCH() asm volatile("")
-#define XC_OPAQUE(x) asm volatile("" : "+v"(x))
-#else
-typedef const void* xgptr_t;
-typedef void* xlptr_t;
-#define XC_WAIT_VM3() ((void)0)
-#define XC_WAIT_VM0() ((void)0)
-#define XC_FENCE() ((void)0)
-#define XC_REAL_BRANCH() ((void)0)
-#define XC_OPAQUE(x) ((void)0)
-#endif
-
-constexpr int kXcC = 320, kXcD = 40, kXcRows = 128;
-constexpr int kXcRowBytes = kXcC * 2;
-constexpr int kXcImage = kXcRows * kXcRowBytes;
-constexpr int kXcStage = 24 * 1024;
-constexpr int kXcLds = kXcImage + 3 * kXcStage;
 
 struct XattnP {
     const half_t* x;
@@ -44,8 +20,6 @@
     int L, Lpad;
     float eps, scale_log2, tau;
 };
-
-__device__ __forceinline__ int xc_img(int row, int col) { return row * kXcRowBytes + ((((col >> 3) ^ ((row >> 1) & 7))) << 4) + (col & 7) * 2; }
 
 __global__ __launch_bounds__(512) void rowchain_xattn_kernel(const XattnP p) {
 #ifdef __HIP__
diff --git a/stable-diffusion-webui_amd/ops.py b/stable-diffusion-webui_amd/ops.py
--- a/stable-diffusion-webui_amd/ops.py
+++ b/stable-diffusion-webui_amd/ops.py
@@ -195,6 +195,26 @@
     return out
 
 
+def qkv_chain(h: torch.Tensor, gn_partial: torch.Tensor, gn_gamma, gn_beta, w_in: torch.Tensor, b_in, ln_gamma, ln_beta, wqk: torch.Tensor,
+              bqk, wv: torch.Tensor, vt_ld: int = 0, vt: torch.Tensor = None, gn_eps: float = 1e-6, ln_eps: float = 1e-5):
+    _lib.require_device()
+    images, rpi, c = h.shape
+    h = h.contiguous()
+    vt_ld = int(vt_ld) if vt_ld else (vt.shape[-1] if vt is not None else rpi)
+    x0 = torch.empty_like(h)
+    qk = torch.empty((images, rpi, 2 * c), dtype=torch.float16, device=h.device)
+    if vt is None:
+        vt = torch.zeros((images, c, vt_ld), dtype=torch.float16, device=h.device)
+    f = lambda t: t.float().contiguous() if t is not None else None
+    gn_partial, gn_gamma, gn_beta, b_in, ln_gamma, ln_beta, bqk = map(f, (gn_partial, gn_gamma, gn_beta, b_in, ln_gamma, ln_beta, bqk))
+    w_in, wqk, wv = w_in.half().contiguous(), wqk.half().contiguous(), wv.half().contiguous()
+    check(lib.sdmi_qkv_chain(ptr(h), ptr(gn_partial), gn_partial.shape[1], ptr(gn_gamma), ptr(gn_beta), float(gn_eps), ptr(w_in),
+                             ptr(b_in) if b_in is not None else None, ptr(ln_gamma), ptr(ln_beta), float(ln_eps), ptr(wqk),
+                             ptr(bqk) if bqk is not None else None, ptr(wv), ptr(x0), ptr(qk), ptr(vt), images * rpi, rpi, c, vt_ld,
+                             stream_ptr()), "sdmi_qkv_chain")
+    return x0, qk, vt
+
+
 def philox_randn(shape, seed: int, offset: int, device) -> torch.Tensor:
     _lib.require_device()
     out = torch.empty(tuple(shape), dtype=torch.float32, device=device)
```

After: 21.16, median of 6. +1.1%, better.
